# WD-Leong/CV-Lite-Object-Detection

Measured on AMD Instinct MI355X. Metric: training images/sec (whole node), FCOS-VOC 512x512 bs=16/GPU, higher is better.
Workload: dtype bf16; 1 GPU; FCOS ResNet-50-FPN train step (targets + fwd + loss + bwd + clip/SGD), 512x512, bs=16 per GPU; model=FCOS-ResNet50-FPN, global_batch=16, image_size=512, parallelism=dp1

## Files before the change

### cv-lite-object-detection_amd/csrc/conv_common.h

```cpp
#pragma once
#include "cvl_common.h"
#include "bn_acc.h"
#include <type_traits>

typedef short s16x8 __attribute__((ext_vector_type(8)));
typedef short s16x4 __attribute__((ext_vector_type(4)));
typedef __bf16 bf16x8 __attribute__((ext_vector_type(8)));
typedef float f32x4 __attribute__((ext_vector_type(4)));

constexpr int kMaxSeg = CVL_CONV_MAX_SEG;

extern thread_local int g_cvl_conv_last_kernel;
extern thread_local int g_cvl_conv_last_ktile;

__device__ __forceinline__ int xcd_remap(int b, int nwg) {
  const int q = nwg / 8, r = nwg % 8, x = b % 8;
  return (x < r ? x * (q + 1) : r * (q + 1) + (x - r) * q) + b / 8;
}

template <int N>
__device__ __forceinline__ void wait_vm() {
  __builtin_amdgcn_s_waitcnt((N & 15) | ((N >> 4) << 14) | (7 << 4) | (15 << 8));
}

__device__ __forceinline__ s16x4 ds_tr16(unsigned addr) {
  s16x4 v;
  asm volatile("ds_read_b64_tr_b16 %0, %1" : "=v"(v) : "v"(addr));
  return v;
}
__device__ __forceinline__ void lgkm_wait() { asm volatile("s_waitcnt lgkmcnt(0)" ::: "memory"); }
__device__ __forceinline__ void tr_pin(s16x4& v) { asm volatile("" : "+v"(v)); }
__device__ __forceinline__ s16x8 tr_join(s16x4 l, s16x4 h) {
  return s16x8{l[0], l[1], l[2], l[3], h[0], h[1], h[2], h[3]};
}

__device__ __forceinline__ unsigned lds_addr(const void* p) {
  return (unsigned)(size_t)(const __attribute__((address_space(3))) void*)p;
}

struct ConvSeg {
  int Hr, Wr, Hs, Ws;
  long src_base, src_img, dst_base, dst_img;
  int m_start;
  int rows;
  const cvl_bf16* w;
  const float* bias;
};

struct ConvArgs {
  const cvl_bf16* src;
  void* dst;
  acc_u64* stats;
  int acc_slots;
  int nseg, B;
  ConvSeg seg[kMaxSeg];
  int Cin, KH, KW, stride, pad_t, pad_l;
  int K, Npad, n_store, ld_dst, dst_coff, dst_f32, relu_out, relu_in;
  float beta;
  int m_tiles, m_total;
  float* slab;
  int splits, ksteps_per_split;
  int dbg;
  int dst_up, dst_w;
  const cvl_bf16* bz;
  const float* bmr;
  const float* bga;
  const float* bbe;
  acc_u64* bsum;
  float bhi;
  const cvl_bf16* by;
  unsigned long long* probe;
  const cvl_bf16* ymask;
};

uint64_t* cvl_probe_current(bool take);
void cvl_probe_enter_call();
void cvl_probe_leave_call();

__device__ __forceinline__ void probe_enter(unsigned long long* p) {
  if (blockIdx.x == 0 && threadIdx.x == 0) __hip_atomic_store(p, wall_clock64(), __ATOMIC_RELAXED, __HIP_MEMORY_SCOPE_AGENT);
}
__device__ __forceinline__ void probe_leave(unsigned long long* p) {
  __syncthreads();
  if (threadIdx.x == 0) {
    if (atomicAdd(p + 3, 1ull) == (unsigned long long)gridDim.x - 1) {
      const unsigned long long t = wall_clock64();
      const unsigned long long t0 = __hip_atomic_load(p, __ATOMIC_RELAXED, __HIP_MEMORY_SCOPE_AGENT);
      atomicAdd(p + 1, t - t0);
      atomicAdd(p + 2, 1ull);
      __hip_atomic_store(p + 3, 0ull, __ATOMIC_RELAXED, __HIP_MEMORY_SCOPE_AGENT);
    }
  }
}

int cvl_bn_acc_prepare(uint64_t* acc, long nstat, hipStream_t s);

int cvl_wgrad_reduce(const float* slab, float* dst0, float* dst1, long n4, int splits, int groups, float beta,
                     hipStream_t s);
int cvl_wgrad_defer_guard(const float* dst, hipStream_t s);
int cvl_wgrad_reduce_lanes(long elems4, int splits);

struct BnSumArgs {
  const cvl_bf16* z;
  const float* mr;
  const float* gamma;
  const float* beta;
  acc_u64* sums;
  float hi;
  const cvl_bf16* y;
};

enum { CVL_BSUM_NONE = 0, CVL_BSUM_Z = 1, CVL_BSUM_Y = 2 };
struct ConvCallOpts {
  bool bn_stats;
  int bsum;
  bool ymask;
  size_t workspace_bytes;
};

enum { CVL_PRE_NONE = 0, CVL_PRE_ZERO_GAPS = 1, CVL_PRE_S2DG3_PACK = 2 };

struct ConvPlan {
  int kernel;
  int bn, bk;
  bool dgrad;
  bool sw;
  bool wres;
  bool prio, acc, stamps;
  int stages;
  int bsum;
  bool ymask;
  int splits, ksteps_per_split;
  int grid;
  size_t workspace_bytes;
  int pre;
  size_t pack_bytes;
  int dbg;
  cvl_conv_desc desc;
  ConvArgs geo;
};

int conv_plan(const cvl_conv_desc* d, const ConvCallOpts& o, ConvPlan* p);
size_t conv_plan_workspace_bound(const cvl_conv_desc* d);
static inline void conv_plan_set_splits(ConvPlan* p, int nk, int want) {
  p->ksteps_per_split = (nk + want - 1) / want;
  p->splits = (nk + p->ksteps_per_split - 1) / p->ksteps_per_split;
}
static inline int conv_plan_ktile(const ConvPlan& p) { return p.kernel == CVL_CK_X32 || p.kernel == CVL_CK_P ? p.bk : 0; }

int launch_base(const ConvPlan& p, const ConvArgs& a, hipStream_t s);
int launch_l(const ConvPlan& p, const ConvArgs& a, hipStream_t s);
int launch_x(const ConvPlan& p, const ConvArgs& a, hipStream_t s);
int launch_h(const ConvPlan& p, const ConvArgs& a, hipStream_t s);
int launch_p(const ConvPlan& p, const ConvArgs& a, hipStream_t s);

bool cvl_conv_h_fits(const cvl_conv_desc* d, const ConvArgs& a, int* halo_px);
constexpr int kConvHWresCb = 2;
constexpr int kConvHStampWgs = 4096;
constexpr unsigned kConvBufRecords = 0x7fffffffu;

template <class F>
static inline void with_bool(bool b, F&& f) {
  if (b) f(std::true_type{});
  else f(std::false_type{});
}

__device__ __forceinline__ long conv_dst_row(const ConvArgs& a, const ConvSeg& S, int img, int q) {
  long r = q;
  if (a.dst_up != 1) {
    const int y = q / S.Wr, x = q - (q / S.Wr) * S.Wr;
    r = (long)y * a.dst_up * a.dst_w + (long)x * a.dst_up;
  }
  return S.dst_base + (long)img * S.dst_img + r;
}

static inline int cvl_conv_prepare(const cvl_conv_desc* d, int bm, ConvArgs* a) {
  CVL_CHECK_ARG(d);
  CVL_CHECK_ARG(d->nseg >= 1 && d->nseg <= kMaxSeg && d->B >= 1);
  CVL_CHECK_ARG(d->Cin > 0 && d->KH > 0 && d->KW > 0 && d->stride > 0);
  CVL_CHECK_ARG(d->mode == CVL_CONV_FWD || d->mode == CVL_CONV_DGRAD);
  CVL_CHECK_ARG(d->Npad > 0 && d->n_store > 0 && d->n_store <= d->Npad);
  CVL_CHECK_ARG(d->ld_dst >= d->dst_coff + d->n_store);
  a->slab = nullptr;
  a->splits = 1;
  a->ksteps_per_split = 0;
  a->dst_up = 1;
  a->dst_w = 0;
  a->dbg = 0;
  a->bz = nullptr; a->bmr = nullptr; a->bga = nullptr; a->bbe = nullptr; a->bsum = nullptr; a->bhi = 0.f;
  a->by = nullptr;
  a->probe = nullptr;
  a->ymask = nullptr;
  a->acc_slots = cvl_bn_acc_slots();
  a->nseg = d->nseg;
  a->B = d->B;
  a->Cin = d->Cin; a->KH = d->KH; a->KW = d->KW; a->stride = d->stride;
  a->pad_t = d->pad_t; a->pad_l = d->pad_l;
  a->K = d->KH * d->KW * d->Cin;
  a->Npad = d->Npad; a->n_store = d->n_store; a->ld_dst = d->ld_dst; a->dst_coff = d->dst_coff;
  a->dst_f32 = d->dst_f32; a->relu_out = d->relu_out; a->relu_in = d->relu_in; a->beta = d->beta;
  int m = 0;
  for (int i = 0; i < kMaxSeg; ++i) {
    ConvSeg& s = a->seg[i];
    if (i >= d->nseg) {
      s = a->seg[0];
      s.m_start = 0x7fffffff;
      continue;
    }
    const cvl_conv_seg& q = d->seg[i];
    CVL_CHECK_ARG(q.Hr > 0 && q.Wr > 0 && q.Hs > 0 && q.Ws > 0 && q.w);
    s.Hr = q.Hr; s.Wr = q.Wr; s.Hs = q.Hs; s.Ws = q.Ws;
    s.src_base = q.src_base; s.src_img = q.src_img; s.dst_base = q.dst_base; s.dst_img = q.dst_img;
    s.w = reinterpret_cast<const cvl_bf16*>(q.w);
    s.bias = q.bias;
    s.m_start = m;
    s.rows = d->B * q.Hr * q.Wr;
    m += ((s.rows + bm - 1) / bm) * bm;
  }
  a->m_total = m;
  a->m_tiles = m / bm;
  return CVL_OK;
}
```

### cv-lite-object-detection_amd/csrc/conv_dispatch.hip

```cpp
#include "conv_common.h"

namespace {

constexpr int BM_BASE = 128, NT_BASE = 256;
constexpr int BM = 256;
constexpr int H_BN = 64, H_BK = 32;

int device_cus() {
  static const int n = cvl_device_cus();
  return n;
}

int pick_bn(int npad) { return npad % 128 == 0 ? 128 : (npad % 64 == 0 ? 64 : 32); }

int base_split_want(const ConvArgs& a) {
  if (a.nseg != 1) return 1;
  const int BN_ = pick_bn(a.Npad), BK_ = a.Cin % 64 == 0 ? 64 : 32;
  const int tiles = a.m_tiles * (a.Npad / BN_);
  const int nk = a.K / BK_;
  const int max_tiles = cvl_tune_int("CVL_KSPLIT_MAX_TILES", 192);
  const int target = cvl_tune_int("CVL_KSPLIT_TARGET", 384);
  const int min_nk = cvl_dispatch_int("ksplit_min_nk", 4);
  if (tiles >= max_tiles || nk < min_nk) return 1;
  int s = (target + tiles - 1) / tiles;
// ... 55 lines not shown
    cvl_conv_seg& g = dd.seg[cls];
    g = q;
    g.Hr = q.Hs;
    g.Wr = q.Ws;
    g.w = sub + (size_t)cls * d->Npad * 4 * d->Cin;
    g.bias = nullptr;
    g.dst_base = q.dst_base + (long)(cls >> 1) * q.Wr + (cls & 1);
  }
  return dd;
}
const cvl_bf16* const kPackPlaceholder = reinterpret_cast<const cvl_bf16*>(16);

bool dst_chunks8(const cvl_conv_desc* d) { return d->n_store % 8 == 0 && d->ld_dst % 8 == 0 && d->dst_coff % 8 == 0; }

bool tiles_in_images(const ConvArgs& a, bool dense) {
  for (int i = 0; i < a.nseg; ++i) {
    const long hw = (long)a.seg[i].Hr * a.seg[i].Wr;
    if (hw % BM || (dense && a.seg[i].dst_img != hw)) return false;
  }
  return true;
}

bool buffer_bounds_ok(const ConvArgs& a) {
  for (int i = 0; i < a.nseg; ++i) {
    const ConvSeg& q = a.seg[i];
    const long src_bytes = (q.src_base + (long)a.B * q.src_img) * a.Cin * 2;
    if (src_bytes >= (long)kConvBufRecords - 65536) return false;
  }
  return (long)a.Npad * a.K * 2 < (long)kConvBufRecords;
}

bool x32_fits(const cvl_conv_desc* d, const ConvArgs& a) {
  const bool dg = d->mode == CVL_CONV_DGRAD;
  if (a.Npad % 256 || a.Cin % 32 || a.K / 32 < 1 || d->KH * d->KW > 32 || a.relu_in || (dg && d->stride != 1) ||
      a.dst_up != 1)
    return false;
  return buffer_bounds_ok(a);
}

bool plan_x(const cvl_conv_desc* d, const ConvArgs& a, const ConvCallOpts& o, ConvPlan* p) {
  if (cvl_dispatch_flag("no_x") || !x32_fits(d, a)) return false;
  p->kernel = CVL_CK_X32;
  p->bn = 256;
  p->bk = 32;
  p->grid = a.m_tiles * (a.Npad / 256);
  p->dbg = cvl_tune_int("CVL_X_ABLATE", 0);
  p->sw = !a.dst_f32 && !o.bn_stats && a.beta == 0.f && dst_chunks8(d) && !cvl_dispatch_flag("x_no_sw");
  p->ymask = p->sw && o.ymask && !a.relu_out && !cvl_dispatch_flag("no_relu_mask_fuse");
  return true;
}

bool p_fits(const cvl_conv_desc* d, const ConvArgs& a, const ConvCallOpts& o) {
  if (d->KH != 1 || d->KW != 1 || d->pad_t || d->pad_l || a.relu_in || a.nseg != 1 || a.K % 32) return false;
  const bool by = o.bsum == CVL_BSUM_Y;
  if (o.bsum && ((d->mode != CVL_CONV_DGRAD && a.dst_up == 1) || a.dst_f32 || (a.beta != 0.f) != by ||
                 (a.dst_up != 1 && !by) || o.bn_stats || (a.seg[0].Hr * a.seg[0].Wr) % BM ||
                 (a.dst_up == 1 && a.seg[0].dst_img != (long)a.seg[0].Hr * a.seg[0].Wr) || a.Npad % 64))
    return false;
  if (d->mode == CVL_CONV_DGRAD && d->stride != 1) return false;
  const ConvSeg& q = a.seg[0];
  if (d->stride == 1 && (q.Hs != q.Hr || q.Ws != q.Wr)) return false;
  if (a.dst_f32 ? (a.n_store % 4 || a.ld_dst % 4 || a.dst_coff % 4) : !dst_chunks8(d)) return false;
  if (o.bn_stats && (a.dst_f32 || (q.Hr * q.Wr) % BM)) return false;
  return buffer_bounds_ok(a);
}

bool plan_p(const cvl_conv_desc* d, const ConvArgs& a, const ConvCallOpts& o, ConvPlan* p) {
  if (cvl_dispatch_flag("no_p") || !p_fits(d, a, o)) return false;
  if (o.bsum && cvl_tune_flag("CVL_CONV_P_NO_BSUM")) return false;
  const bool wide = a.K <= 256 || (a.Npad >= 2 * a.K && cvl_dispatch_int("p_wide128", 1));
  const int bn = wide && a.Npad % 128 == 0 ? 128 : (a.Npad % 64 == 0 ? 64 : 0);
  const int fbn = cvl_dispatch_int("p_bn", 0);
  const int use = o.bsum ? 64 : (fbn && a.Npad % fbn == 0 ? fbn : bn);
  if (!use) return false;
  const int ntiles = a.m_tiles * (a.Npad / use);
  const int ntn = a.Npad / use;
  int grid = cvl_tune_int("CVL_CONV_P_WGS", 256);
  if (grid >= ntiles) grid = ntiles;
  else grid -= grid % ntn;
  if (grid < 1) return false;
  p->kernel = CVL_CK_P;
  p->bn = use;
  p->bk = a.K % 64 == 0 && use != 256 && cvl_dispatch_int("p_k64", 1) ? 64 : 32;
  p->grid = grid;
  p->dbg = cvl_tune_int("CVL_P_ABLATE", 0);
  p->bsum = o.bsum;
  p->acc = a.beta != 0.f && !cvl_tune_flag("CVL_P_NO_ACC");
  return true;
}

bool plan_h(const cvl_conv_desc* d, const ConvArgs& a, const ConvCallOpts& o, size_t ws_bytes, ConvPlan* p) {
  int halo_px = 0;
  if (cvl_dispatch_flag("no_h") || !cvl_conv_h_fits(d, a, &halo_px)) return false;
  const bool stg3 = !cvl_dispatch_flag("h_no_3stage") && halo_px <= 512;
  const bool bs = o.bsum != CVL_BSUM_NONE;
  p->kernel = CVL_CK_H64;
  p->bk = H_BK;
  p->bsum = o.bsum;
  if (a.Npad == 32) {
    if (o.bn_stats || bs) return false;
    p->bn = 32;
    p->stages = stg3 ? 3 : 2;
    p->grid = a.m_tiles < device_cus() ? a.m_tiles : device_cus();
    return true;
  }
  const int tiles = a.m_tiles * (a.Npad / H_BN);
  const bool sw_ok = !d->dst_f32 && d->beta == 0.f && dst_chunks8(d) && !(o.bn_stats && bs) && tiles_in_images(a, bs);
  if (!cvl_dispatch_flag("h_no_n32") && a.Npad % H_BN == 0 && 2 * tiles <= device_cus() && sw_ok) {
    p->bn = 32;
    p->sw = true;
    p->stages = stg3 ? 3 : 2;
    p->grid = 2 * tiles;
    return true;
  }
  const int ncb = a.Cin / H_BK;
  int splits = 1;
  if (a.nseg == 1 && !bs && ws_bytes && d->n_store % 8 == 0 && d->dst_coff % 8 == 0 &&
      (d->dst_f32 || d->ld_dst % 8 == 0) && d->n_store / 8 <= 256) {
    splits = h_split_want(a);
    if (slab_bytes(a, splits) > ws_bytes) splits = 1;
  }
  if (splits > 1) conv_plan_set_splits(p, ncb, splits);
  const int per_cu = cvl_tune_int("CVL_CONV_H_WG_PER_CU", 1);
  p->grid = p->splits > 1 ? tiles : (tiles < device_cus() * per_cu ? tiles : device_cus() * per_cu);
  p->bn = H_BN;
  p->stages = 2;
  p->wres = p->splits <= 1 && a.Npad == H_BN && ncb <= kConvHWresCb && a.nseg == 1 && !cvl_dispatch_flag("h_no_wres");
  p->sw = p->splits <= 1 && sw_ok && !cvl_dispatch_flag("h_no_sw");
  p->stamps = cvl_tune_flag("CVL_H_STAMPS") && p->splits <= 1 && p->grid <= kConvHStampWgs;
  return true;
}

bool large_fits(const cvl_conv_desc* d, const ConvCallOpts& o) {
  if (d->Cin % 32 != 0 || d->relu_in) return false;
  return d->dst_f32 ? (d->n_store % 4 == 0 && !o.bn_stats) : dst_chunks8(d);
}

bool plan_large(const cvl_conv_desc* d, const ConvArgs& a, const ConvCallOpts& o, ConvPlan* p) {
  if (cvl_dispatch_flag("no_l")) return false;
  const bool bs = o.bsum != CVL_BSUM_NONE, by = o.bsum == CVL_BSUM_Y;
  if (bs && (d->mode != CVL_CONV_DGRAD || d->dst_f32 || (d->beta != 0.f && !by) || a.dst_up != 1 || o.bn_stats))
    return false;
  if (by && (d->KH != 1 || d->KW != 1)) return false;
  if (d->Npad == 32 && d->KH == 3 && d->KW == 3 && d->mode == CVL_CONV_FWD && d->dst_f32 && !o.bn_stats &&
      !bs && a.dst_up == 1 && d->Cin % 32 == 0 && !d->relu_in && !cvl_dispatch_flag("no_h32"))
    return plan_h(d, a, o, 0, p);
  if (!large_fits(d, o)) return false;
  if (d->dst_f32 && (cvl_tune_flag("CVL_CONV_L_F32_N8") || cvl_tune_flag("CVL_CONV_L_NO_F32"))) return false;
  const bool l_cin = d->Cin % 64 == 0;
  const bool w256 = d->Npad % 256 == 0 && !cvl_dispatch_flag("no_256") &&
                    (d->mode == CVL_CONV_FWD || !cvl_tune_flag("CVL_CONV_NO_DGRAD_256"));
  const int bn = w256 ? 256 : (d->Npad % 128 == 0 ? 128 : (d->Npad % 64 == 0 ? 64 : 0));
  if (!bn) return false;
  if (l_cin && d->KH * d->KW * d->Cin < cvl_tune_int("CVL_CONV_L_MIN_K", 0) && !bs) return false;
  if (d->KH == 1 && d->KW == 1) {
    if (plan_p(d, a, o, p)) return true;
    if (by) return false;
  }
  const long min_tiles = cvl_dispatch_int("l_min_tiles", 128);
  int use_bn = bn;
  if (use_bn == 256 && (long)a.m_tiles * (a.Npad / 256) < cvl_dispatch_int("l256_min_tiles", 256)) use_bn = 128;
  const int w256_min_k = cvl_dispatch_int("w256_min_k", 512);
  if (use_bn == 256 && a.K < w256_min_k) use_bn = 128;
  const int fill = cvl_tune_int("CVL_CONV_L64_FILL", 256);
  const bool fill_pre = !cvl_tune_flag("CVL_CONV_L64_NO_FILL_PRE");
  const bool to64 = fill && use_bn == 128 && (long)a.m_tiles * (a.Npad / 128) < fill && a.Npad % 64 == 0 &&
                    !(bs && cvl_tune_flag("CVL_BSUM_NO_FILL"));
  if (!l_cin && d->Cin == 32 && bn == 256 && !bs && !o.bn_stats && cvl_dispatch_int("x_cin32", 1) &&
      plan_x(d, a, o, p))
    return true;
  const bool h_width = use_bn == 64 || to64 || !l_cin || cvl_tune_flag("CVL_CONV_H_ANY_N");
  if (h_width && use_bn != 256 && (!bs || ((a.seg[0].Hr * a.seg[0].Wr) % BM == 0 && !o.bn_stats)) &&
      (!bs || tiles_in_images(a, true)) && plan_h(d, a, o, o.workspace_bytes, p))
    return true;
  if (!l_cin) return false;
  if (fill_pre && to64) use_bn = 64;
  if ((long)a.m_tiles * (a.Npad / use_bn) < min_tiles) return false;
  if (to64) use_bn = 64;
  if (o.bn_stats)
    for (int i = 0; i < a.nseg; ++i)
      if ((a.seg[i].Hr * a.seg[i].Wr) % 4) return false;
  if (bs && (use_bn == 256 || !tiles_in_images(a, true))) return false;
  if (use_bn == 256 && plan_x(d, a, o, p)) return true;
  p->kernel = use_bn == 256 ? CVL_CK_L256 : (use_bn == 128 ? CVL_CK_L128 : CVL_CK_L64);
  p->bn = use_bn;
  p->bk = 64;
  p->grid = a.m_tiles * (a.Npad / use_bn);
  p->bsum = o.bsum;
  p->prio = !cvl_tune_flag("CVL_CONV_NO_PRIO");
  p->sw = !a.dst_f32 && a.beta == 0.f && !bs && a.dst_up == 1 && dst_chunks8(d) && !cvl_dispatch_flag("l_no_sw") &&
          (!o.bn_stats || tiles_in_images(a, false));
  return true;
}

void plan_base(const cvl_conv_desc* d, const ConvArgs& a, const ConvCallOpts& o, ConvPlan* p) {
// ... 127 lines not shown
```

### cv-lite-object-detection_amd/csrc/conv_igemm.hip

```cpp
#include "conv_common.h"

namespace {

constexpr int BM = 128;
constexpr int NT = 256;

template <int BK>
__device__ __forceinline__ int swz(int r) {
  return BK == 128 ? (r & 15) : (BK == 64 ? ((r >> 1) & 7) : ((r >> 2) & 3));
}

__device__ __forceinline__ s16x8 relu_bf16x8(s16x8 v) {
#pragma unroll
  for (int i = 0; i < 8; ++i) v[i] = v[i] < 0 ? (short)0 : v[i];
  return v;
}



template <int BN, int BK, bool DGRAD>
__global__ void __launch_bounds__(NT) conv_igemm_kernel(ConvArgs a) {
  constexpr int WM = BM / 2, WN = BN / 2;
  constexpr int TM = WM / 16, TN = WN / 16;
  constexpr int CPR = BK / 8;
// ... 398 lines not shown
  for (int line = blockIdx.y; line < B * H; line += gridDim.y) {
    const int img = line / H, y = line - img * H;
    const bool full = y % s != 0;
    const long base = dst_base + (long)img * dst_img + (long)y * W;
    for (int i = blockIdx.x * blockDim.x + threadIdx.x; i < W * n8; i += gridDim.x * blockDim.x) {
      const int x = i / n8, c = i - x * n8;
      if (!full && x % s == 0) continue;
      const long row = base + x;
      if (is_f32) reinterpret_cast<float*>(dst)[row * ld + coff + c] = 0.f;
      else *reinterpret_cast<s16x8*>(reinterpret_cast<cvl_bf16*>(dst) + row * ld + coff + c * 8) = s16x8{0, 0, 0, 0, 0, 0, 0, 0};
    }
  }
}

namespace {

int pre_pass(const ConvPlan& p, const cvl_conv_desc* d, void* dst, void* workspace, hipStream_t s) {
  if (p.pre == CVL_PRE_S2DG3_PACK) {
    const long b = (16L * d->Npad * (d->Cin / 8) + NT - 1) / NT;
    hipLaunchKernelGGL(s2dgrad3_pack_kernel, dim3((int)(b > 4096 ? 4096 : (b < 1 ? 1 : b))), dim3(NT), 0, s,
                       reinterpret_cast<const cvl_bf16*>(d->seg[0].w), reinterpret_cast<cvl_bf16*>(workspace), d->Npad,
                       d->Cin);
  } else if (p.pre == CVL_PRE_ZERO_GAPS) {
    const cvl_conv_seg& q = d->seg[0];
    const long line = (long)q.Wr * (d->dst_f32 ? d->n_store : d->n_store / 8);
    const int bx = (int)((line + NT - 1) / NT);
    const int by = d->B * q.Hr < 65535 ? d->B * q.Hr : 65535;
    hipLaunchKernelGGL(zero_gaps_kernel, dim3(bx < 1 ? 1 : bx, by), dim3(NT), 0, s, dst, d->dst_f32, q.dst_base,
                       q.dst_img, d->ld_dst, d->dst_coff, d->n_store, d->B, q.Hr, q.Wr, d->stride);
  } else {
    return CVL_OK;
  }
  return cvl_launch_status();
}

struct ConvIo {
  const void* src;
  void* dst;
  acc_u64* stats;
  const BnSumArgs* bsum;
  const void* ymask;
  void* workspace;
};

void fill_args(const ConvPlan& p, const ConvIo& io, ConvArgs* a) {
  *a = p.geo;
  a->src = reinterpret_cast<const cvl_bf16*>(io.src);
  a->dst = io.dst;
  a->stats = io.stats;
  if (p.bsum) {
    const BnSumArgs& b = *io.bsum;
    a->bz = b.z; a->bmr = b.mr; a->bga = b.gamma; a->bbe = b.beta; a->bsum = b.sums; a->bhi = b.hi;
    a->by = b.y;
  }
  if (p.ymask) a->ymask = reinterpret_cast<const cvl_bf16*>(io.ymask);
  if (p.kernel == CVL_CK_X32) a->probe = reinterpret_cast<unsigned long long*>(cvl_probe_current(true));
  a->dbg = p.dbg;
  a->splits = p.splits;
  a->ksteps_per_split = p.ksteps_per_split;
  char* ws = reinterpret_cast<char*>(io.workspace);
  if (p.splits > 1) a->slab = reinterpret_cast<float*>(ws + p.pack_bytes);
  if (p.pre == CVL_PRE_S2DG3_PACK)
    for (int i = 0; i < kMaxSeg; ++i)
      a->seg[i].w = reinterpret_cast<const cvl_bf16*>(ws) + (size_t)(i < a->nseg ? i : 0) * a->Npad * a->K;
}

}

thread_local int g_cvl_conv_last_kernel = CVL_CK_NONE;
thread_local int g_cvl_conv_last_ktile = 0;

extern "C" int cvl_conv_igemm_last_kernel(void) { return g_cvl_conv_last_kernel; }
extern "C" int cvl_conv_igemm_last_ktile(void) { return g_cvl_conv_last_ktile; }

int launch_base(const ConvPlan& p, const ConvArgs& a, hipStream_t s) {
  if (p.bn == 128) launch_bn<128>(p, a, s);
  else if (p.bn == 64) launch_bn<64>(p, a, s);
  else launch_bn<32>(p, a, s);
  return cvl_launch_status();
}

namespace {
int conv_run(const ConvPlan& p, const cvl_conv_desc* d, const ConvIo& io, hipStream_t s) {
  int st = pre_pass(p, d, io.dst, io.workspace, s);
  if (st) return st;
  ConvArgs a;
  fill_args(p, io, &a);
  switch (p.kernel) {
    case CVL_CK_P: st = launch_p(p, a, s); break;
    case CVL_CK_X32: st = launch_x(p, a, s); break;
    case CVL_CK_H64: st = launch_h(p, a, s); break;
    case CVL_CK_L64: case CVL_CK_L128: case CVL_CK_L256: st = launch_l(p, a, s); break;
    default: st = launch_base(p, a, s); break;
  }
  g_cvl_conv_last_kernel = p.kernel;
  g_cvl_conv_last_ktile = conv_plan_ktile(p);
  if (st || p.splits <= 1) return st;
  return splitk_finish_launch(a, s);
}
}

extern "C" const char* cvl_conv_kernel_name(int code) {
  switch (code) {
    case CVL_CK_BASE: return "conv_igemm_kernel (128-row)";
    case CVL_CK_BASE_SPLITK: return "conv_igemm_kernel (128-row, split-K)";
    case CVL_CK_L64: return "conv_igemm_l_kernel<64> (256x64)";
// ... 9 lines not shown
    case CVL_CK_WG_X: return "conv_wgrad_x_kernel (256x256, 5-slot ring of 32-row steps, grouped)";
    case CVL_CK_WG_H: return "conv_wgrad_h_kernel (64 ci x 64 co x 9 taps, 128-row halo steps)";
    case CVL_CK_H64: return "conv_igemm_h_kernel (256x64, 3x3 halo + 9-tap weight stage per channel block)";
    case CVL_CK_P: return "conv_igemm_p_kernel (persistent 1x1, K-tile stream across tiles)";
    default: return "none";
  }
}

int cvl_conv_f32(const cvl_conv_desc* d, const void* src, void* dst, acc_u64* bn_stats, hipStream_t s);
int cvl_relu_backward(const void* dy, const void* y, void* dx, long n, float beta, cvl_stream_t stream);

extern "C" size_t cvl_conv_igemm_workspace_size(const cvl_conv_desc* d) {
  if (!d) return 0;
  if (d->prec == CVL_PREC_F32) return 16;
  return conv_plan_workspace_bound(d);
}

extern "C" int cvl_conv_igemm(const cvl_conv_desc* d, const void* src, void* dst, uint64_t* bn_stats_acc,
                              void* workspace, size_t workspace_bytes, cvl_stream_t stream) {
  CVL_CHECK_ARG(d);
  acc_u64* bn_stats = reinterpret_cast<acc_u64*>(bn_stats_acc);
  if (d->prec == CVL_PREC_F32) return cvl_conv_f32(d, src, dst, bn_stats, (hipStream_t)stream);
  ConvPlan p;
  const int st = conv_plan(d, ConvCallOpts{bn_stats != nullptr, CVL_BSUM_NONE, false, workspace ? workspace_bytes : 0}, &p);
  if (st) return st;
  CVL_CHECK_ARG(src && dst);
  cvl_probe_enter_call();
  const int rst = conv_run(p, d, ConvIo{src, dst, bn_stats, nullptr, nullptr, workspace}, (hipStream_t)stream);
  cvl_probe_leave_call();
  return rst;
}

extern "C" int cvl_conv_igemm_relu_mask(const cvl_conv_desc* d, const void* src, void* dst, const void* y,
                                        void* workspace, size_t workspace_bytes, cvl_stream_t stream) {
  CVL_CHECK_ARG(d && src && dst && y && d->mode == CVL_CONV_DGRAD && d->prec == CVL_PREC_BF16 && !d->dst_f32 &&
                d->beta == 0.f && !d->relu_out);
  ConvPlan p;
  int st = conv_plan(d, ConvCallOpts{false, CVL_BSUM_NONE, true, workspace ? workspace_bytes : 0}, &p);
  if (st) return st;
  if (!p.ymask) CVL_CHECK_ARG(d->ld_dst == d->n_store && d->dst_coff == 0);
  cvl_probe_enter_call();
  st = conv_run(p, d, ConvIo{src, dst, nullptr, nullptr, y, workspace}, (hipStream_t)stream);
  cvl_probe_leave_call();
  if (st || p.ymask) return st;
  long rows = 0;
  for (int i = 0; i < d->nseg; ++i) {
    const long e = d->seg[i].dst_base + (long)d->B * (d->seg[i].dst_img ? d->seg[i].dst_img : (long)d->seg[i].Hr * d->seg[i].Wr);
    rows = e > rows ? e : rows;
  }
  return cvl_relu_backward(dst, y, dst, rows * d->n_store, 0.f, stream);
}

namespace {
int dgrad_bnsum_call(const cvl_conv_desc* d, const void* src, void* dst, int form, const BnSumArgs& b, int32_t* fused,
                     void* workspace, size_t workspace_bytes, cvl_stream_t stream) {
  *fused = 0;
  if (d->prec == CVL_PREC_F32) return cvl_conv_f32(d, src, dst, nullptr, (hipStream_t)stream);
  const size_t ws = workspace ? workspace_bytes : 0;
  ConvPlan p;
  int st = conv_plan(d, ConvCallOpts{false, form, false, ws}, &p);
  if (st) return st;
  const bool fuse = p.kernel != CVL_CK_NONE && src && dst;
  if (!fuse && (st = conv_plan(d, ConvCallOpts{false, CVL_BSUM_NONE, false, ws}, &p))) return st;
  CVL_CHECK_ARG(src && dst);
  if (!fuse) cvl_probe_enter_call();
  st = conv_run(p, d, ConvIo{src, dst, nullptr, &b, nullptr, workspace}, (hipStream_t)stream);
  if (!fuse) cvl_probe_leave_call();
  *fused = fuse && st == CVL_OK ? 1 : 0;
  return st;
}
}

extern "C" int cvl_conv_igemm_dgrad_bnsum(const cvl_conv_desc* d, const void* src, void* dst, const void* z,
                                          const float* mean_rstd, const float* gamma, const float* beta, float act_hi,
                                          uint64_t* sums, int32_t* fused, void* workspace, size_t workspace_bytes,
                                          cvl_stream_t stream) {
  CVL_CHECK_ARG(d && fused && z && mean_rstd && gamma && beta && sums);
  const BnSumArgs b{reinterpret_cast<const cvl_bf16*>(z), mean_rstd, gamma, beta, reinterpret_cast<acc_u64*>(sums),
                    act_hi, nullptr};
  return dgrad_bnsum_call(d, src, dst, CVL_BSUM_Z, b, fused, workspace, workspace_bytes, stream);
}

extern "C" int cvl_conv_igemm_dgrad_bnsum_res(const cvl_conv_desc* d, const void* src, void* dst, const void* y,
                                              const void* z, const float* mean_rstd, const float* gamma,
                                              const float* beta, uint64_t* sums, int32_t* fused, void* workspace,
                                              size_t workspace_bytes, cvl_stream_t stream) {
  CVL_CHECK_ARG(d && fused && y && z && mean_rstd && gamma && beta && sums);
  const BnSumArgs b{reinterpret_cast<const cvl_bf16*>(z), mean_rstd, gamma, beta, reinterpret_cast<acc_u64*>(sums),
                    INFINITY, reinterpret_cast<const cvl_bf16*>(y)};
  return dgrad_bnsum_call(d, src, dst, CVL_BSUM_Y, b, fused, workspace, workspace_bytes, stream);
}
```

### cv-lite-object-detection_amd/csrc/conv_igemm_p.hip

```cpp
#include "conv_common.h"

namespace {

constexpr int NT = 512, BM = 256;
constexpr unsigned kRecords = 0x7fffffffu;
constexpr unsigned kOOB = 0x80000000u;
constexpr int LDS_BYTES = 163840;

template <int BK>
__device__ __forceinline__ int swz(int r) { return (r >> 1) & (BK / 8 - 1); }

__device__ __forceinline__ void dma16(__amdgpu_buffer_rsrc_t r, const void* lds_dst, unsigned voff) {
  __builtin_amdgcn_raw_ptr_buffer_load_lds(r, (__attribute__((address_space(3))) void*)lds_dst, 16, (int)voff, 0,
                                           0, 0);
}

template <int BN, int BK>
struct PCfg {
  static constexpr int WGM = BN == 256 ? 2 : 4, WGN = 8 / WGM;
  static constexpr int WM = BM / WGM, WN = BN / WGN, TM = WM / 16, TN = WN / 16;
  static constexpr int SLOT_B = (BM + BN) * BK * 2;
  static constexpr int PR = 8 * 64 * 16 / (BK * 2);
  static constexpr int APW = BM / PR;
  static constexpr int BPW = BN >= PR ? BN / PR : 1;
  static constexpr int PW = APW + BPW;
  static constexpr int RED_B = WGM * BN * 2 * 4;
  static constexpr int DUMMY_B = BN < PR ? 4 * 1024 : 0;
  static constexpr int NS = (LDS_BYTES - RED_B - DUMMY_B) / SLOT_B;
  static constexpr int D = NS - 1;
  static_assert(D >= 2, "ring too short");
};

typedef __bf16 bf16x2 __attribute__((ext_vector_type(2)));
typedef float f32x2 __attribute__((ext_vector_type(2)));
typedef unsigned u32x4 __attribute__((ext_vector_type(4)));

__device__ __forceinline__ void wait_vm_atleast(int n) {
  if (n >= 63) wait_vm<63>();
  else if (n >= 48) wait_vm<48>();
  else if (n >= 36) wait_vm<36>();
  else if (n >= 30) wait_vm<30>();
  else if (n >= 24) wait_vm<24>();
  else if (n >= 21) wait_vm<21>();
  else if (n >= 18) wait_vm<18>();
  else if (n >= 15) wait_vm<15>();
  else if (n >= 12) wait_vm<12>();
  else if (n >= 9) wait_vm<9>();
  else if (n >= 6) wait_vm<6>();
  else if (n >= 3) wait_vm<3>();
  else wait_vm<0>();
}

__device__ __forceinline__ s16x8 gload16_untracked(const void* p) {
  s16x8 v;
  asm volatile("global_load_dwordx4 %0, %1, off" : "=v"(v) : "v"(p) : "memory");
  return v;
}
__device__ __forceinline__ void pin16(s16x8& v) { asm volatile("" : "+v"(v)); }

template <int BN, int BK, bool RELU, bool F32, int BS = 0, bool ACC = false>
__global__ void __launch_bounds__(NT) conv_igemm_p_kernel(ConvArgs a, int ntiles) {
  using C = PCfg<BN, BK>;
  constexpr int TM = C::TM, TN = C::TN, NS = C::NS, D = C::D;
  __shared__ __attribute__((aligned(16))) char lds[C::NS * C::SLOT_B + C::RED_B + C::DUMMY_B];
  float* red = reinterpret_cast<float*>(lds + NS * C::SLOT_B);
  char* dummy = lds + NS * C::SLOT_B + C::RED_B;

  const int tid = threadIdx.x;
  const int wave = __builtin_amdgcn_readfirstlane(tid >> 6), lane = tid & 63;
  const ConvSeg& S = a.seg[0];
  const int HWr = S.Hr * S.Wr;
  const int ntn = a.Npad / BN;
  const int nk = a.K / BK;
  const int G = gridDim.x;
  const int L = xcd_remap(blockIdx.x, G);
  const int nmc = G / ntn;
  const int mchunk = (a.m_tiles + nmc - 1) / nmc;
  const int mt0 = (L / ntn) * mchunk;
  const int my_tiles = max(0, min(mchunk, a.m_tiles - mt0));
  const int total = my_tiles * nk;
  const bool dense_src = a.stride == 1 && S.Hs == S.Hr && S.Ws == S.Wr && S.src_img == (long)HWr;
  const int Cin2 = a.Cin * 2;
  const int K2 = a.K * 2;

  constexpr int LPR = BK / 8, PR = C::PR, WR = PR / 8;
  const int prow = wave * WR + lane / LPR, ch = lane % LPR;
  const unsigned chs = (unsigned)((ch ^ swz<BK>(prow)) * 16);
  const __amdgpu_buffer_rsrc_t rsA = __builtin_amdgcn_make_buffer_rsrc((void*)a.src, (short)0, (int)kRecords, 0x00020000);
  const __amdgpu_buffer_rsrc_t rsB = __builtin_amdgcn_make_buffer_rsrc((void*)S.w, (short)0, (int)kRecords, 0x00020000);

  int ik = 0, it = 0, islot = 0;
  unsigned ia[C::APW], ib[C::BPW];
  const int n0 = (L % ntn) * BN;
  auto set_issue_tile = [&](int k) {
    const int m0 = (mt0 + k) * BM;
#pragma unroll
    for (int p = 0; p < C::APW; ++p) {
      const int ml = ((a.dbg & 16) ? 0 : m0) + p * PR + prow;
      long pix;
      if (dense_src) {
        pix = S.src_base + ml;
      } else {
        const int img = ml / HWr, q = ml - img * HWr;
        const int oy = q / S.Wr, ox = q - oy * S.Wr;
        pix = S.src_base + (long)img * S.src_img + (long)(oy * a.stride) * S.Ws + ox * a.stride;
      }
      ia[p] = ml < S.rows ? (unsigned)(pix * Cin2) + chs : kOOB;
    }
#pragma unroll
    for (int j = 0; j < C::BPW; ++j) {
      const int nr = n0 + j * PR + prow;
// ... 20 lines not shown
    if (live && ++ik == nk) {
      ik = 0;
      ++it;
      if (it < my_tiles) set_issue_tile(it);
    }
  };

  const int wm = wave / C::WGN, wn = wave % C::WGN;
  const int lr = lane & 15, lg = lane >> 4;
  unsigned fao[TM], fbo[TN];
#pragma unroll
  for (int i = 0; i < TM; ++i) {
    const int r = wm * C::WM + i * 16 + lr;
    fao[i] = (unsigned)(r * BK * 2 + ((lg ^ swz<BK>(r)) * 16));
  }
#pragma unroll
  for (int j = 0; j < TN; ++j) {
    const int r = wn * C::WN + j * 16 + lr;
    fbo[j] = (unsigned)(BM * BK * 2 + r * BK * 2 + ((lg ^ swz<BK>(r)) * 16));
  }
  f32x4 acc[TM][TN];
#pragma unroll
  for (int i = 0; i < TM; ++i)
#pragma unroll
    for (int j = 0; j < TN; ++j) acc[i][j] = f32x4{0.f, 0.f, 0.f, 0.f};

  float bcol[TN][4];
#pragma unroll
  for (int j = 0; j < TN; ++j)
#pragma unroll
    for (int e = 0; e < 4; ++e) {
      const int n = n0 + wn * C::WN + j * 16 + 4 * lg + e;
      bcol[j][e] = (S.bias && n < a.n_store) ? S.bias[n] : 0.f;
    }
  constexpr int NJP = BS ? TN / 2 : 1;
  const int lgo = ((lg & 1) ? 16 : 0) + ((lg & 2) ? 8 : 0);
  float bga[NJP][8], bbe[NJP][8], bm[NJP][8], brs[NJP][8], bs1[NJP][8], bs2[NJP][8];
  int bimg = -1;
  if (BS) {
#pragma unroll
    for (int jp = 0; jp < NJP; ++jp)
#pragma unroll
      for (int u = 0; u < 8; ++u) {
        const int c = n0 + wn * C::WN + jp * 32 + lgo + u;
        bga[jp][u] = a.bga[c];
        bbe[jp][u] = a.bbe[c];
        bs1[jp][u] = 0.f;
        bs2[jp][u] = 0.f;
      }
  }
  wait_vm<0>();
  s16x8 zv[BS ? TM : 1][NJP];
  s16x8 yv[BS == 2 ? TM : 1][BS == 2 ? NJP : 1];
  s16x8 ov[ACC ? TM : 1][ACC ? TN / 2 : 1];

  float ss1[TN][4], ss2[TN][4];
#pragma unroll
  for (int j = 0; j < TN; ++j)
#pragma unroll
    for (int e = 0; e < 4; ++e) { ss1[j][e] = 0.f; ss2[j][e] = 0.f; }
  auto row16_sum = [](float v) {
    v += __int_as_float(__builtin_amdgcn_mov_dpp(__float_as_int(v), 0xB1, 0xF, 0xF, false));
    v += __int_as_float(__builtin_amdgcn_mov_dpp(__float_as_int(v), 0x4E, 0xF, 0xF, false));
    v += __int_as_float(__builtin_amdgcn_mov_dpp(__float_as_int(v), 0x141, 0xF, 0xF, false));
    v += __int_as_float(__builtin_amdgcn_mov_dpp(__float_as_int(v), 0x140, 0xF, 0xF, false));
    return v;
  };
  auto flush_stats = [&](int img) {
#pragma unroll
    for (int j = 0; j < TN; ++j)
#pragma unroll
      for (int e = 0; e < 4; ++e) {
        const float s1 = row16_sum(ss1[j][e]), s2 = row16_sum(ss2[j][e]);
        ss1[j][e] = 0.f;
        ss2[j][e] = 0.f;
        if (lr == 0) {
          const int c = wn * C::WN + j * 16 + 4 * lg + e;
          red[(wm * BN + c) * 2] = s1;
          red[(wm * BN + c) * 2 + 1] = s2;
        }
      }
    __syncthreads();
    if (tid < BN && n0 + tid < a.n_store) {
      float t1 = 0.f, t2 = 0.f;
#pragma unroll
      for (int w = 0; w < C::WGM; ++w) { t1 += red[(w * BN + tid) * 2]; t2 += red[(w * BN + tid) * 2 + 1]; }
      acc_u64* st = a.stats + acc_idx((long)img * a.n_store + n0 + tid, 0, a.acc_slots);
      acc_add(st, t1, a.acc_slots);
      acc_add(st + a.acc_slots, t2, a.acc_slots);
    }
  };

  auto flush_bsum = [&](int img) {
#pragma unroll
    for (int jp = 0; jp < NJP; ++jp)
#pragma unroll
      for (int u = 0; u < 8; ++u) {
        const float t1 = row16_sum(bs1[jp][u]), t2 = row16_sum(bs2[jp][u]);
        bs1[jp][u] = 0.f;
        bs2[jp][u] = 0.f;
        if (lr == 0) {
          const int c = wn * C::WN + jp * 32 + lgo + u;
          red[(wm * BN + c) * 2] = t1;
          red[(wm * BN + c) * 2 + 1] = t2;
        }
      }
    __syncthreads();
    if (tid < BN && n0 + tid < a.n_store) {
      float t1 = 0.f, t2 = 0.f;
#pragma unroll
      for (int w = 0; w < C::WGM; ++w) { t1 += red[(w * BN + tid) * 2]; t2 += red[(w * BN + tid) * 2 + 1]; }
      acc_u64* st = a.bsum + acc_idx((long)img * a.n_store + n0 + tid, 0, a.acc_slots);
      acc_add(st, t1, a.acc_slots);
      acc_add(st + a.acc_slots, t2, a.acc_slots);
    }
  };

  auto epilogue = [&](int k) {
    const int m0 = (mt0 + k) * BM;
    const bool dense_dst = a.dst_up == 1 && S.dst_img == (long)HWr;
    const bool do_stats = a.stats && !(a.dbg & 1);
    if (ACC) {
      wait_vm_atleast(C::PW * (nk - 1));
#pragma unroll
      for (int i = 0; i < TM; ++i)
#pragma unroll
        for (int jp = 0; jp < TN / 2; ++jp) pin16(ov[i][jp]);
    }
    if (BS) {
      wait_vm_atleast(C::PW * (nk - 1));
#pragma unroll
      for (int i = 0; i < TM; ++i)
#pragma unroll
        for (int jp = 0; jp < NJP; ++jp) {
          pin16(zv[i][jp]);
          if (BS == 2) pin16(yv[i][jp]);
        }
      const int img = m0 / HWr;
      if (img != bimg) {
        bimg = img;
#pragma unroll
        for (int jp = 0; jp < NJP; ++jp)
#pragma unroll
          for (int u = 0; u < 8; ++u) {
            const long bc = (long)img * a.n_store + n0 + wn * C::WN + jp * 32 + lgo + u;
            bm[jp][u] = a.bmr[bc * 2];
            brs[jp][u] = a.bmr[bc * 2 + 1];
          }
      }
    }
#pragma unroll
    for (int i = 0; i < TM; ++i) {
      const int ml = m0 + wm * C::WM + i * 16 + lr;
      const bool row_ok = ml < S.rows && !(a.dbg & 2);
      long drow;
      if (dense_dst || !row_ok) {
        drow = S.dst_base + ml;
      } else {
        const int img = ml / HWr, q = ml - img * HWr;
        drow = conv_dst_row(a, S, img, q);
      }
      if (F32) {
#pragma unroll
        for (int j = 0; j < TN; ++j) {
          f32x4 v;
#pragma unroll
          for (int e = 0; e < 4; ++e) {
            v[e] = acc[i][j][e] + bcol[j][e];
            if (RELU) v[e] = fmaxf(v[e], 0.f);
          }
          const int n = n0 + wn * C::WN + j * 16 + 4 * lg;
          if (!row_ok || n >= a.n_store) continue;
          f32x4* pd = reinterpret_cast<f32x4*>(reinterpret_cast<float*>(a.dst) + drow * a.ld_dst + a.dst_coff + n);
          if (a.beta != 0.f) v += a.beta * *pd;
          *pd = v;
        }
        continue;
      }
#pragma unroll
      for (int j = 0; j < TN; j += 2) {
        unsigned pk[2][2];
#pragma unroll
        for (int jj = 0; jj < 2; ++jj)
#pragma unroll
          for (int h = 0; h < 2; ++h) {
            float v0 = acc[i][j + jj][2 * h] + bcol[j + jj][2 * h];
            float v1 = acc[i][j + jj][2 * h + 1] + bcol[j + jj][2 * h + 1];
            if (RELU) { v0 = fmaxf(v0, 0.f); v1 = fmaxf(v1, 0.f); }
            const unsigned u = __builtin_bit_cast(unsigned, __builtin_convertvector((f32x2){v0, v1}, bf16x2));
            pk[jj][h] = u;
            if (do_stats) {
              const float r0 = __uint_as_float(u << 16), r1 = __uint_as_float(u & 0xffff0000u);
              ss1[j + jj][2 * h] += r0;
              ss2[j + jj][2 * h] = __builtin_fmaf(r0, r0, ss2[j + jj][2 * h]);
              ss1[j + jj][2 * h + 1] += r1;
              ss2[j + jj][2 * h + 1] = __builtin_fmaf(r1, r1, ss2[j + jj][2 * h + 1]);
            }
          }
#pragma unroll
        for (int h = 0; h < 2; ++h) {
          const auto sw = __builtin_amdgcn_permlane16_swap(pk[0][h], pk[1][h], false, false);
          pk[0][h] = sw[0];
          pk[1][h] = sw[1];
        }
        const int n = n0 + wn * C::WN + j * 16 + ((lg & 1) ? 16 : 0) + ((lg & 2) ? 8 : 0);
        if (!row_ok || n >= a.n_store) continue;
        s16x8* pd = reinterpret_cast<s16x8*>(reinterpret_cast<cvl_bf16*>(a.dst) + drow * a.ld_dst + a.dst_coff + n);
        s16x8 o = __builtin_bit_cast(s16x8, (u32x4){pk[0][0], pk[0][1], pk[1][0], pk[1][1]});
        if (ACC) {
          const s16x8 old = ov[i][j / 2];
#pragma unroll
          for (int u = 0; u < 8; ++u)
            o[u] = (short)f32_to_bf16(bf16_to_f32((cvl_bf16)o[u]) + a.beta * bf16_to_f32((cvl_bf16)old[u]));
        } else if (a.beta != 0.f) {
          const s16x8 old = *pd;
#pragma unroll
          for (int u = 0; u < 8; ++u)
            o[u] = (short)f32_to_bf16(bf16_to_f32((cvl_bf16)o[u]) + a.beta * bf16_to_f32((cvl_bf16)old[u]));
        }
        if (BS) {
          const s16x8 zz = zv[i][j / 2];
#pragma unroll
          for (int u = 0; u < 8; ++u) {
            const float zf = bf16_to_f32((cvl_bf16)zz[u]);
            const float xh = (zf - bm[j / 2][u]) * brs[j / 2][u];
            bool on;
            if (BS == 2) {
              on = bf16_to_f32((cvl_bf16)yv[i][j / 2][u]) > 0.f;
            } else {
              const float af = __builtin_fmaf(bga[j / 2][u], xh, bbe[j / 2][u]);
              on = af > 0.f && af < a.bhi;
            }
            const float gv = on ? bf16_to_f32((cvl_bf16)o[u]) : 0.f;
            bs1[j / 2][u] += gv;
            bs2[j / 2][u] = __builtin_fmaf(gv, xh, bs2[j / 2][u]);
          }
        }
        *pd = o;
      }
    }
    if (do_stats) {
      const int img = m0 / HWr;
      if (k == my_tiles - 1 || (m0 + BM) / HWr != img) flush_stats(img);
    }
    if (BS) {
      const int img = m0 / HWr;
      if (k == my_tiles - 1 || (m0 + BM) / HWr != img) flush_bsum(img);
    }
#pragma unroll
    for (int i = 0; i < TM; ++i)
#pragma unroll
      for (int j = 0; j < TN; ++j) acc[i][j] = f32x4{0.f, 0.f, 0.f, 0.f};
  };

  unsigned long long* stamp = ((a.dbg & 8) && tid == 0) ? reinterpret_cast<unsigned long long*>(a.dst) + blockIdx.x * 4 : nullptr;
  if (stamp) stamp[0] = wall_clock64();
#pragma unroll
  for (int d = 0; d < D; ++d) issue();
  int rslot = 0, ck = 0, ct = 0;
  for (int g = 0; g < total; ++g) {
    wait_vm<(D - 1) * C::PW>();
    __builtin_amdgcn_s_barrier();
    asm volatile("" ::: "memory");
    issue();
    if (ACC && ck == 0) {
      const int m0 = (mt0 + ct) * BM;
      const bool dense_dst = a.dst_up == 1 && S.dst_img == (long)HWr;
#pragma unroll
      for (int i = 0; i < TM; ++i) {
        const int ml = m0 + wm * C::WM + i * 16 + lr;
        long drow = S.dst_base;
        if (ml < S.rows) {
          if (dense_dst) {
            drow = S.dst_base + ml;
          } else {
            const int img = ml / HWr, q = ml - img * HWr;
            drow = conv_dst_row(a, S, img, q);
          }
        }
#pragma unroll
        for (int jp = 0; jp < TN / 2; ++jp) {
          int n = n0 + wn * C::WN + jp * 32 + lgo;
          if (n >= a.n_store) n = 0;
          ov[i][jp] = gload16_untracked(reinterpret_cast<const cvl_bf16*>(a.dst) + drow * a.ld_dst + a.dst_coff + n);
        }
      }
    }
    if (BS && ck == 0) {
      const int m0 = (mt0 + ct) * BM;
      const bool dense_dst = a.dst_up == 1 && S.dst_img == (long)HWr;
#pragma unroll
      for (int i = 0; i < TM; ++i)
#pragma unroll
        for (int jp = 0; jp < NJP; ++jp) {
          const int ml = m0 + wm * C::WM + i * 16 + lr;
          long row = S.dst_base + ml;
          if (!dense_dst && ml < S.rows) {
            const int img = ml / HWr, q = ml - img * HWr;
            row = conv_dst_row(a, S, img, q);
          }
          zv[i][jp] = gload16_untracked(a.bz + row * a.ld_dst + a.dst_coff + n0 + wn * C::WN + jp * 32 + lgo);
          if (BS == 2)
            yv[i][jp] = gload16_untracked(a.by + row * a.ld_dst + a.dst_coff + n0 + wn * C::WN + jp * 32 + lgo);
        }
    }
    const char* sl = lds + rslot * C::SLOT_B;
#pragma unroll
    for (int kh = 0; kh < BK / 32; ++kh) {
      s16x8 fa[TM], fb[TN];
#pragma unroll
      for (int i = 0; i < TM; ++i) fa[i] = *reinterpret_cast<const s16x8*>(sl + (fao[i] ^ (unsigned)(kh * 64)));
#pragma unroll
      for (int j = 0; j < TN; ++j) fb[j] = *reinterpret_cast<const s16x8*>(sl + (fbo[j] ^ (unsigned)(kh * 64)));
#pragma unroll
      for (int i = 0; i < TM; ++i)
#pragma unroll
        for (int j = 0; j < TN; ++j)
          acc[i][j] = __builtin_amdgcn_mfma_f32_16x16x32_bf16(__builtin_bit_cast(bf16x8, fb[j]),
                                                               __builtin_bit_cast(bf16x8, fa[i]), acc[i][j], 0, 0, 0);
    }
    rslot = rslot == NS - 1 ? 0 : rslot + 1;
    if (++ck == nk) {
      ck = 0;
      epilogue(ct);
      ++ct;
    }
  }
  wait_vm<0>();
  if (stamp) { stamp[1] = wall_clock64(); stamp[2] = total; }
}

template <int BN_, int BK_, bool ACC_>
void p_launch(const ConvPlan& p, const ConvArgs& a, hipStream_t s) {
  const dim3 grid(p.grid);
  const int ntiles = a.m_tiles * (a.Npad / p.bn);
  if (p.bsum == CVL_BSUM_Y) {
    hipLaunchKernelGGL((conv_igemm_p_kernel<64, BK_, false, false, 2, true>), grid, dim3(NT), 0, s, a, ntiles);
  } else if (p.bsum) {
    hipLaunchKernelGGL((conv_igemm_p_kernel<64, BK_, false, false, 1>), grid, dim3(NT), 0, s, a, ntiles);
  } else if (a.dst_f32) {
    with_bool(a.relu_out != 0, [&](auto RELU) {
      hipLaunchKernelGGL((conv_igemm_p_kernel<BN_, BK_, decltype(RELU)::value, true>), grid, dim3(NT), 0, s, a, ntiles);
    });
  } else if (a.relu_out) {
    hipLaunchKernelGGL((conv_igemm_p_kernel<BN_, BK_, true, false>), grid, dim3(NT), 0, s, a, ntiles);
  } else if (p.acc) {
    hipLaunchKernelGGL((conv_igemm_p_kernel<BN_, BK_, false, false, false, ACC_>), grid, dim3(NT), 0, s, a, ntiles);
  } else {
    hipLaunchKernelGGL((conv_igemm_p_kernel<BN_, BK_, false, false>), grid, dim3(NT), 0, s, a, ntiles);
  }
}

}

int launch_p(const ConvPlan& p, const ConvArgs& a, hipStream_t s) {
  if (p.bn == 256) p_launch<256, 32, false>(p, a, s);
  else if (p.bn == 128 && p.bk == 64) p_launch<128, 64, true>(p, a, s);
  else if (p.bn == 128) p_launch<128, 32, true>(p, a, s);
  else if (p.bk == 64) p_launch<64, 64, true>(p, a, s);
  else p_launch<64, 32, true>(p, a, s);
  return cvl_launch_status();
}
```

### cv-lite-object-detection_amd/csrc/nn_ops.hip

```cpp
#include "conv_common.h"

namespace {

constexpr int NT = 256;

__device__ __forceinline__ void unpack8(s16x8 v, float* f) {
#pragma unroll
  for (int i = 0; i < 8; ++i) f[i] = bf16_to_f32((cvl_bf16)v[i]);
}
__device__ __forceinline__ s16x8 pack8(const float* f) {
  s16x8 v;
#pragma unroll
  for (int i = 0; i < 8; ++i) v[i] = (short)f32_to_bf16(f[i]);
  return v;
}

#ifndef BN_NT
#define BN_NT 1
#endif
__device__ __forceinline__ s16x8 ld_rows(const cvl_bf16* p) {
  if (BN_NT) return __builtin_nontemporal_load(reinterpret_cast<const s16x8*>(p));
  return *reinterpret_cast<const s16x8*>(p);
}

// ... 204 lines not shown
  const int c = blockIdx.x * NT + threadIdx.x;
  if (c >= C) return;
  for (int b = 0; b < B; ++b) {
    float mean, rstd;
    double var;
    const long bc = (long)b * C + c;
    bn_moments(acc_dec(stats, bc, 0, slots), acc_dec(stats, bc, 1, slots), HW, eps, &mean, &rstd, &var);
    mr[((long)b * C + c) * 2] = mean;
    mr[((long)b * C + c) * 2 + 1] = rstd;
  }
  if (run_mean) bn_running(stats, slots, B, C, c, HW, eps, momentum, run_mean, run_var);
}

struct BnFin {
  const acc_u64* stats;
  float* mr_out;
  float* run_mean;
  float* run_var;
  float eps, momentum;
  int slots;
};

#ifndef BNA_UNR_V
#define BNA_UNR_V 4
#endif
constexpr int BNA_UNR = BNA_UNR_V;

constexpr int BN_FIN_MAXC = 2048;

struct BnRes {
  const cvl_bf16* z;
  const float* gamma;
  const float* beta;
  BnFin fin;
};

__device__ __forceinline__ void bn_fin_prologue(const BnFin& fin, float2* smr, int b, int C, int HW) {
  for (int c = threadIdx.x; c < C; c += NT) {
    const long bc = (long)b * C + c;
    float mm, rr;
    double var;
    bn_moments(acc_dec(fin.stats, bc, 0, fin.slots), acc_dec(fin.stats, bc, 1, fin.slots), HW, fin.eps, &mm, &rr, &var);
    smr[c] = float2{mm, rr};
    if (blockIdx.x == 0) { fin.mr_out[bc * 2] = mm; fin.mr_out[bc * 2 + 1] = rr; }
  }
}

__device__ __forceinline__ void bn_fin_running(const BnFin& fin, int nimg, int C, int HW) {
  if (fin.run_mean)
    for (int c = blockIdx.x * NT + threadIdx.x; c < C; c += gridDim.x * NT)
      bn_running(fin.stats, fin.slots, nimg, C, c, HW, fin.eps, fin.momentum, fin.run_mean, fin.run_var);
}

template <bool FIN, bool RBN = false>
__global__ void __launch_bounds__(NT) bn_apply_kernel(const cvl_bf16* __restrict__ z, const float* __restrict__ mr,
                                                      const float* __restrict__ gamma, const float* __restrict__ beta,
                                                      const cvl_bf16* __restrict__ res, cvl_bf16* __restrict__ y,
                                                      int C, int HW, int relu, int rows_per_blk, BnFin fin,
                                                      BnRes rb) {
  static_assert(FIN || !RBN, "the BN residual form fuses both finalizes");
  const int b = FIN ? (int)blockIdx.y - 1 : (int)blockIdx.y;
  const int C8 = C / 8;
  const int tpr = C8 < NT ? C8 : NT;
  const int rpp = NT / tpr;
  const int cg = threadIdx.x % tpr, rsub = threadIdx.x / tpr;
  __shared__ float2 smr[FIN ? BN_FIN_MAXC : 1];
  __shared__ float2 smr2[RBN ? BN_FIN_MAXC : 1];
  if (FIN && b < 0) {
    bn_fin_running(fin, (int)gridDim.y - 1, C, HW);
    if (RBN) bn_fin_running(rb.fin, (int)gridDim.y - 1, C, HW);
    return;
  }
  if (FIN) {
    bn_fin_prologue(fin, smr, b, C, HW);
    if (RBN) bn_fin_prologue(rb.fin, smr2, b, C, HW);
    __syncthreads();
  }
  if (rsub >= rpp) return;
  const int r0 = blockIdx.x * rows_per_blk;
  const int r1 = min(r0 + rows_per_blk, HW);
  for (int cgb = cg; cgb < C8; cgb += tpr) {
    const int c0 = cgb * 8;
    float m[8], rs[8], ga[8], be[8];
    float m2[8], rs2[8], ga2[8], be2[8];
#pragma unroll
    for (int u = 0; u < 8; ++u) {
      const long bc = (long)b * C + c0 + u;
      if (FIN) {
        m[u] = smr[c0 + u].x;
        rs[u] = smr[c0 + u].y;
      } else {
        m[u] = mr[bc * 2];
        rs[u] = mr[bc * 2 + 1];
      }
      ga[u] = gamma[c0 + u];
      be[u] = beta[c0 + u];
      if (RBN) {
        m2[u] = smr2[c0 + u].x;
        rs2[u] = smr2[c0 + u].y;
        ga2[u] = rb.gamma[c0 + u];
        be2[u] = rb.beta[c0 + u];
      }
    }
    const cvl_bf16* rsrc = RBN ? rb.z : res;
    for (int r = r0 + rsub; r < r1; r += rpp * BNA_UNR) {
      s16x8 vz[BNA_UNR], vr[BNA_UNR];
      long off[BNA_UNR];
#pragma unroll
      for (int q = 0; q < BNA_UNR; ++q) {
        const int rq = min(r + q * rpp, r1 - 1);
        off[q] = ((long)b * HW + rq) * C + c0;
        vz[q] = ld_rows(z + off[q]);
        if (rsrc) vr[q] = ld_rows(rsrc + off[q]);
      }
#pragma unroll
      for (int q = 0; q < BNA_UNR; ++q) {
        if (r + q * rpp >= r1) break;
        float v[8], rr[8];
        unpack8(vz[q], v);
        if (RBN) {
          unpack8(vr[q], rr);
#pragma unroll
          for (int u = 0; u < 8; ++u) rr[u] = bn_affine(rr[u], m2[u], rs2[u], ga2[u], be2[u]);
          unpack8(pack8(rr), rr);
        } else if (res) {
          unpack8(vr[q], rr);
        }
#pragma unroll
        for (int u = 0; u < 8; ++u) {
          float o = bn_affine(v[u], m[u], rs[u], ga[u], be[u]);
          if (RBN || res) o += rr[u];
          if (relu) o = o > 0.f ? o : 0.f;
          if (relu == 2) o = fminf(o, 6.0f);
          v[u] = o;
        }
        *reinterpret_cast<s16x8*>(y + off[q]) = pack8(v);
      }
    }
  }
}

inline int bn_rows_per_blk(int B, int HW, int C) {
  const int C8 = C / 8, tpr = C8 < NT ? C8 : NT, rpp = NT / tpr;
  static const int target = cvl_tune_int("CVL_BNA_BLOCKS", 1024);
  const int chunks = (target + B - 1) / B;
  int rpb = (HW + chunks - 1) / chunks;
  const int lo = rpp * 4 * (C8 > NT ? 1 : 1);
  rpb = rpb < lo ? lo : rpb;
  return (rpb + rpp - 1) / rpp * rpp;
}

inline int bn1_rows_per_blk(int B, int HW, int C) {
  const int C8 = C / 8, tpr = C8 < NT ? C8 : NT, rpp = NT / tpr;
  static const int target = cvl_tune_int("CVL_BNB1_BLOCKS", 512);
  const int chunks = (target + B - 1) / B;
  int rpb = (HW + chunks - 1) / chunks;
  const int lo = rpp * 4;
  rpb = rpb < lo ? lo : rpb;
  return (rpb + rpp - 1) / rpp * rpp;
}

#ifndef BN_UNR_V
#define BN_UNR_V 4
#endif
constexpr int BN_UNR = BN_UNR_V;

struct BnPG {
  float* dgamma;
  float* dbeta;
  float* conv_dbias;
  float beta_acc;
  const acc_u64* psums;
  int slots;
  const cvl_bf16* sc_z = nullptr;
  const float* sc_mr = nullptr;
};

template <int PASS, int MASK = 0, bool SC = false>
__global__ void __launch_bounds__(NT) bn_bwd_kernel(const cvl_bf16* __restrict__ dy, const cvl_bf16* __restrict__ y,
                                                    const cvl_bf16* __restrict__ z, const float* __restrict__ mr,
                                                    const float* __restrict__ gamma, const acc_u64* __restrict__ sums,
                                                    cvl_bf16* __restrict__ dz, cvl_bf16* __restrict__ g_out,
                                                    float* __restrict__ part, int C, int HW, int rows_per_blk,
                                                    int group, float dz_beta, BnPG pg,
                                                    const float* __restrict__ bnb, float act_hi) {
  const int nimg = PASS == 1 ? (int)gridDim.y - 1 : (int)gridDim.y;
  const int b = PASS == 1 ? (int)blockIdx.y - 1 : (int)blockIdx.y;
  const int C8 = C / 8;
  const int tpr = C8 < NT ? C8 : NT;
  const int rpp = NT / tpr;
  const int cg = threadIdx.x % tpr, rsub = threadIdx.x / tpr;
  const int r0 = blockIdx.x * rows_per_blk;
  const int r1 = min(r0 + rows_per_blk, HW);
  const int g0 = (b / group) * group;
  const int gsz = min(g0 + group, nimg) - g0;
  const float inv = 1.0f / ((float)HW * (float)gsz);
  __shared__ float red[NT][17];
  if (PASS == 1 && b < 0) {
    if (!pg.dgamma) return;
    const acc_u64* ps = pg.psums ? pg.psums : sums;
    for (int c = blockIdx.x * NT + threadIdx.x; c < C; c += gridDim.x * NT) {
      if (pg.conv_dbias) pg.conv_dbias[c] = 0.f;
      double a1 = 0.0, a2 = 0.0;
#pragma unroll 8
      for (int bb = 0; bb < nimg; ++bb) {
        a1 += acc_dec(ps, (long)bb * C + c, 0, pg.slots);
        a2 += acc_dec(ps, (long)bb * C + c, 1, pg.slots);
      }
      pg.dbeta[c] = (float)a1 + (pg.beta_acc != 0.f ? pg.beta_acc * pg.dbeta[c] : 0.f);
      pg.dgamma[c] = (float)a2 + (pg.beta_acc != 0.f ? pg.beta_acc * pg.dgamma[c] : 0.f);
    }
    return;
  }
  const int n_iter = (C8 + tpr - 1) / tpr;
  for (int itr = 0; itr < n_iter; ++itr) {
    const int cgb = itr * tpr + cg;
    const bool act = cgb < C8;
    const int c0 = (act ? cgb : C8 - 1) * 8;
    float m[8], rs[8], s1[8], s2[8], k1[8], k2[8], gm[8], ga[8], be[8];
    float msc[8], rssc[8];
    const bool use_y = PASS != 2 && (MASK == 0 ? y != nullptr : MASK == 1);
    const bool zmask = PASS != 2 && (MASK == 0 ? (!y && bnb) : MASK == 2);
#pragma unroll
    for (int u = 0; u < 8; ++u) {
      const long bc = (long)b * C + c0 + u;
      m[u] = PASS == 2 ? 0.f : mr[bc * 2];
      rs[u] = PASS == 2 ? 1.f : mr[bc * 2 + 1];
      ga[u] = zmask ? gamma[c0 + u] : 0.f;
      be[u] = zmask ? bnb[c0 + u] : 0.f;
      s1[u] = 0.f; s2[u] = 0.f;
      if (PASS == 1) {
        k1[u] = (float)acc_dec(sums, bc, 0, pg.slots) * inv;
        k2[u] = (float)acc_dec(sums, bc, 1, pg.slots) * inv;
        gm[u] = gamma[c0 + u] * rs[u];
      }
      if (SC) {
        msc[u] = pg.sc_mr[bc * 2];
        rssc[u] = pg.sc_mr[bc * 2 + 1];
      }
    }

    if (rsub < rpp && act) {
      for (int r = r0 + rsub; r < r1; r += rpp * BN_UNR) {
        s16x8 vg[BN_UNR], vz[BN_UNR], vy[BN_UNR], vs[SC ? BN_UNR : 1];
        long off[BN_UNR];
#pragma unroll
        for (int q = 0; q < BN_UNR; ++q) {
          const int rq = min(r + q * rpp, r1 - 1);
          off[q] = ((long)b * HW + rq) * C + c0;
          vg[q] = ld_rows(dy + off[q]);
          if (PASS != 2) vz[q] = ld_rows(z + off[q]);
          if (use_y) vy[q] = ld_rows(y + off[q]);
          if (SC) vs[q] = ld_rows(pg.sc_z + off[q]);
        }
#pragma unroll
        for (int q = 0; q < BN_UNR; ++q) {
          const bool ok = r + q * rpp < r1;
          float g[8], zz[8];
          unpack8(vg[q], g);
          if (PASS == 2) {
            if (ok) {
#pragma unroll
              for (int u = 0; u < 8; ++u) { s1[u] += g[u]; s2[u] += g[u] * g[u]; }
            }
            continue;
          }
          unpack8(vz[q], zz);
          if (use_y) {
            float yy[8];
            unpack8(vy[q], yy);
#pragma unroll
            for (int u = 0; u < 8; ++u) g[u] = (yy[u] > 0.f && yy[u] < act_hi) ? g[u] : 0.f;
          } else if (zmask) {
#pragma unroll
            for (int u = 0; u < 8; ++u) {
              const float a = bn_affine(zz[u], m[u], rs[u], ga[u], be[u]);
              g[u] = (a > 0.f && a < act_hi) ? g[u] : 0.f;
            }
          }
          if (PASS == 0) {
            if (ok) {
#pragma unroll
              for (int u = 0; u < 8; ++u) {
                s1[u] += g[u];
                s2[u] += g[u] * ((zz[u] - m[u]) * rs[u]);
              }
            }
          } else if (ok) {
            if (g_out) *reinterpret_cast<s16x8*>(g_out + off[q]) = pack8(g);
            if (SC) {
              float zs[8];
              unpack8(vs[q], zs);
#pragma unroll
              for (int u = 0; u < 8; ++u) {
                s1[u] += g[u];
                s2[u] += g[u] * ((zs[u] - msc[u]) * rssc[u]);
              }
            }
            float o[8];
#pragma unroll
            for (int u = 0; u < 8; ++u) {
              const float xh = (zz[u] - m[u]) * rs[u];
              o[u] = gm[u] * (g[u] - k1[u] - xh * k2[u]);
            }
            if (dz_beta != 0.f) {
              float old[8];
              unpack8(*reinterpret_cast<const s16x8*>(dz + off[q]), old);
#pragma unroll
              for (int u = 0; u < 8; ++u) o[u] += dz_beta * old[u];
            }
            *reinterpret_cast<s16x8*>(dz + off[q]) = pack8(o);
          }
        }
      }
    }
    if (PASS == 1 && !SC) continue;
    __syncthreads();
#pragma unroll
    for (int u = 0; u < 8; ++u) { red[threadIdx.x][u] = s1[u]; red[threadIdx.x][8 + u] = s2[u]; }
    __syncthreads();
    if (rsub == 0 && act) {
      float* pp = part + (((long)b * gridDim.x + blockIdx.x) * C + c0) * 2;
      for (int u = 0; u < 8; ++u) {
        float a1 = 0.f, a2 = 0.f;
        for (int k = 0; k < rpp; ++k) { a1 += red[k * tpr + cg][u]; a2 += red[k * tpr + cg][8 + u]; }
// ... 834 lines not shown
  if (Kp % 8 == 0 && Kp <= I2C_MAXK && KH <= 7 && KW <= 7 && stride >= 1 && stride <= 2 && C <= 4 &&
      (long)B * Ho < (1L << 24)) {
    const int nseg = (Wo + I2C_PX - 1) / I2C_PX;
    const int nrb = (Ho + I2C_OY - 1) / I2C_OY;
    hipLaunchKernelGGL(im2col_tile_kernel, dim3(B * nrb * nseg), dim3(NT), 0, S_, x, (cvl_bf16*)out, H, W, C, KH, KW,
                       stride, pad_t, pad_l, Ho, Wo, Kp / 8);
    return cvl_launch_status();
  }
  if (Kp % 8 == 0 && total / 8 < (1L << 31) - NT && (long)H * W * C < (1L << 31)) {
    const int n8 = (int)(total / 8);
    hipLaunchKernelGGL(im2col8_kernel, dim3((n8 + NT - 1) / NT), dim3(NT), 0, S_, x, (cvl_bf16*)out, n8, H, W, C,
                       KW, KH * KW * C, stride, pad_t, pad_l, Ho, Wo, Kp / 8);
    return cvl_launch_status();
  }
  hipLaunchKernelGGL(im2col_kernel, dim3(grid_for(total)), dim3(NT), 0, S_, x, (cvl_bf16*)out, B, H, W,
                     C, KH, KW, stride, pad_t, pad_l, Ho, Wo, Kp);
  return cvl_launch_status();
}

extern "C" int cvl_bn_acc_slots(void) { return g_acc_slots; }

int cvl_bn_acc_prepare(uint64_t* acc, long nstat, hipStream_t s) { return acc_decode_launch((acc_u64*)acc, nstat, s); }

extern "C" int cvl_bn_set_exact(int on) {
  g_acc_slots = on ? kAccSlots : 1;
  return CVL_OK;
}

extern "C" int cvl_bn_acc_decode(const uint64_t* acc, double* out, int64_t n, cvl_stream_t stream) {
  CVL_CHECK_ARG(acc && out && n >= 0);
  if (n == 0) return CVL_OK;
  hipLaunchKernelGGL(bn_acc_decode_kernel, dim3(grid_for(n)), dim3(NT), 0, S_, (const acc_u64*)acc, out, (long)n,
                     g_acc_slots);
  return cvl_launch_status();
}

extern "C" int cvl_bn_finalize(uint64_t* stats, float* mean_rstd, float* run_mean, float* run_var,
                               int B, int C, int HW, float eps, float momentum, cvl_stream_t stream) {
  CVL_CHECK_ARG(stats && mean_rstd && B > 0 && C > 0 && HW > 0);
  const int dst = acc_decode_launch((acc_u64*)stats, 2L * B * C, S_);
  if (dst) return dst;
  hipLaunchKernelGGL(bn_finalize_kernel, dim3((C + NT - 1) / NT), dim3(NT), 0, S_, (const acc_u64*)stats, mean_rstd,
                     run_mean, run_var, B, C, HW, eps, momentum, g_acc_slots);
  return cvl_launch_status();
}

extern "C" int cvl_bn_apply(const void* z, const float* mean_rstd, const float* gamma, const float* beta,
                            const void* residual, void* y, int B, int HW, int C, int relu,
                            cvl_stream_t stream) {
  CVL_CHECK_ARG(z && mean_rstd && gamma && beta && y && C % 8 == 0 && B > 0 && HW > 0);
  const int rpb = bn_rows_per_blk(B, HW, C);
  hipLaunchKernelGGL(bn_apply_kernel<false>, dim3((HW + rpb - 1) / rpb, B), dim3(NT), 0, S_, (const cvl_bf16*)z,
                     mean_rstd, gamma, beta, (const cvl_bf16*)residual, (cvl_bf16*)y, C, HW, relu, rpb,
                     BnFin{nullptr, nullptr, nullptr, nullptr, 0.f, 0.f, 1}, BnRes{});
  return cvl_launch_status();
}

extern "C" int cvl_bn_finalize_apply(uint64_t* stats, float* mean_rstd, float* run_mean, float* run_var,
                                     const void* z, const float* gamma, const float* beta, const void* residual,
                                     void* y, int B, int HW, int C, int relu, float eps, float momentum,
                                     cvl_stream_t stream) {
  CVL_CHECK_ARG(stats && mean_rstd && z && gamma && beta && y && C % 8 == 0 && B > 0 && HW > 0);
  CVL_CHECK_ARG(C <= BN_FIN_MAXC);
  CVL_CHECK_ARG((run_mean == nullptr) == (run_var == nullptr));
  const int dst = acc_decode_launch((acc_u64*)stats, 2L * B * C, S_);
  if (dst) return dst;
  const int rpb = bn_rows_per_blk(B, HW, C);
  hipLaunchKernelGGL(bn_apply_kernel<true>, dim3((HW + rpb - 1) / rpb, B + 1), dim3(NT), 0, S_, (const cvl_bf16*)z,
                     (const float*)nullptr, gamma, beta, (const cvl_bf16*)residual, (cvl_bf16*)y, C, HW, relu, rpb,
                     BnFin{(const acc_u64*)stats, mean_rstd, run_mean, run_var, eps, momentum, g_acc_slots}, BnRes{});
  return cvl_launch_status();
}

extern "C" int cvl_bn_finalize_apply_bnres(uint64_t* stats, float* mean_rstd, float* run_mean, float* run_var,
                                           const void* z, const float* gamma, const float* beta, uint64_t* res_stats,
                                           float* res_mean_rstd, float* res_run_mean, float* res_run_var,
                                           const void* res_z, const float* res_gamma, const float* res_beta,
                                           float res_eps, float res_momentum, void* y, int B, int HW, int C, int relu,
                                           float eps, float momentum, cvl_stream_t stream) {
  CVL_CHECK_ARG(stats && mean_rstd && z && gamma && beta && y && C % 8 == 0 && B > 0 && HW > 0);
  CVL_CHECK_ARG(res_stats && res_mean_rstd && res_z && res_gamma && res_beta);
  CVL_CHECK_ARG(C <= BN_FIN_MAXC);
  CVL_CHECK_ARG((run_mean == nullptr) == (run_var == nullptr));
  CVL_CHECK_ARG((res_run_mean == nullptr) == (res_run_var == nullptr));
  int dst = acc_decode_launch((acc_u64*)stats, 2L * B * C, S_);
  if (!dst) dst = acc_decode_launch((acc_u64*)res_stats, 2L * B * C, S_);
  if (dst) return dst;
  const int rpb = bn_rows_per_blk(B, HW, C);
  hipLaunchKernelGGL((bn_apply_kernel<true, true>), dim3((HW + rpb - 1) / rpb, B + 1), dim3(NT), 0, S_, (const cvl_bf16*)z,
                     (const float*)nullptr, gamma, beta, (const cvl_bf16*)nullptr, (cvl_bf16*)y, C, HW, relu, rpb,
                     BnFin{(const acc_u64*)stats, mean_rstd, run_mean, run_var, eps, momentum, g_acc_slots},
                     BnRes{(const cvl_bf16*)res_z, res_gamma, res_beta,
                           BnFin{(const acc_u64*)res_stats, res_mean_rstd, res_run_mean, res_run_var, res_eps,
                                 res_momentum, g_acc_slots}});
  return cvl_launch_status();
}

extern "C" size_t cvl_bn_backward_workspace_size(int B, int HW, int C) {
  if (B <= 0 || HW <= 0 || C <= 0) return 0;
  const int rpb = bn_bwd_rows_per_blk(B, HW, C);
  const int nchunk = (HW + rpb - 1) / rpb;
  return sizeof(acc_u64) * 2 * (size_t)B * C + sizeof(double) * 2 * (size_t)C +
         sizeof(float) * 2 * 2 * (size_t)B * nchunk * C;
}

static int bn_backward_impl(const void* dy, const void* y_relu, const float* bn_beta, const void* z,
                            const float* mean_rstd, const float* gamma, void* workspace, size_t workspace_bytes,
                            void* dz, void* g_out, float* dgamma, float* dbeta, float beta_acc, float* conv_dbias,
                            int B, int HW, int C, cvl_stream_t stream, float act_hi = INFINITY) {
  CVL_CHECK_ARG(dy && z && mean_rstd && gamma && workspace && dz && dgamma && dbeta && C % 8 == 0);
  CVL_CHECK_ARG(B > 0 && HW > 0);
  CVL_CHECK_ARG(workspace_bytes >= cvl_bn_backward_workspace_size(B, HW, C));
  const int rpb = bn_bwd_rows_per_blk(B, HW, C);
  const int nchunk = (HW + rpb - 1) / rpb;
  acc_u64* sums = reinterpret_cast<acc_u64*>(workspace);
  double* dbsum = reinterpret_cast<double*>(sums + 2 * (size_t)B * C);
  float* part0 = reinterpret_cast<float*>(dbsum + 2 * (size_t)C);
  dim3 g1(nchunk, B);
  const bool ym = y_relu != nullptr, zm = !ym && bn_beta != nullptr;
  auto k0 = ym ? bn_bwd_kernel<0, 1> : zm ? bn_bwd_kernel<0, 2> : bn_bwd_kernel<0, 3>;
  auto k1 = ym ? bn_bwd_kernel<1, 1> : zm ? bn_bwd_kernel<1, 2> : bn_bwd_kernel<1, 3>;
  hipLaunchKernelGGL(k0, g1, dim3(NT), 0, S_, (const cvl_bf16*)dy, (const cvl_bf16*)y_relu,
                     (const cvl_bf16*)z, mean_rstd, gamma, (const acc_u64*)nullptr, (cvl_bf16*)nullptr,
                     (cvl_bf16*)nullptr, part0, C, HW, rpb, 1, 0.f, BnPG{}, bn_beta, act_hi);
  hipLaunchKernelGGL(bn_colsum_kernel, dim3((C + 31) / 32, B), dim3(NT), 0, S_, (const float*)part0, nchunk, C,
                     sums, 1);
  const int rpb1 = bn1_rows_per_blk(B, HW, C);
  hipLaunchKernelGGL(k1, dim3((HW + rpb1 - 1) / rpb1, B + 1), dim3(NT), 0, S_, (const cvl_bf16*)dy, (const cvl_bf16*)y_relu,
                     (const cvl_bf16*)z, mean_rstd, gamma, (const acc_u64*)sums, (cvl_bf16*)dz, (cvl_bf16*)g_out,
                     (float*)nullptr, C, HW, rpb1, 1, 0.f, BnPG{dgamma, dbeta, conv_dbias, beta_acc, nullptr, 1}, bn_beta,
                     act_hi);
  return cvl_launch_status();
}

extern "C" int cvl_bn_backward(const void* dy, const void* y_relu, const void* z, const float* mean_rstd,
                               const float* gamma, void* workspace, size_t workspace_bytes, void* dz, void* g_out,
                               float* dgamma, float* dbeta, float beta_acc, float* conv_dbias, int B, int HW,
                               int C, cvl_stream_t stream) {
  return bn_backward_impl(dy, y_relu, nullptr, z, mean_rstd, gamma, workspace, workspace_bytes, dz, g_out, dgamma,
                          dbeta, beta_acc, conv_dbias, B, HW, C, stream);
}

extern "C" int cvl_bn_backward_relu(const void* dy, const void* z, const float* mean_rstd, const float* gamma,
                                    const float* beta, void* workspace, size_t workspace_bytes, void* dz,
                                    float* dgamma, float* dbeta, float beta_acc, float* conv_dbias, int B, int HW,
                                    int C, cvl_stream_t stream) {
  CVL_CHECK_ARG(beta);
  return bn_backward_impl(dy, nullptr, beta, z, mean_rstd, gamma, workspace, workspace_bytes, dz, nullptr, dgamma,
                          dbeta, beta_acc, conv_dbias, B, HW, C, stream);
}

extern "C" int cvl_bn_backward_relu6(const void* dy, const void* z, const float* mean_rstd, const float* gamma,
                                     const float* beta, void* workspace, size_t workspace_bytes, void* dz,
                                     float* dgamma, float* dbeta, float beta_acc, float* conv_dbias, int B, int HW,
                                     int C, cvl_stream_t stream) {
  CVL_CHECK_ARG(beta);
  return bn_backward_impl(dy, nullptr, beta, z, mean_rstd, gamma, workspace, workspace_bytes, dz, nullptr, dgamma,
                          dbeta, beta_acc, conv_dbias, B, HW, C, stream, 6.0f);
}

extern "C" int cvl_bn_backward_relu_sums(const void* dy, const void* z, const float* mean_rstd, const float* gamma,
                                         const float* beta, uint64_t* sums, void* dz, float* dgamma,
                                         float* dbeta, float beta_acc, float* conv_dbias, float act_hi, int B,
                                         int HW, int C, cvl_stream_t stream) {
  CVL_CHECK_ARG(dy && z && mean_rstd && gamma && beta && sums && dz && dgamma && dbeta && C % 8 == 0);
  CVL_CHECK_ARG(B > 0 && HW > 0);
  const int dst = acc_decode_launch((acc_u64*)sums, 2L * B * C, S_);
  if (dst) return dst;
  const int rpb = bn1_rows_per_blk(B, HW, C);
  const int nchunk = (HW + rpb - 1) / rpb;
  hipLaunchKernelGGL((bn_bwd_kernel<1, 2>), dim3(nchunk, B + 1), dim3(NT), 0, S_, (const cvl_bf16*)dy, (const cvl_bf16*)nullptr,
                     (const cvl_bf16*)z, mean_rstd, gamma, (const acc_u64*)sums, (cvl_bf16*)dz, (cvl_bf16*)nullptr, (float*)nullptr,
                     C, HW, rpb, 1, 0.f, BnPG{dgamma, dbeta, conv_dbias, beta_acc, nullptr, g_acc_slots}, beta, act_hi);
  return cvl_launch_status();
}

extern "C" int cvl_bn_backward_res_sums(const void* dy, const void* y, const void* z, const float* mean_rstd,
                                        const float* gamma, uint64_t* sums, void* dz, void* g_out,
                                        float* dgamma, float* dbeta, float beta_acc, float* conv_dbias, int B,
                                        int HW, int C, cvl_stream_t stream) {
  CVL_CHECK_ARG(dy && y && z && mean_rstd && gamma && sums && dz && dgamma && dbeta && C % 8 == 0);
  CVL_CHECK_ARG(B > 0 && HW > 0);
  const int dst = acc_decode_launch((acc_u64*)sums, 2L * B * C, S_);
  if (dst) return dst;
  const int rpb = bn1_rows_per_blk(B, HW, C);
  const int nchunk = (HW + rpb - 1) / rpb;
  hipLaunchKernelGGL((bn_bwd_kernel<1, 1>), dim3(nchunk, B + 1), dim3(NT), 0, S_, (const cvl_bf16*)dy, (const cvl_bf16*)y,
                     (const cvl_bf16*)z, mean_rstd, gamma, (const acc_u64*)sums, (cvl_bf16*)dz, (cvl_bf16*)g_out, (float*)nullptr,
                     C, HW, rpb, 1, 0.f, BnPG{dgamma, dbeta, conv_dbias, beta_acc, nullptr, g_acc_slots}, (const float*)nullptr, INFINITY);
  return cvl_launch_status();
}

extern "C" size_t cvl_bn_backward_res_sums_sc_workspace_size(int B, int HW, int C) {
  if (B <= 0 || HW <= 0 || C <= 0) return 0;
  const int rpb = bn1_rows_per_blk(B, HW, C);
  return sizeof(float) * 2 * (size_t)B * ((HW + rpb - 1) / rpb) * C;
}

extern "C" int cvl_bn_backward_res_sums_sc(const void* dy, const void* y, const void* z, const float* mean_rstd,
                                           const float* gamma, uint64_t* sums, void* dz, void* g_out,
                                           float* dgamma, float* dbeta, float beta_acc, float* conv_dbias,
                                           const void* z_sc, const float* mean_rstd_sc, void* workspace,
                                           size_t workspace_bytes, uint64_t* sc_sums, int B, int HW, int C,
                                           cvl_stream_t stream) {
  CVL_CHECK_ARG(dy && y && z && mean_rstd && gamma && sums && dz && g_out && dgamma && dbeta && C % 8 == 0);
  CVL_CHECK_ARG(z_sc && mean_rstd_sc && workspace && sc_sums && B > 0 && HW > 0);
  CVL_CHECK_ARG(workspace_bytes >= cvl_bn_backward_res_sums_sc_workspace_size(B, HW, C));
  const int dst = acc_decode_launch((acc_u64*)sums, 2L * B * C, S_);
  if (dst) return dst;
  const int rpb = bn1_rows_per_blk(B, HW, C);
  const int nchunk = (HW + rpb - 1) / rpb;
  float* part = reinterpret_cast<float*>(workspace);
  BnPG pg{dgamma, dbeta, conv_dbias, beta_acc, nullptr, g_acc_slots};
  pg.sc_z = (const cvl_bf16*)z_sc;
  pg.sc_mr = mean_rstd_sc;
  hipLaunchKernelGGL((bn_bwd_kernel<1, 1, true>), dim3(nchunk, B + 1), dim3(NT), 0, S_, (const cvl_bf16*)dy,
                     (const cvl_bf16*)y, (const cvl_bf16*)z, mean_rstd, gamma, (const acc_u64*)sums, (cvl_bf16*)dz,
                     (cvl_bf16*)g_out, part, C, HW, rpb, 1, 0.f, pg, (const float*)nullptr, INFINITY);
  hipLaunchKernelGGL(bn_colsum_kernel, dim3((C + 31) / 32, B), dim3(NT), 0, S_, (const float*)part, nchunk, C,
                     (acc_u64*)sc_sums, 1);
  return cvl_launch_status();
}

extern "C" size_t cvl_bn_backward_sc_workspace_size(int B, int HW, int C) {
  if (B <= 0 || HW <= 0 || C <= 0) return 0;
  return cvl_bn_backward_workspace_size(B, HW, C) + cvl_bn_backward_res_sums_sc_workspace_size(B, HW, C);
}

extern "C" int cvl_bn_backward_sc(const void* dy, const void* y, const void* z, const float* mean_rstd,
                                  const float* gamma, void* workspace, size_t workspace_bytes, void* dz, void* g_out,
                                  float* dgamma, float* dbeta, float beta_acc, float* conv_dbias, const void* z_sc,
                                  const float* mean_rstd_sc, uint64_t* sc_sums, int B, int HW, int C,
                                  cvl_stream_t stream) {
  CVL_CHECK_ARG(dy && y && z && mean_rstd && gamma && workspace && dz && g_out && dgamma && dbeta && C % 8 == 0);
  CVL_CHECK_ARG(z_sc && mean_rstd_sc && sc_sums && B > 0 && HW > 0);
  CVL_CHECK_ARG(workspace_bytes >= cvl_bn_backward_sc_workspace_size(B, HW, C));
  const int rpb = bn_bwd_rows_per_blk(B, HW, C);
  const int nchunk = (HW + rpb - 1) / rpb;
  acc_u64* sums = reinterpret_cast<acc_u64*>(workspace);
  double* dbsum = reinterpret_cast<double*>(sums + 2 * (size_t)B * C);
  float* part0 = reinterpret_cast<float*>(dbsum + 2 * (size_t)C);
  float* part_sc = reinterpret_cast<float*>(reinterpret_cast<char*>(workspace) + cvl_bn_backward_workspace_size(B, HW, C));
  hipLaunchKernelGGL((bn_bwd_kernel<0, 1>), dim3(nchunk, B), dim3(NT), 0, S_, (const cvl_bf16*)dy, (const cvl_bf16*)y,
                     (const cvl_bf16*)z, mean_rstd, gamma, (const acc_u64*)nullptr, (cvl_bf16*)nullptr,
                     (cvl_bf16*)nullptr, part0, C, HW, rpb, 1, 0.f, BnPG{}, (const float*)nullptr, INFINITY);
  hipLaunchKernelGGL(bn_colsum_kernel, dim3((C + 31) / 32, B), dim3(NT), 0, S_, (const float*)part0, nchunk, C,
                     sums, 1);
  const int rpb1 = bn1_rows_per_blk(B, HW, C);
  const int nchunk1 = (HW + rpb1 - 1) / rpb1;
  BnPG pg{dgamma, dbeta, conv_dbias, beta_acc, nullptr, 1};
  pg.sc_z = (const cvl_bf16*)z_sc;
  pg.sc_mr = mean_rstd_sc;
  hipLaunchKernelGGL((bn_bwd_kernel<1, 1, true>), dim3(nchunk1, B + 1), dim3(NT), 0, S_, (const cvl_bf16*)dy,
                     (const cvl_bf16*)y, (const cvl_bf16*)z, mean_rstd, gamma, (const acc_u64*)sums, (cvl_bf16*)dz,
                     (cvl_bf16*)g_out, part_sc, C, HW, rpb1, 1, 0.f, pg, (const float*)nullptr, INFINITY);
  hipLaunchKernelGGL(bn_colsum_kernel, dim3((C + 31) / 32, B), dim3(NT), 0, S_, (const float*)part_sc, nchunk1, C,
                     (acc_u64*)sc_sums, 1);
  return cvl_launch_status();
}

extern "C" int cvl_bn_backward_sums(const void* dy, const void* z, const float* mean_rstd, const float* gamma,
                                    const uint64_t* sums, void* dz, float* dgamma, float* dbeta, float beta_acc,
                                    float* conv_dbias, int B, int HW, int C, cvl_stream_t stream) {
  CVL_CHECK_ARG(dy && z && mean_rstd && gamma && sums && dz && dgamma && dbeta && C % 8 == 0 && B > 0 && HW > 0);
  const int rpb = bn1_rows_per_blk(B, HW, C);
  const int nchunk = (HW + rpb - 1) / rpb;
  hipLaunchKernelGGL((bn_bwd_kernel<1, 3>), dim3(nchunk, B + 1), dim3(NT), 0, S_, (const cvl_bf16*)dy,
                     (const cvl_bf16*)nullptr, (const cvl_bf16*)z, mean_rstd, gamma, (const acc_u64*)sums, (cvl_bf16*)dz,
                     (cvl_bf16*)nullptr, (float*)nullptr, C, HW, rpb, 1, 0.f,
                     BnPG{dgamma, dbeta, conv_dbias, beta_acc, nullptr, 1}, (const float*)nullptr, INFINITY);
  return cvl_launch_status();
}

extern "C" int cvl_bn_relu_maxpool3x3s2(const void* z, const float* mean_rstd, const float* gamma, const float* beta,
                                        void* y, uint8_t* argmax, int B, int H, int W, int C, cvl_stream_t stream) {
  CVL_CHECK_ARG(z && mean_rstd && gamma && beta && y && argmax && C % 8 == 0 && B > 0);
  const int Ho = (H + 2 - 3) / 2 + 1, Wo = (W + 2 - 3) / 2 + 1;
  if (C == 64) {
    const long blocks = (long)B * ((Ho + PTY - 1) / PTY) * ((Wo + PTX - 1) / PTX);
    CVL_CHECK_ARG(blocks < (1l << 31));
    hipLaunchKernelGGL(bn_relu_maxpool64_kernel, dim3((unsigned)blocks), dim3(NT), 0, S_, (const cvl_bf16*)z,
                       mean_rstd, gamma, beta, (cvl_bf16*)y, argmax, H, W, Ho, Wo);
    return cvl_launch_status();
  }
  const long total = (long)B * Ho * Wo * (C / 8);
  hipLaunchKernelGGL(bn_relu_maxpool_kernel, dim3(grid_for(total)), dim3(NT), 0, S_, (const cvl_bf16*)z, mean_rstd,
                     gamma, beta, (cvl_bf16*)y, argmax, B, H, W, C, Ho, Wo);
  return cvl_launch_status();
}

extern "C" int cvl_maxpool3x3s2(const void* x, void* y, uint8_t* argmax, int B, int H, int W, int C,
                                cvl_stream_t stream) {
  CVL_CHECK_ARG(x && y && argmax && C % 8 == 0);
  const int Ho = (H + 2 - 3) / 2 + 1, Wo = (W + 2 - 3) / 2 + 1;
  const long total = (long)B * Ho * Wo * (C / 8);
  hipLaunchKernelGGL(maxpool_fwd_kernel, dim3(grid_for(total)), dim3(NT), 0, S_, (const cvl_bf16*)x,
                     (cvl_bf16*)y, argmax, B, H, W, C, Ho, Wo);
  return cvl_launch_status();
}

extern "C" int cvl_maxpool3x3s2_backward(const void* dy, const uint8_t* argmax, void* dx, int B, int H,
                                         int W, int C, cvl_stream_t stream) {
  CVL_CHECK_ARG(dy && dx && argmax && C % 8 == 0);
  const int Ho = (H + 2 - 3) / 2 + 1, Wo = (W + 2 - 3) / 2 + 1;
  if (C == 64) {
    const long blocks = (long)B * ((H + BTY - 1) / BTY) * ((W + BTX - 1) / BTX);
    CVL_CHECK_ARG(blocks < (1l << 31));
    hipLaunchKernelGGL(maxpool_bwd64_kernel<false>, dim3((unsigned)blocks), dim3(NT), 0, S_, (const cvl_bf16*)dy, argmax,
                       (cvl_bf16*)dx, H, W, Ho, Wo, PoolBn{});
    return cvl_launch_status();
  }
// ... 253 lines not shown
```

### cv-lite-object-detection_amd/cvlite/_lib.py

```python
import ctypes
import os

import torch

_HERE = os.path.dirname(os.path.abspath(__file__))
LIB_PATH = os.environ.get("CVL_LIB") or os.path.join(_HERE, "libcvlite_hip.so")


def dispatch(key, default=0):
    for tok in os.environ.get("CVL_DISPATCH", "").split(","):
        k, _, v = tok.strip().partition("=")
        if k == key:
            return int(v) if v else 1
    return default

c_int, c_float, c_size_t, c_void_p = ctypes.c_int, ctypes.c_float, ctypes.c_size_t, ctypes.c_void_p
P = c_void_p

SIGNATURES = {
    "cvl_version": (c_int, []),
    "cvl_fcos_assign": (c_int, [P, P, P, c_int, c_int, c_int, c_int, c_int, P, P, P, P, P]),
    "cvl_fcos_loss_workspace_size": (c_size_t, [c_int, c_int]),
    "cvl_fcos_loss": (c_int, [P, c_int, P, c_int, P, c_int, c_int, c_int, c_int, c_float, P,
                              P, c_int, c_int, P, c_int, c_int, P, c_size_t, P]),
    "cvl_fcos_loss_ex": (c_int, [P, c_int, P, c_int, P, c_int, c_int, c_int, c_int, c_float, c_float, c_float,
                                 c_float, P, P, c_int, c_int, P, c_int, c_int, P, c_size_t, P]),
    "cvl_fcos_decode": (c_int, [P, c_int, c_int, c_int, ctypes.c_double, P, P]),
    "cvl_fcos_v1_decode": (c_int, [P, c_int, c_int, c_int, c_float, c_float, P, P]),
    "cvl_conv_igemm_workspace_size": (c_size_t, [P]),
    "cvl_conv_igemm": (c_int, [P, P, P, P, P, c_size_t, P]),
    "cvl_conv_igemm_relu_mask": (c_int, [P, P, P, P, P, c_size_t, P]),
    "cvl_conv_igemm_last_kernel": (c_int, []),
    "cvl_conv_igemm_last_ktile": (c_int, []),
    "cvl_conv_igemm_plan": (c_int, [P, c_int, c_size_t, P, P]),
    "cvl_conv_kernel_name": (ctypes.c_char_p, [c_int]),
    "cvl_centernet_peak_decode_workspace_size": (ctypes.c_size_t, [c_int, c_int, c_int, c_int]),
    "cvl_centernet_peak_decode": (c_int, [P, c_int, c_int, c_int, c_int, c_int, c_float, c_float, c_int, P, P, P,
                                          ctypes.c_size_t, P]),
    "cvl_conv_igemm_dgrad_bnsum": (c_int, [P, P, P, P, P, P, P, c_float, P, P, P, ctypes.c_size_t, P]),
    "cvl_bn_backward_relu_sums": (c_int, [P, P, P, P, P, P, P, P, P, c_float, P, c_float, c_int, c_int, c_int, P]),
    "cvl_conv_igemm_dgrad_bnsum_res": (c_int, [P, P, P, P, P, P, P, P, P, P, P, ctypes.c_size_t, P]),
    "cvl_bn_backward_res_sums": (c_int, [P, P, P, P, P, P, P, P, P, P, c_float, P, c_int, c_int, c_int, P]),
    "cvl_bn_backward_res_sums_sc_workspace_size": (c_size_t, [c_int, c_int, c_int]),
    "cvl_bn_backward_res_sums_sc": (c_int, [P, P, P, P, P, P, P, P, P, P, c_float, P, P, P, P, c_size_t, P, c_int,
                                            c_int, c_int, P]),
    "cvl_bn_backward_sums": (c_int, [P, P, P, P, P, P, P, P, c_float, P, c_int, c_int, c_int, P]),
    "cvl_bn_backward_sc_workspace_size": (c_size_t, [c_int, c_int, c_int]),
    "cvl_bn_backward_sc": (c_int, [P, P, P, P, P, P, c_size_t, P, P, P, P, c_float, P, P, P, P, c_int, c_int, c_int, P]),
    "cvl_probe_arm": (c_int, [P]),
    "cvl_probe_clock_hz": (ctypes.c_double, []),
    "cvl_conv_wgrad_workspace_size": (c_size_t, [P]),
    "cvl_conv_wgrad": (c_int, [P, P, P, P, c_float, P, c_size_t, P]),
    "cvl_conv_wgrad_grouped_workspace_size": (c_size_t, [P, c_int]),
    "cvl_conv_wgrad_grouped": (c_int, [P, c_int, P, P, P, c_float, P, c_size_t, P]),
    "cvl_conv_wgrad_batch_workspace_size": (c_size_t, [P, c_int]),
    "cvl_conv_wgrad_batch": (c_int, [P, c_int, P, P, P, c_float, P, c_size_t, P]),
    "cvl_pack_conv_weights": (c_int, [P, c_int, c_int, c_int, c_int, c_int, c_int, P, c_int, c_int, P, P]),
    "cvl_pack_conv_weights_multi": (c_int, [P, P, c_int, P]),
    "cvl_im2col": (c_int, [P, c_int, c_int, c_int, c_int, c_int, c_int, c_int, c_int, c_int, c_int,
                           c_int, c_int, P, P]),
    "cvl_bn_finalize": (c_int, [P, P, P, P, c_int, c_int, c_int, c_float, c_float, P]),
    "cvl_bn_acc_decode": (c_int, [P, P, ctypes.c_int64, P]),
    "cvl_bn_set_exact": (c_int, [c_int]),
    "cvl_bn_acc_slots": (c_int, []),
    "cvl_stem_conv7x7s2": (c_int, [P, c_int, c_int, c_int, P, P, P, P, P]),
    "cvl_stem_wgrad_workspace_size": (c_size_t, [c_int, c_int, c_int]),
    "cvl_stem_wgrad": (c_int, [P, c_int, c_int, c_int, P, P, c_float, P, c_size_t, P]),
    "cvl_bn_apply": (c_int, [P, P, P, P, P, P, c_int, c_int, c_int, c_int, P]),
    "cvl_bn_finalize_apply": (c_int, [P, P, P, P, P, P, P, P, P, c_int, c_int, c_int, c_int, c_float, c_float, P]),
    "cvl_bn_finalize_apply_bnres": (c_int, [P, P, P, P, P, P, P, P, P, P, P, P, P, P, c_float, c_float, P, c_int,
                                            c_int, c_int, c_int, c_float, c_float, P]),
    "cvl_bn_backward_workspace_size": (c_size_t, [c_int, c_int, c_int]),
    "cvl_bn_backward": (c_int, [P, P, P, P, P, P, c_size_t, P, P, P, P, c_float, P, c_int, c_int, c_int, P]),
    "cvl_bn_backward_relu": (c_int, [P, P, P, P, P, P, c_size_t, P, P, P, c_float, P, c_int, c_int, c_int, P]),
    "cvl_maxpool3x3s2": (c_int, [P, P, P, c_int, c_int, c_int, c_int, P]),
    "cvl_bn_relu_maxpool3x3s2": (c_int, [P, P, P, P, P, P, c_int, c_int, c_int, c_int, P]),
    "cvl_maxpool3x3s2_backward": (c_int, [P, P, P, c_int, c_int, c_int, c_int, P]),
    "cvl_maxpool3x3s2_backward_bn_relu_workspace_size": (c_size_t, [c_int, c_int, c_int, c_int]),
    "cvl_maxpool3x3s2_backward_bn_relu": (c_int, [P, P, P, P, P, P, P, c_size_t, P, P, P, P, c_float, P, c_int, c_int,
                                                  c_int, c_int, P]),
    "cvl_upsample2x_add": (c_int, [P, P, P, c_int, c_int, c_int, c_int, P]),
    "cvl_upsample2x_backward": (c_int, [P, P, c_int, c_int, c_int, c_int, c_float, P]),
    "cvl_relu_backward": (c_int, [P, P, P, ctypes.c_long, c_float, P]),
    "cvl_add": (c_int, [P, P, P, ctypes.c_long, P]),
    "cvl_bias_grad_workspace_size": (c_size_t, [c_int, c_int, c_int]),
    "cvl_bias_grad_multi_workspace_size": (c_size_t, [P, c_int]),
    "cvl_bias_grad_multi": (c_int, [P, c_int, P, c_size_t, P]),
    "cvl_bias_grad": (c_int, [P, c_int, c_int, c_int, ctypes.c_int64, ctypes.c_int64, c_int, c_int, P, c_size_t,
# ... 52 lines not shown
                                     P, P]),
    "cvl_centernet_decode": (c_int, [P, c_int, c_int, c_int, c_int, ctypes.c_double, c_float, ctypes.c_double,
                                     ctypes.c_double, ctypes.c_double, ctypes.c_double, P, P, P]),
    "cvl_centernet_scale_decode": (c_int, [P, c_int, c_int, c_int, c_int, c_int, c_int, c_int, c_int, P, c_float,
                                           c_float, ctypes.c_double, ctypes.c_double, ctypes.c_double,
                                           ctypes.c_double, P, P, P]),
    "cvl_nms_workspace_size": (c_size_t, [c_int, c_int]),
    "cvl_nms": (c_int, [P, c_int, P, c_int, ctypes.c_double, P, P, P, P]),
    "cvl_soft_nms_workspace_size": (c_size_t, [c_int, c_int]),
    "cvl_soft_nms": (c_int, [P, c_int, P, c_int, ctypes.c_double, P, P, P, P, P]),
    "cvl_retina_corners": (c_int, [P, c_int, c_int, c_int, c_float, c_float, c_int, P, P]),
    "cvl_retina_decode_workspace_size": (c_size_t, [c_int, P, c_int]),
    "cvl_retina_decode": (c_int, [P, c_int, P, c_int, c_int, P, P, P, c_int, c_int, c_float, P, P, P, c_size_t,
                                  P]),
    "cvl_retina_nms_workspace_size": (c_size_t, [c_int, c_int]),
    "cvl_retina_nms": (c_int, [P, c_int, P, c_int, c_int, c_float, P, P, P, P]),
    "cvl_fcos_center_assign": (c_int, [P, P, P, c_int, c_int, c_int, c_int, c_int, P, P, c_int, P, P, P]),
    "cvl_fcos_center_v1_assign": (c_int, [P, P, P, c_int, c_int, c_int, c_int, c_int, P, P, P, P, P]),
    "cvl_resize_pad_normalize": (c_int, [P, c_int, c_int, c_int, c_int, c_int, c_int, c_int, c_int, c_int, P, P]),
    "cvl_image_augment_workspace_size": (c_size_t, [c_int, c_int]),
    "cvl_image_augment": (c_int, [P, P, P, P, P, P, c_int, c_int, c_int, c_int, P, c_size_t, P]),
    "cvl_fcos_detect_workspace_size": (c_size_t, [c_int, c_int, c_int, c_int]),
    "cvl_fcos_detect": (c_int, [P, c_int, P, c_int, c_int, P, P, c_int, c_int, c_float, c_float, c_int, c_int, P, P,
                                P, P, P, c_size_t, P]),
    "cvl_jpeg_info": (c_int, [P, c_size_t, P]),
    "cvl_jpeg_entropy_decode": (c_int, [P, c_size_t, P, c_size_t, P]),
    "cvl_jpeg_batch_sizes": (c_int, [P, c_int, P, P]),
    "cvl_jpeg_decode_batch": (c_int, [P, P, c_int, P, P, c_size_t, P, c_size_t, P, P]),
    "cvl_bn_apply_f32": (c_int, [P, P, P, P, P, P, c_int, c_int, c_int, c_int, P]),
    "cvl_bn_finalize_apply_f32": (c_int, [P, P, P, P, P, P, P, P, P, c_int, c_int, c_int, c_int, c_float, c_float,
                                          P]),
    "cvl_bn_backward_f32_workspace_size": (c_size_t, [c_int, c_int]),
    "cvl_bn_backward_f32": (c_int, [P, P, P, P, P, P, P, c_size_t, P, P, P, P, c_float, P, c_float, c_int, c_int,
                                    c_int, P]),
    "cvl_maxpool3x3s2_f32": (c_int, [P, P, P, c_int, c_int, c_int, c_int, P]),
    "cvl_maxpool3x3s2_backward_f32": (c_int, [P, P, P, c_int, c_int, c_int, c_int, P]),
    "cvl_upsample2x_add_f32": (c_int, [P, P, P, c_int, c_int, c_int, c_int, P]),
    "cvl_upsample2x_backward_f32": (c_int, [P, P, c_int, c_int, c_int, c_int, c_float, P]),
    "cvl_relu_backward_f32": (c_int, [P, P, P, ctypes.c_long, c_float, P]),
    "cvl_add_f32": (c_int, [P, P, P, ctypes.c_long, P]),
    "cvl_bias_grad_multi_f32": (c_int, [P, c_int, P]),
    "cvl_retina_loss_f32": (c_int, [P, c_int, P, c_int, P, c_int, P, c_int, c_int, P, c_float, P, P, c_int, P, c_int,
                                    P, P]),
}


class CvlError(RuntimeError):
    pass


_lib = None


NEWER = {"cvl_conv_igemm_last_ktile", "cvl_conv_igemm_plan"}


def load():
    global _lib
    if _lib is None:
        if not os.path.exists(LIB_PATH):
            raise CvlError("cvlite native library not built (%s): run __graft_entry__.build() or "
                           "make -C cv-lite-object-detection_amd/csrc" % LIB_PATH)
        lib = ctypes.CDLL(LIB_PATH)
        for name, (res, args) in SIGNATURES.items():
            if name in NEWER and os.environ.get("CVL_LIB") and not hasattr(lib, name):
                continue
            fn = getattr(lib, name)
            fn.restype = res
            fn.argtypes = args
        _lib = lib
        if os.environ.get("CVL_BN_EXACT", "0") == "1":
            lib.cvl_bn_set_exact(1)
    return _lib


def call(name, *args):
    st = getattr(load(), name)(*args)
    if st != 0:
        if st >= 1000:
            raise CvlError("%s failed: hipError %d" % (name, st - 1000))
        raise CvlError("%s: invalid argument (status %d)" % (name, st))
    return True


def ptr(t):
    return None if t is None else c_void_p(t.data_ptr())


def stream():
    return c_void_p(torch.cuda.current_stream().cuda_stream)


def require_cuda(*tensors):
    if not torch.cuda.is_available():
        raise CvlError("cvlite ops need an MI355X GPU (no CPU fallback)")
    for t in tensors:
        if t is not None and not t.is_cuda:
            raise CvlError("cvlite ops take device tensors")
        if t is not None and not t.is_contiguous():
            raise CvlError("cvlite ops take contiguous tensors")
```

### cv-lite-object-detection_amd/cvlite/layers.py

```python
import math

import os

import torch

from . import ops_nn as nn
from . import _lib

BF16 = torch.bfloat16
F32 = torch.float32


def act_dtype(precision=None):
    p = (precision or os.environ.get("CVL_PRECISION", "bf16")).lower()
    if p not in ("bf16", "fp32"):
        raise ValueError("precision must be 'bf16' or 'fp32'")
    return F32 if p == "fp32" else BF16


def glorot_uniform(fan_in, fan_out):
    lim = math.sqrt(6.0 / (fan_in + fan_out))

    def init(gen, shape):
        return (torch.rand(shape, generator=gen, dtype=torch.float64) * 2 - 1).mul_(lim).float()
# ... 145 lines not shown

    def dgrad_desc(self, B, segs, ld_dst=None, beta=0.0):
        Ho, Wo = segs[0]["Hs"], segs[0]["Ws"]
        _, _, pt, pl = self.out_hw(segs[0]["Hr"], segs[0]["Wr"])
        return nn.make_desc(nn.DGRAD, B, self.cout_pad, self.k, self.k, self.stride, pt, pl, self.cin_pad,
                            self.cin, self.cin if ld_dst is None else ld_dst, segs, beta=beta)

    def fwd(self, x, B, H, W, out=None, stats=None, relu_out=False, relu_in=False):
        Ho, Wo, _, _ = self.out_hw(H, W)
        if out is None:
            out = torch.empty((B, Ho, Wo, self.cout), dtype=x.dtype, device=x.device)
        d = self.fwd_desc(B, [nn.seg(Ho, Wo, H, W, self.wf, self.bias_arg())], ld_dst=self.cout,
                          relu_out=relu_out, relu_in=relu_in)
        nn.conv_igemm(d, x, out, stats)
        return out, Ho, Wo

    def wgrad(self, x, dy, B, H, W, relu_in=False, dw=None, beta=0.0, bias=True):
        Ho, Wo, _, _ = self.out_hw(H, W)
        d = self.fwd_desc(B, [nn.seg(Ho, Wo, H, W, self.wf, None)], ld_dst=self.cout_pad_ld(dy),
                          relu_in=relu_in)
        if _wgb is not None and self.k in (1, 3) and beta == 0.0 and not relu_in and x.dtype == BF16:
            _wgb.append((d, x, dy, self.dw if dw is None else dw))
        else:
            nn.conv_wgrad(d, x, dy, self.dw if dw is None else dw, beta)
        if self.has_bias and bias:
            nn.bias_grad(dy, self.cout_pad_ld(dy), 0, self.cout, 0, Ho * Wo, Ho * Wo, B, self.db)

    def cout_pad_ld(self, dy):
        return int(dy.shape[-1])

    def dgrad(self, dy, B, H, W, out=None, beta=0.0, bn_next=None):
        Ho, Wo, _, _ = self.out_hw(H, W)
        if out is None:
            out = torch.empty((B, H, W, self.cin), dtype=dy.dtype, device=dy.device)
        d = self.dgrad_desc(B, [nn.seg(H, W, Ho, Wo, self.wd)], ld_dst=self.cin, beta=beta)
        if bn_next is None:
            nn.conv_igemm(d, dy, out)
            return out
        z, mr, ga, be, sums = bn_next[:5]
        y = bn_next[5] if len(bn_next) > 5 else None
        zero = sums is None
        if zero:
            sums = nn.bn_acc(B, self.cin, dy.device, zero=False)
        if y is not None:
            fused = nn.conv_igemm_dgrad_bnsum_res(d, dy, out, y, z, mr, ga, be, sums, zero=zero)
        else:
            fused = nn.conv_igemm_dgrad_bnsum(d, dy, out, z, mr, ga, be, sums, zero=zero)
        return out, (sums if fused else None)


FUSE_BNSUM = not _lib.dispatch("no_bnsum_fuse")
FUSE_BNSUM_RES = FUSE_BNSUM and not _lib.dispatch("no_bnsum_res")
FUSE_SC_BNSUM = FUSE_BNSUM_RES and not _lib.dispatch("no_sc_bnsum")

WGRAD_BATCH = not _lib.dispatch("no_wgrad_batch")
_wgb = None


class wgrad_batch(object):
    def __enter__(self):
        global _wgb
        self.own = _wgb is None and WGRAD_BATCH
        if self.own:
            _wgb = []
        return self

    def __exit__(self, exc_type, *exc):
        global _wgb
        if self.own:
            try:
                if exc_type is None:
                    flush_wgrad_batch()
            finally:
                _wgb = None
        return False


def conv_wgrad(d, x, dy, dw):
    if _wgb is not None and x.dtype == BF16:
        _wgb.append((d, x, dy, dw))
    else:
        nn.conv_wgrad(d, x, dy, dw)


def flush_wgrad_batch():
    if _wgb:
        items = list(_wgb)
        del _wgb[:]
        nn.conv_wgrad_batch([i[0] for i in items], [i[1] for i in items], [i[2] for i in items],
                            [i[3] for i in items])


class StatsArena(object):

    def __init__(self, n_stats, device):
        self.slots = nn.acc_slots()
        self.buf = torch.zeros(n_stats * self.slots, dtype=torch.int64, device=device)
        self.off = 0

    def take(self, B, c):
        n = B * c * 2 * self.slots
        assert self.off + n <= self.buf.numel(), "stats arena too small"
        v = self.buf[self.off:self.off + n].view(B, c, 2, self.slots)
        self.off += n
        return v


class BatchNorm(object):

    def __init__(self, store, name, c, eps=1.001e-5, momentum=0.99):
        self.name, self.c, self.eps, self.momentum = name, c, eps, momentum
        self.gname = store.add(name + "/gamma", (c,), constant(1.0))
        self.bname = store.add(name + "/beta", (c,), constant(0.0))
        self.store = store
        self.run_mean = self.run_var = None

    def init_buffers(self, device):
        self.run_mean = torch.zeros(self.c, dtype=torch.float32, device=device)
        self.run_var = torch.ones(self.c, dtype=torch.float32, device=device)

    def moving_mean_rstd(self, B):
        mr = torch.empty((B, self.c, 2), dtype=torch.float32, device=self.run_mean.device)
        mr[:, :, 0] = self.run_mean
        mr[:, :, 1] = torch.rsqrt(self.run_var + self.eps)
        return mr

    def normalize(self, z, stats, B, HW, relu, residual=None, train=True, residual_bn=None):
        y = torch.empty_like(z)
        if train and residual_bn is not None:
            rz, rstats, rmr, rbn = residual_bn
            mr = torch.empty((B, self.c, 2), dtype=torch.float32, device=z.device)
            nn.bn_finalize_apply_bnres(stats, mr, self.run_mean, self.run_var, z, self.gamma, self.beta, rstats, rmr,
                                       rbn.run_mean, rbn.run_var, rz, rbn.gamma, rbn.beta, rbn.eps, rbn.momentum, y,
                                       B, HW, self.c, relu, self.eps, self.momentum)
        elif train:
            mr = torch.empty((B, self.c, 2), dtype=torch.float32, device=z.device)
            nn.bn_finalize_apply(stats, mr, self.run_mean, self.run_var, z, self.gamma, self.beta, residual, y, B,
                                 HW, self.c, relu, self.eps, self.momentum)
        else:
            mr = self.moving_mean_rstd(B)
            nn.bn_apply(z, mr, self.gamma, self.beta, residual, y, B, HW, self.c, relu)
        return y, mr

    @property
    def gamma(self):
        return self.store.p(self.gname)

    @property
    def beta(self):
        return self.store.p(self.bname)


class ConvBN(object):

    def __init__(self, store, name, k, cin, cout, stride=1, pad="same", dgrad=True, cin_k=None,
                 bn_name=None):
        self.conv = Conv(store, name + "_conv" if bn_name is None else name, k, cin, cout, stride, pad,
                         bias=True, dgrad=dgrad, cin_k=cin_k)
        self.bn = BatchNorm(store, (name + "_bn") if bn_name is None else bn_name, cout)

    def forward(self, x, B, H, W, relu=True, residual=None, train=True, arena=None, defer=False,
                residual_bn=None):
        c = self.conv.cout
        Ho, Wo, _, _ = self.conv.out_hw(H, W)
        stats = None
        if train:
            stats = arena.take(B, c) if arena is not None else nn.bn_acc(B, c, x.device)
        z, _, _ = self.conv.fwd(x, B, H, W, stats=stats)
        if defer:
            assert train and residual is None and not relu, "defer: the projection shortcut's BN only"
            mr = torch.empty((B, c, 2), dtype=torch.float32, device=z.device)
            return (z, stats, mr, self.bn), (x, z, None, mr, B, H, W, Ho, Wo, relu, False)
        y, mr = self.bn.normalize(z, stats, B, Ho * Wo, relu, residual=residual, train=train,
                                  residual_bn=residual_bn)
        return y, (x, z, y, mr, B, H, W, Ho, Wo, relu, residual is not None or residual_bn is not None)

    def bn_next_ctx(self, saved, arena=None):
        x, z, y, mr, B, H, W, Ho, Wo, relu, has_res = saved
        if not relu or has_res or not FUSE_BNSUM or z.dtype != BF16:
            return None
        return (z, mr, self.bn.gamma, self.bn.beta, arena.take(B, self.bn.c) if arena is not None else None)
# ... 51 lines not shown
```

### cv-lite-object-detection_amd/cvlite/ops_nn.py

```python
import ctypes

import torch

from . import _lib
from ._lib import ptr, stream

c_int, c_int64, c_float, c_void_p = ctypes.c_int, ctypes.c_int64, ctypes.c_float, ctypes.c_void_p
BF16 = torch.bfloat16
FWD, DGRAD = 0, 1
MAX_SEG = 10


class ConvSeg(ctypes.Structure):
    _fields_ = [("Hr", c_int), ("Wr", c_int), ("Hs", c_int), ("Ws", c_int),
                ("src_base", c_int64), ("src_img", c_int64), ("dst_base", c_int64), ("dst_img", c_int64),
                ("w", c_void_p), ("bias", c_void_p)]


class ConvDesc(ctypes.Structure):
    _fields_ = [("mode", c_int), ("B", c_int), ("Cin", c_int), ("KH", c_int), ("KW", c_int),
                ("stride", c_int), ("pad_t", c_int), ("pad_l", c_int), ("Npad", c_int),
                ("n_store", c_int), ("ld_dst", c_int), ("dst_coff", c_int), ("dst_f32", c_int),
                ("relu_out", c_int), ("relu_in", c_int), ("beta", c_float), ("nseg", c_int),
                ("seg", ConvSeg * MAX_SEG), ("prec", c_int)]
# ... 221 lines not shown


def bn_acc(B, C, device, zero=True):
    f = torch.zeros if zero else torch.empty
    return f((B, C, 2, acc_slots()), dtype=torch.int64, device=device)


def bn_acc_value(acc):
    acc = acc.contiguous()
    out = torch.empty(acc.shape[:-1], dtype=torch.float64, device=acc.device)
    _lib.call("cvl_bn_acc_decode", acc_ptr(acc), ptr(out), out.numel(), stream())
    return out


def _acc_add_f32(bins, f):
    u = f.contiguous().view(torch.int32).to(torch.int64) & 0xffffffff
    e = (u >> 23) & 0xff
    r = e - ACC_E0
    k = torch.div(r.clamp(min=0), ACC_W, rounding_mode="floor")
    bad = (e == 255) | ((e != 0) & (r >= 0) & (k >= ACC_BINS))
    ok = (e != 0) & (r >= 0) & (k < ACC_BINS)
    m = ((u & 0x7fffff) | 0x800000) << (r - k * ACC_W).clamp(min=0)
    v = torch.where((u >> 31) == 1, -m, m)
    bins.scatter_add_(-1, torch.where(ok, k, 0).unsqueeze(-1), torch.where(ok, v, 0).unsqueeze(-1))
    bins[..., ACC_BINS] += bad.to(torch.int64)


def bn_acc_encode(values, exact=None):
    v = values.to(torch.float64)
    if exact is None:
        exact = acc_slots() == ACC_SLOTS
    if not exact:
        return v.contiguous().view(torch.int64).unsqueeze(-1).clone()
    out = torch.zeros(v.shape + (ACC_SLOTS,), dtype=torch.int64, device=v.device)
    hi = v.to(torch.float32)
    r = v - hi.double()
    mid = r.to(torch.float32)
    lo = (r - mid.double()).to(torch.float32)
    for piece in (hi, mid, lo):
        _acc_add_f32(out, piece)
    return out


def bn_finalize(stats, mean_rstd, run_mean, run_var, B, C, HW, eps, momentum):
    _lib.call("cvl_bn_finalize", acc_ptr(stats), ptr(mean_rstd), ptr(run_mean), ptr(run_var), B, C, HW,
              float(eps), float(momentum), stream())


def bn_apply(z, mean_rstd, gamma, beta, residual, y, B, HW, C, relu):
    _lib.call("cvl_bn_apply_f32" if _is_f32(z) else "cvl_bn_apply", ptr(z), ptr(mean_rstd), ptr(gamma), ptr(beta), ptr(residual), ptr(y),
              B, HW, C, int(relu), stream())


def bn_finalize_apply(stats, mean_rstd, run_mean, run_var, z, gamma, beta, residual, y, B, HW, C, relu, eps,
                      momentum):
    _lib.call("cvl_bn_finalize_apply_f32" if _is_f32(z) else "cvl_bn_finalize_apply", acc_ptr(stats), ptr(mean_rstd), ptr(run_mean), ptr(run_var), ptr(z), ptr(gamma),
              ptr(beta), ptr(residual), ptr(y), B, HW, C, int(relu), float(eps), float(momentum), stream())


def bn_finalize_apply_bnres(stats, mean_rstd, run_mean, run_var, z, gamma, beta, res_stats, res_mean_rstd,
                            res_run_mean, res_run_var, res_z, res_gamma, res_beta, res_eps, res_momentum, y, B,
                            HW, C, relu, eps, momentum):
    _lib.call("cvl_bn_finalize_apply_bnres", acc_ptr(stats), ptr(mean_rstd), ptr(run_mean), ptr(run_var), ptr(z),
              ptr(gamma), ptr(beta), acc_ptr(res_stats), ptr(res_mean_rstd), ptr(res_run_mean), ptr(res_run_var),
              ptr(res_z), ptr(res_gamma), ptr(res_beta), float(res_eps), float(res_momentum), ptr(y), B, HW, C,
              int(relu), float(eps), float(momentum), stream())


def bn_backward(dy, y_relu, z, mean_rstd, gamma, dz, g_out, dgamma, dbeta, B, HW, C, beta_acc=0.0,
                conv_dbias=None):
    if _is_f32(dy):
        return bn_backward_f32(dy, y_relu, z, mean_rstd, gamma, None, dz, g_out, dgamma, dbeta, B, HW, C, beta_acc,
                               conv_dbias)
    n = int(_lib.load().cvl_bn_backward_workspace_size(B, HW, C))
    ws = torch.empty(n, dtype=torch.uint8, device=dy.device)
    _lib.call("cvl_bn_backward", ptr(dy), ptr(y_relu), ptr(z), ptr(mean_rstd), ptr(gamma), ptr(ws), n,
              ptr(dz), ptr(g_out), ptr(dgamma), ptr(dbeta), float(beta_acc), ptr(conv_dbias), B, HW, C,
              stream())


def bn_backward_f32(dy, y_relu, z, mean_rstd, gamma, bn_beta, dz, g_out, dgamma, dbeta, B, HW, C, beta_acc=0.0,
                    conv_dbias=None, act_hi=float("inf")):
    n = int(_lib.load().cvl_bn_backward_f32_workspace_size(B, C))
    ws = torch.empty(n, dtype=torch.uint8, device=dy.device)
    _lib.call("cvl_bn_backward_f32", ptr(dy), ptr(y_relu), ptr(z), ptr(mean_rstd), ptr(gamma), ptr(bn_beta), ptr(ws), n,
              ptr(dz), ptr(g_out), ptr(dgamma), ptr(dbeta), float(beta_acc), ptr(conv_dbias), float(act_hi), B, HW, C,
              stream())


def bn_backward_relu6(dy, z, mean_rstd, gamma, beta, dz, dgamma, dbeta, B, HW, C, beta_acc=0.0, conv_dbias=None):
    n = int(_lib.load().cvl_bn_backward_workspace_size(B, HW, C))
    ws = torch.empty(n, dtype=torch.uint8, device=dy.device)
    _lib.call("cvl_bn_backward_relu6", ptr(dy), ptr(z), ptr(mean_rstd), ptr(gamma), ptr(beta), ptr(ws), n, ptr(dz),
              ptr(dgamma), ptr(dbeta), float(beta_acc), ptr(conv_dbias), B, HW, C, stream())


def _dw_shapes(x, Ho, Wo):
    B, H, W, C = x.shape
    return B, H, W, C, Ho, Wo


def depthwise_fwd(x, w, y, k, stride, pad_t, pad_l):
    B, H, W, C = x.shape
    Ho, Wo = y.shape[1], y.shape[2]
    _lib.call("cvl_depthwise_fwd", ptr(x), ptr(w), ptr(y), B, H, W, C, int(k), int(stride), int(pad_t), int(pad_l),
              Ho, Wo, stream())


def depthwise_dgrad(dy, w, dx, k, stride, pad_t, pad_l, beta=0.0):
    B, H, W, C = dx.shape
    Ho, Wo = dy.shape[1], dy.shape[2]
    _lib.call("cvl_depthwise_dgrad", ptr(dy), ptr(w), ptr(dx), B, H, W, C, int(k), int(stride), int(pad_t),
              int(pad_l), Ho, Wo, float(beta), stream())


def depthwise_wgrad(x, dy, dw, k, stride, pad_t, pad_l, beta=0.0):
    B, H, W, C = x.shape
    Ho, Wo = dy.shape[1], dy.shape[2]
    n = int(_lib.load().cvl_depthwise_wgrad_workspace_size(B, Ho, Wo, C, int(k)))
    ws = torch.empty(max(n, 16), dtype=torch.uint8, device=x.device)
    _lib.call("cvl_depthwise_wgrad", ptr(x), ptr(dy), ptr(dw), float(beta), B, H, W, C, int(k), int(stride),
              int(pad_t), int(pad_l), Ho, Wo, ptr(ws), ws.numel(), stream())


def conv_igemm_dgrad_bnsum(desc, src, dst, z, mean_rstd, gamma, beta, sums, act_hi=float("inf"), zero=True):
    _prec(desc, src)
    n = int(_lib.load().cvl_conv_igemm_workspace_size(ctypes.byref(desc)))
    ws = torch.empty(n, dtype=torch.uint8, device=src.device) if n > 16 else None
    if zero:
        sums.zero_()
    flag = ctypes.c_int32(0)
    _lib.call("cvl_conv_igemm_dgrad_bnsum", ctypes.byref(desc), ptr(src), ptr(dst), ptr(z), ptr(mean_rstd), ptr(gamma),
              ptr(beta), float(act_hi), acc_ptr(sums), ctypes.addressof(flag), ptr(ws), n if ws is not None else 0,
              stream())
    return bool(flag.value)


def conv_igemm_dgrad_bnsum_res(desc, src, dst, y, z, mean_rstd, gamma, beta, sums, zero=True):
    _prec(desc, src)
    n = int(_lib.load().cvl_conv_igemm_workspace_size(ctypes.byref(desc)))
    ws = torch.empty(n, dtype=torch.uint8, device=src.device) if n > 16 else None
    if zero:
        sums.zero_()
    flag = ctypes.c_int32(0)
    _lib.call("cvl_conv_igemm_dgrad_bnsum_res", ctypes.byref(desc), ptr(src), ptr(dst), ptr(y), ptr(z),
              ptr(mean_rstd), ptr(gamma), ptr(beta), acc_ptr(sums), ctypes.addressof(flag), ptr(ws),
              n if ws is not None else 0, stream())
    return bool(flag.value)


def bn_backward_res_sums(dy, y, z, mean_rstd, gamma, sums, dz, g_out, dgamma, dbeta, B, HW, C, beta_acc=0.0,
                         conv_dbias=None):
    _lib.call("cvl_bn_backward_res_sums", ptr(dy), ptr(y), ptr(z), ptr(mean_rstd), ptr(gamma), acc_ptr(sums), ptr(dz),
              ptr(g_out), ptr(dgamma), ptr(dbeta), float(beta_acc), ptr(conv_dbias), B, HW, C, stream())


def bn_backward_res_sums_sc(dy, y, z, mean_rstd, gamma, sums, dz, g_out, dgamma, dbeta, z_sc, mean_rstd_sc, sc_sums,
                            B, HW, C, beta_acc=0.0, conv_dbias=None):
    n = int(_lib.load().cvl_bn_backward_res_sums_sc_workspace_size(B, HW, C))
    ws = torch.empty(n, dtype=torch.uint8, device=dy.device)
    _lib.call("cvl_bn_backward_res_sums_sc", ptr(dy), ptr(y), ptr(z), ptr(mean_rstd), ptr(gamma), acc_ptr(sums),
              ptr(dz), ptr(g_out), ptr(dgamma), ptr(dbeta), float(beta_acc), ptr(conv_dbias), ptr(z_sc),
              ptr(mean_rstd_sc), ptr(ws), n, ptr(sc_sums), B, HW, C, stream())


def bn_backward_sc(dy, y, z, mean_rstd, gamma, dz, g_out, dgamma, dbeta, z_sc, mean_rstd_sc, sc_sums, B, HW, C,
                   beta_acc=0.0, conv_dbias=None):
    n = int(_lib.load().cvl_bn_backward_sc_workspace_size(B, HW, C))
    ws = torch.empty(n, dtype=torch.uint8, device=dy.device)
    _lib.call("cvl_bn_backward_sc", ptr(dy), ptr(y), ptr(z), ptr(mean_rstd), ptr(gamma), ptr(ws), n, ptr(dz),
              ptr(g_out), ptr(dgamma), ptr(dbeta), float(beta_acc), ptr(conv_dbias), ptr(z_sc), ptr(mean_rstd_sc),
              ptr(sc_sums), B, HW, C, stream())


def bn_backward_sums(dy, z, mean_rstd, gamma, sums, dz, dgamma, dbeta, B, HW, C, beta_acc=0.0, conv_dbias=None):
    _lib.call("cvl_bn_backward_sums", ptr(dy), ptr(z), ptr(mean_rstd), ptr(gamma), ptr(sums), ptr(dz), ptr(dgamma),
              ptr(dbeta), float(beta_acc), ptr(conv_dbias), B, HW, C, stream())


def bn_backward_relu_sums(dy, z, mean_rstd, gamma, beta, sums, dz, dgamma, dbeta, B, HW, C, beta_acc=0.0,
                          conv_dbias=None, act_hi=float("inf")):
    _lib.call("cvl_bn_backward_relu_sums", ptr(dy), ptr(z), ptr(mean_rstd), ptr(gamma), ptr(beta), acc_ptr(sums), ptr(dz),
              ptr(dgamma), ptr(dbeta), float(beta_acc), ptr(conv_dbias), float(act_hi), B, HW, C, stream())


def bn_backward_relu(dy, z, mean_rstd, gamma, beta, dz, dgamma, dbeta, B, HW, C, beta_acc=0.0, conv_dbias=None):
    if _is_f32(dy):
        return bn_backward_f32(dy, None, z, mean_rstd, gamma, beta, dz, None, dgamma, dbeta, B, HW, C, beta_acc,
                               conv_dbias)
    n = int(_lib.load().cvl_bn_backward_workspace_size(B, HW, C))
    ws = torch.empty(n, dtype=torch.uint8, device=dy.device)
    _lib.call("cvl_bn_backward_relu", ptr(dy), ptr(z), ptr(mean_rstd), ptr(gamma), ptr(beta), ptr(ws), n, ptr(dz),
              ptr(dgamma), ptr(dbeta), float(beta_acc), ptr(conv_dbias), B, HW, C, stream())


def bn_relu_maxpool3x3s2(z, mean_rstd, gamma, beta, y, argmax):
    B, H, W, C = z.shape
    _lib.call("cvl_bn_relu_maxpool3x3s2", ptr(z), ptr(mean_rstd), ptr(gamma), ptr(beta), ptr(y), ptr(argmax), B, H,
              W, C, stream())


def maxpool3x3s2(x, y, argmax):
    B, H, W, C = x.shape
    _lib.call("cvl_maxpool3x3s2_f32" if _is_f32(x) else "cvl_maxpool3x3s2", ptr(x), ptr(y), ptr(argmax), B, H, W, C, stream())


def maxpool3x3s2_backward(dy, argmax, dx):
    B, H, W, C = dx.shape
    _lib.call("cvl_maxpool3x3s2_backward_f32" if _is_f32(dy) else "cvl_maxpool3x3s2_backward", ptr(dy), ptr(argmax), ptr(dx), B, H, W, C, stream())


def maxpool3x3s2_backward_bn_relu(dp, argmax, z, mean_rstd, gamma, beta, dy, dz, dgamma, dbeta, beta_acc=0.0,
                                  conv_dbias=None):
    B, H, W, C = z.shape
    n = int(_lib.load().cvl_maxpool3x3s2_backward_bn_relu_workspace_size(B, H, W, C))
    ws = torch.empty(n, dtype=torch.uint8, device=z.device)
    _lib.call("cvl_maxpool3x3s2_backward_bn_relu", ptr(dp), ptr(argmax), ptr(z), ptr(mean_rstd), ptr(gamma),
              ptr(beta), ptr(ws), n, ptr(dy), ptr(dz), ptr(dgamma), ptr(dbeta), float(beta_acc), ptr(conv_dbias),
              B, H, W, C, stream())


def upsample2x_add(a, b, out, B, H, W, C):
    _lib.call("cvl_upsample2x_add_f32" if _is_f32(a) else "cvl_upsample2x_add", ptr(a), ptr(b), ptr(out), B, H, W, C, stream())
# ... 232 lines not shown
```

### include/cvlite.h

```cpp
#ifndef CVLITE_H_
#define CVLITE_H_

#include <stddef.h>
#include <stdint.h>

#ifdef __cplusplus
extern "C" {
#endif

typedef void* cvl_stream_t;

enum { CVL_OK = 0, CVL_EINVAL = 1, CVL_EHIP = 1000 };

int cvl_version(void);

int cvl_fcos_assign(const float* boxes, const int32_t* nbox, const float* img_dim, int B, int n_max,
                    int pad_h, int pad_w, int num_classes, const int32_t* strides ,
                    const float* size_bounds , float* targets, int32_t* num_targets,
                    cvl_stream_t stream);

size_t cvl_fcos_loss_workspace_size(int B, int P);
int cvl_fcos_loss(const float* reg_pred, int ld_reg, const float* cls_pred, int ld_cls,
                  const float* targets, int B, int P, int num_classes, int reg_type,
                  float grad_scale, float* losses, void* d_reg, int ld_dreg, int dreg_dtype,
// ... 108 lines not shown
               int pad_l, int Ho, int Wo, int Kp, void* out, cvl_stream_t stream);

int cvl_bn_finalize(uint64_t* stats, float* mean_rstd, float* run_mean, float* run_var, int B,
                    int C, int HW, float eps, float momentum, cvl_stream_t stream);
int cvl_bn_apply(const void* z, const float* mean_rstd, const float* gamma, const float* beta,
                 const void* residual, void* y, int B, int HW, int C, int relu, cvl_stream_t stream);
int cvl_bn_finalize_apply(uint64_t* stats, float* mean_rstd, float* run_mean, float* run_var,
                          const void* z, const float* gamma, const float* beta, const void* residual, void* y,
                          int B, int HW, int C, int relu, float eps, float momentum, cvl_stream_t stream);
int cvl_bn_finalize_apply_bnres(uint64_t* stats, float* mean_rstd, float* run_mean, float* run_var,
                                const void* z, const float* gamma, const float* beta, uint64_t* res_stats,
                                float* res_mean_rstd, float* res_run_mean, float* res_run_var,
                                const void* res_z, const float* res_gamma, const float* res_beta,
                                float res_eps, float res_momentum, void* y, int B, int HW, int C, int relu,
                                float eps, float momentum, cvl_stream_t stream);
size_t cvl_bn_backward_workspace_size(int B, int HW, int C);
int cvl_bn_backward(const void* dy, const void* y_relu, const void* z, const float* mean_rstd,
                    const float* gamma, void* workspace, size_t workspace_bytes, void* dz, void* g_out,
                    float* dgamma, float* dbeta, float beta_acc, float* conv_dbias, int B, int HW, int C,
                    cvl_stream_t stream);
int cvl_bn_backward_relu(const void* dy, const void* z, const float* mean_rstd, const float* gamma,
                         const float* beta, void* workspace, size_t workspace_bytes, void* dz, float* dgamma,
                         float* dbeta, float beta_acc, float* conv_dbias, int B, int HW, int C,
                         cvl_stream_t stream);
int cvl_conv_igemm_dgrad_bnsum(const cvl_conv_desc* d, const void* src, void* dst, const void* z,
                               const float* mean_rstd, const float* gamma, const float* beta, float act_hi,
                               uint64_t* sums, int32_t* fused, void* workspace, size_t workspace_bytes,
                               cvl_stream_t stream);
int cvl_bn_backward_relu_sums(const void* dy, const void* z, const float* mean_rstd, const float* gamma,
                              const float* beta, uint64_t* sums, void* dz, float* dgamma, float* dbeta,
                              float beta_acc, float* conv_dbias, float act_hi, int B, int HW, int C,
                              cvl_stream_t stream);
int cvl_conv_igemm_dgrad_bnsum_res(const cvl_conv_desc* d, const void* src, void* dst, const void* y, const void* z,
                                   const float* mean_rstd, const float* gamma, const float* beta, uint64_t* sums,
                                   int32_t* fused, void* workspace, size_t workspace_bytes, cvl_stream_t stream);
int cvl_bn_backward_res_sums(const void* dy, const void* y, const void* z, const float* mean_rstd, const float* gamma,
                             uint64_t* sums, void* dz, void* g_out, float* dgamma, float* dbeta, float beta_acc,
                             float* conv_dbias, int B, int HW, int C, cvl_stream_t stream);
size_t cvl_bn_backward_res_sums_sc_workspace_size(int B, int HW, int C);
int cvl_bn_backward_res_sums_sc(const void* dy, const void* y, const void* z, const float* mean_rstd,
                                const float* gamma, uint64_t* sums, void* dz, void* g_out, float* dgamma,
                                float* dbeta, float beta_acc, float* conv_dbias, const void* z_sc,
                                const float* mean_rstd_sc, void* workspace, size_t workspace_bytes,
                                uint64_t* sc_sums, int B, int HW, int C, cvl_stream_t stream);
size_t cvl_bn_backward_sc_workspace_size(int B, int HW, int C);
int cvl_bn_backward_sc(const void* dy, const void* y, const void* z, const float* mean_rstd, const float* gamma,
                       void* workspace, size_t workspace_bytes, void* dz, void* g_out, float* dgamma, float* dbeta,
                       float beta_acc, float* conv_dbias, const void* z_sc, const float* mean_rstd_sc,
                       uint64_t* sc_sums, int B, int HW, int C, cvl_stream_t stream);
int cvl_bn_backward_sums(const void* dy, const void* z, const float* mean_rstd, const float* gamma,
                         const uint64_t* sums, void* dz, float* dgamma, float* dbeta, float beta_acc,
                         float* conv_dbias, int B, int HW, int C, cvl_stream_t stream);

int cvl_bn_backward_relu6(const void* dy, const void* z, const float* mean_rstd, const float* gamma,
                          const float* beta, void* workspace, size_t workspace_bytes, void* dz, float* dgamma,
                          float* dbeta, float beta_acc, float* conv_dbias, int B, int HW, int C, cvl_stream_t stream);

int cvl_bn_relu_maxpool3x3s2(const void* z, const float* mean_rstd, const float* gamma, const float* beta, void* y,
                             uint8_t* argmax, int B, int H, int W, int C, cvl_stream_t stream);
int cvl_maxpool3x3s2(const void* x, void* y, uint8_t* argmax, int B, int H, int W, int C,
                     cvl_stream_t stream);
int cvl_maxpool3x3s2_backward(const void* dy, const uint8_t* argmax, void* dx, int B, int H, int W,
                              int C, cvl_stream_t stream);
size_t cvl_maxpool3x3s2_backward_bn_relu_workspace_size(int B, int H, int W, int C);
int cvl_maxpool3x3s2_backward_bn_relu(const void* dp, const uint8_t* argmax, const void* z, const float* mean_rstd,
                                      const float* gamma, const float* beta, void* workspace,
                                      size_t workspace_bytes, void* dy, void* dz, float* dgamma, float* dbeta,
                                      float beta_acc, float* conv_dbias, int B, int H, int W, int C,
                                      cvl_stream_t stream);
int cvl_upsample2x_add(const void* a, const void* b, void* out, int B, int H, int W, int C,
                       cvl_stream_t stream);
int cvl_upsample2x_backward(const void* dout, void* db, int B, int H, int W, int C, float beta,
                            cvl_stream_t stream);
int cvl_relu_backward(const void* dy, const void* y, void* dx, long n, float beta, cvl_stream_t stream);
int cvl_add(const void* a, const void* b, void* out, long n, cvl_stream_t stream);
size_t cvl_bias_grad_workspace_size(int ncol, int HW, int B);
int cvl_bias_grad(const void* dy, int ld, int coff, int ncol, int64_t base, int64_t img_stride, int HW,
                  int B, void* workspace, size_t workspace_bytes, float* db, float beta, cvl_stream_t stream);
#define CVL_BIAS_MAX_ITEMS 16
typedef struct {
  const void* dy;
  float* db;
  int64_t base, img_stride;
  int ld, coff, ncol, HW, B;
  float beta;
} cvl_bias_item;
size_t cvl_bias_grad_multi_workspace_size(const cvl_bias_item* items, int n);
int cvl_bias_grad_multi(const cvl_bias_item* items, int n, void* workspace, size_t workspace_bytes,
                        cvl_stream_t stream);

int cvl_bn_apply_f32(const float* z, const float* mean_rstd, const float* gamma, const float* beta,
                     const float* residual, float* y, int B, int HW, int C, int relu, cvl_stream_t stream);
int cvl_bn_finalize_apply_f32(uint64_t* stats, float* mean_rstd, float* run_mean, float* run_var,
                              const float* z, const float* gamma, const float* beta, const float* residual,
                              float* y, int B, int HW, int C, int relu, float eps, float momentum,
                              cvl_stream_t stream);
size_t cvl_bn_backward_f32_workspace_size(int B, int C);
int cvl_bn_backward_f32(const float* dy, const float* y_relu, const float* z, const float* mean_rstd,
                        const float* gamma, const float* bn_beta, void* workspace, size_t workspace_bytes,
                        float* dz, float* g_out, float* dgamma, float* dbeta, float beta_acc,
                        float* conv_dbias, float act_hi, int B, int HW, int C, cvl_stream_t stream);
int cvl_maxpool3x3s2_f32(const float* x, float* y, uint8_t* argmax, int B, int H, int W, int C,
                         cvl_stream_t stream);
int cvl_maxpool3x3s2_backward_f32(const float* dy, const uint8_t* argmax, float* dx, int B, int H, int W,
                                  int C, cvl_stream_t stream);
int cvl_upsample2x_add_f32(const float* a, const float* b, float* out, int B, int H, int W, int C,
// ... 207 lines not shown
```

Before: 1427 images/s.

## Store ReLU masks as packed bits and use them in BN backward and dgrad

The BN-apply kernels in the forward pass now also write a 1-bit-per-element ReLU mask beside the bf16 output. The BN backward kernels and the fused dgrad+BN-sum conv kernel read these bits instead of reloading the full bf16 activation y to rebuild the ReLU gate. This cuts backward memory traffic per gated element from 2 bytes to 1 bit. In exchange the forward pass does an extra byte-store per 8 channels, and the new code adds more kernel variants and alignment constraints.

```diff
diff --git a/cv-lite-object-detection_amd/csrc/conv_common.h b/cv-lite-object-detection_amd/csrc/conv_common.h
--- a/cv-lite-object-detection_amd/csrc/conv_common.h
+++ b/cv-lite-object-detection_amd/csrc/conv_common.h
@@ -69,6 +69,7 @@
   acc_u64* bsum;
   float bhi;
   const cvl_bf16* by;
+  const uint8_t* bbits;
   unsigned long long* probe;
   const cvl_bf16* ymask;
 };
@@ -108,9 +109,10 @@
   acc_u64* sums;
   float hi;
   const cvl_bf16* y;
-};
-
-enum { CVL_BSUM_NONE = 0, CVL_BSUM_Z = 1, CVL_BSUM_Y = 2 };
+  const uint8_t* bits;
+};
+
+enum { CVL_BSUM_NONE = 0, CVL_BSUM_Z = 1, CVL_BSUM_Y = 2, CVL_BSUM_BITS = 3 };
 struct ConvCallOpts {
   bool bn_stats;
   int bsum;
@@ -189,6 +191,7 @@
   a->dbg = 0;
   a->bz = nullptr; a->bmr = nullptr; a->bga = nullptr; a->bbe = nullptr; a->bsum = nullptr; a->bhi = 0.f;
   a->by = nullptr;
+  a->bbits = nullptr;
   a->probe = nullptr;
   a->ymask = nullptr;
   a->acc_slots = cvl_bn_acc_slots();
diff --git a/cv-lite-object-detection_amd/csrc/conv_dispatch.hip b/cv-lite-object-detection_amd/csrc/conv_dispatch.hip
--- a/cv-lite-object-detection_amd/csrc/conv_dispatch.hip
+++ b/cv-lite-object-detection_amd/csrc/conv_dispatch.hip
@@ -131,7 +131,8 @@
 
 bool p_fits(const cvl_conv_desc* d, const ConvArgs& a, const ConvCallOpts& o) {
   if (d->KH != 1 || d->KW != 1 || d->pad_t || d->pad_l || a.relu_in || a.nseg != 1 || a.K % 32) return false;
-  const bool by = o.bsum == CVL_BSUM_Y;
+  const bool by = o.bsum == CVL_BSUM_Y || o.bsum == CVL_BSUM_BITS;
+  if (o.bsum == CVL_BSUM_BITS && (a.ld_dst % 8 || a.dst_coff % 8)) return false;
   if (o.bsum && ((d->mode != CVL_CONV_DGRAD && a.dst_up == 1) || a.dst_f32 || (a.beta != 0.f) != by ||
                  (a.dst_up != 1 && !by) || o.bn_stats || (a.seg[0].Hr * a.seg[0].Wr) % BM ||
                  (a.dst_up == 1 && a.seg[0].dst_img != (long)a.seg[0].Hr * a.seg[0].Wr) || a.Npad % 64))
@@ -217,9 +218,12 @@
 
 bool plan_large(const cvl_conv_desc* d, const ConvArgs& a, const ConvCallOpts& o, ConvPlan* p) {
   if (cvl_dispatch_flag("no_l")) return false;
-  const bool bs = o.bsum != CVL_BSUM_NONE, by = o.bsum == CVL_BSUM_Y;
-  if (bs && (d->mode != CVL_CONV_DGRAD || d->dst_f32 || (d->beta != 0.f && !by) || a.dst_up != 1 || o.bn_stats))
-    return false;
+  const bool bs = o.bsum != CVL_BSUM_NONE, by = o.bsum == CVL_BSUM_Y || o.bsum == CVL_BSUM_BITS;
+  const bool scat = by && a.dst_up != 1 && d->KH == 1 && d->KW == 1 && d->mode == CVL_CONV_FWD;
+  if (bs && !scat &&
+      (d->mode != CVL_CONV_DGRAD || d->dst_f32 || (d->beta != 0.f && !by) || a.dst_up != 1 || o.bn_stats))
+    return false;
+  if (scat && (d->dst_f32 || o.bn_stats)) return false;
   if (by && (d->KH != 1 || d->KW != 1)) return false;
   if (d->Npad == 32 && d->KH == 3 && d->KW == 3 && d->mode == CVL_CONV_FWD && d->dst_f32 && !o.bn_stats &&
       !bs && a.dst_up == 1 && d->Cin % 32 == 0 && !d->relu_in && !cvl_dispatch_flag("no_h32"))
diff --git a/cv-lite-object-detection_amd/csrc/conv_igemm.hip b/cv-lite-object-detection_amd/csrc/conv_igemm.hip
--- a/cv-lite-object-detection_amd/csrc/conv_igemm.hip
+++ b/cv-lite-object-detection_amd/csrc/conv_igemm.hip
@@ -474,6 +474,7 @@
     const BnSumArgs& b = *io.bsum;
     a->bz = b.z; a->bmr = b.mr; a->bga = b.gamma; a->bbe = b.beta; a->bsum = b.sums; a->bhi = b.hi;
     a->by = b.y;
+    a->bbits = b.bits;
   }
   if (p.ymask) a->ymask = reinterpret_cast<const cvl_bf16*>(io.ymask);
   if (p.kernel == CVL_CK_X32) a->probe = reinterpret_cast<unsigned long long*>(cvl_probe_current(true));
@@ -589,6 +590,18 @@
 }
 
 namespace {
+int dgrad_bnsum_plan_form(const cvl_conv_desc* d, int offer, size_t ws, int32_t* form) {
+  *form = CVL_BSUM_NONE;
+  if (d->prec == CVL_PREC_F32) return CVL_OK;
+  for (int f = offer; f != CVL_BSUM_NONE; f = f == CVL_BSUM_BITS ? CVL_BSUM_Y : CVL_BSUM_NONE) {
+    ConvPlan p;
+    const int st = conv_plan(d, ConvCallOpts{false, f, false, ws}, &p);
+    if (st) return st;
+    if (p.kernel != CVL_CK_NONE) { *form = f; break; }
+  }
+  return CVL_OK;
+}
+
 int dgrad_bnsum_call(const cvl_conv_desc* d, const void* src, void* dst, int form, const BnSumArgs& b, int32_t* fused,
                      void* workspace, size_t workspace_bytes, cvl_stream_t stream) {
   *fused = 0;
@@ -614,7 +627,7 @@
                                           cvl_stream_t stream) {
   CVL_CHECK_ARG(d && fused && z && mean_rstd && gamma && beta && sums);
   const BnSumArgs b{reinterpret_cast<const cvl_bf16*>(z), mean_rstd, gamma, beta, reinterpret_cast<acc_u64*>(sums),
-                    act_hi, nullptr};
+                    act_hi, nullptr, nullptr};
   return dgrad_bnsum_call(d, src, dst, CVL_BSUM_Z, b, fused, workspace, workspace_bytes, stream);
 }
 
@@ -624,6 +637,39 @@
                                               size_t workspace_bytes, cvl_stream_t stream) {
   CVL_CHECK_ARG(d && fused && y && z && mean_rstd && gamma && beta && sums);
   const BnSumArgs b{reinterpret_cast<const cvl_bf16*>(z), mean_rstd, gamma, beta, reinterpret_cast<acc_u64*>(sums),
-                    INFINITY, reinterpret_cast<const cvl_bf16*>(y)};
+                    INFINITY, reinterpret_cast<const cvl_bf16*>(y), nullptr};
   return dgrad_bnsum_call(d, src, dst, CVL_BSUM_Y, b, fused, workspace, workspace_bytes, stream);
 }
+
+extern "C" int cvl_conv_igemm_dgrad_bnsum_res_bits(const cvl_conv_desc* d, const void* src, void* dst, const void* y,
+                                                   const uint8_t* relu_bits, const void* z, const float* mean_rstd,
+                                                   const float* gamma, const float* beta, uint64_t* sums,
+                                                   int32_t* fused, int32_t* form, void* workspace,
+                                                   size_t workspace_bytes, cvl_stream_t stream) {
+  CVL_CHECK_ARG(d && fused && y && relu_bits && z && mean_rstd && gamma && beta && sums);
+  const BnSumArgs b{reinterpret_cast<const cvl_bf16*>(z), mean_rstd, gamma, beta, reinterpret_cast<acc_u64*>(sums),
+                    INFINITY, reinterpret_cast<const cvl_bf16*>(y), relu_bits};
+  int32_t tmp = 0, *pf = form ? form : &tmp;
+  *pf = 0;
+  int st = dgrad_bnsum_plan_form(d, CVL_BSUM_BITS, workspace ? workspace_bytes : 0, pf);
+  if (st) return st;
+  st = dgrad_bnsum_call(d, src, dst, *pf ? *pf : CVL_BSUM_Y, b, fused, workspace, workspace_bytes, stream);
+  if (st || !*fused) *pf = 0;
+  return st;
+}
+
+extern "C" int cvl_conv_igemm_plan_bnsum(const cvl_conv_desc* d, int offer, size_t workspace_bytes, int32_t* form,
+                                         int32_t* kernel, int32_t* ktile) {
+  CVL_CHECK_ARG(d && form && kernel && ktile && offer >= CVL_BSUM_Z && offer <= CVL_BSUM_BITS);
+  *form = 0;
+  *kernel = CVL_CK_NONE;
+  *ktile = 0;
+  if (d->prec == CVL_PREC_F32) return CVL_OK;
+  int st = dgrad_bnsum_plan_form(d, offer, workspace_bytes, form);
+  if (st) return st;
+  ConvPlan p;
+  if ((st = conv_plan(d, ConvCallOpts{false, *form, false, workspace_bytes}, &p))) return st;
+  *kernel = p.kernel;
+  *ktile = conv_plan_ktile(p);
+  return CVL_OK;
+}
diff --git a/cv-lite-object-detection_amd/csrc/conv_igemm_p.hip b/cv-lite-object-detection_amd/csrc/conv_igemm_p.hip
--- a/cv-lite-object-detection_amd/csrc/conv_igemm_p.hip
+++ b/cv-lite-object-detection_amd/csrc/conv_igemm_p.hip
@@ -57,6 +57,12 @@
   return v;
 }
 __device__ __forceinline__ void pin16(s16x8& v) { asm volatile("" : "+v"(v)); }
+__device__ __forceinline__ unsigned gload1_untracked(const void* p) {
+  unsigned v;
+  asm volatile("global_load_ubyte %0, %1, off" : "=v"(v) : "v"(p) : "memory");
+  return v;
+}
+__device__ __forceinline__ void pin1(unsigned& v) { asm volatile("" : "+v"(v)); }
 
 template <int BN, int BK, bool RELU, bool F32, int BS = 0, bool ACC = false>
 __global__ void __launch_bounds__(NT) conv_igemm_p_kernel(ConvArgs a, int ntiles) {
@@ -183,6 +189,7 @@
   wait_vm<0>();
   s16x8 zv[BS ? TM : 1][NJP];
   s16x8 yv[BS == 2 ? TM : 1][BS == 2 ? NJP : 1];
+  unsigned bv[BS == 3 ? TM : 1][BS == 3 ? NJP : 1];
   s16x8 ov[ACC ? TM : 1][ACC ? TN / 2 : 1];
 
   float ss1[TN][4], ss2[TN][4];
@@ -266,6 +273,7 @@
         for (int jp = 0; jp < NJP; ++jp) {
           pin16(zv[i][jp]);
           if (BS == 2) pin16(yv[i][jp]);
+          if (BS == 3) pin1(bv[i][jp]);
         }
       const int img = m0 / HWr;
       if (img != bimg) {
@@ -358,6 +366,8 @@
             bool on;
             if (BS == 2) {
               on = bf16_to_f32((cvl_bf16)yv[i][j / 2][u]) > 0.f;
+            } else if (BS == 3) {
+              on = (bv[i][j / 2] >> u) & 1u;
             } else {
               const float af = __builtin_fmaf(bga[j / 2][u], xh, bbe[j / 2][u]);
               on = af > 0.f && af < a.bhi;
@@ -433,6 +443,8 @@
           zv[i][jp] = gload16_untracked(a.bz + row * a.ld_dst + a.dst_coff + n0 + wn * C::WN + jp * 32 + lgo);
           if (BS == 2)
             yv[i][jp] = gload16_untracked(a.by + row * a.ld_dst + a.dst_coff + n0 + wn * C::WN + jp * 32 + lgo);
+          if (BS == 3)
+            bv[i][jp] = gload1_untracked(a.bbits + ((row * a.ld_dst + a.dst_coff + n0 + wn * C::WN + jp * 32 + lgo) >> 3));
         }
     }
     const char* sl = lds + rslot * C::SLOT_B;
@@ -465,7 +477,9 @@
 void p_launch(const ConvPlan& p, const ConvArgs& a, hipStream_t s) {
   const dim3 grid(p.grid);
   const int ntiles = a.m_tiles * (a.Npad / p.bn);
-  if (p.bsum == CVL_BSUM_Y) {
+  if (p.bsum == CVL_BSUM_BITS) {
+    hipLaunchKernelGGL((conv_igemm_p_kernel<64, BK_, false, false, 3, true>), grid, dim3(NT), 0, s, a, ntiles);
+  } else if (p.bsum == CVL_BSUM_Y) {
     hipLaunchKernelGGL((conv_igemm_p_kernel<64, BK_, false, false, 2, true>), grid, dim3(NT), 0, s, a, ntiles);
   } else if (p.bsum) {
     hipLaunchKernelGGL((conv_igemm_p_kernel<64, BK_, false, false, 1>), grid, dim3(NT), 0, s, a, ntiles);
diff --git a/cv-lite-object-detection_amd/csrc/nn_ops.hip b/cv-lite-object-detection_amd/csrc/nn_ops.hip
--- a/cv-lite-object-detection_amd/csrc/nn_ops.hip
+++ b/cv-lite-object-detection_amd/csrc/nn_ops.hip
@@ -280,12 +280,12 @@
       bn_running(fin.stats, fin.slots, nimg, C, c, HW, fin.eps, fin.momentum, fin.run_mean, fin.run_var);
 }
 
-template <bool FIN, bool RBN = false>
+template <bool FIN, bool RBN = false, bool BITS = false>
 __global__ void __launch_bounds__(NT) bn_apply_kernel(const cvl_bf16* __restrict__ z, const float* __restrict__ mr,
                                                       const float* __restrict__ gamma, const float* __restrict__ beta,
                                                       const cvl_bf16* __restrict__ res, cvl_bf16* __restrict__ y,
                                                       int C, int HW, int relu, int rows_per_blk, BnFin fin,
-                                                      BnRes rb) {
+                                                      BnRes rb, uint8_t* __restrict__ bits) {
   static_assert(FIN || !RBN, "the BN residual form fuses both finalizes");
   const int b = FIN ? (int)blockIdx.y - 1 : (int)blockIdx.y;
   const int C8 = C / 8;
@@ -362,7 +362,16 @@
           if (relu == 2) o = fminf(o, 6.0f);
           v[u] = o;
         }
-        *reinterpret_cast<s16x8*>(y + off[q]) = pack8(v);
+        const s16x8 pv = pack8(v);
+        *reinterpret_cast<s16x8*>(y + off[q]) = pv;
+        if (BITS) {
+          float rv[8];
+          unpack8(pv, rv);
+          unsigned mk = 0;
+#pragma unroll
+          for (int u = 0; u < 8; ++u) mk |= (rv[u] > 0.f ? 1u : 0u) << u;
+          bits[off[q] >> 3] = (uint8_t)mk;
+        }
       }
     }
   }
@@ -448,6 +457,7 @@
     float m[8], rs[8], s1[8], s2[8], k1[8], k2[8], gm[8], ga[8], be[8];
     float msc[8], rssc[8];
     const bool use_y = PASS != 2 && (MASK == 0 ? y != nullptr : MASK == 1);
+    constexpr bool use_b = PASS != 2 && MASK == 4;
     const bool zmask = PASS != 2 && (MASK == 0 ? (!y && bnb) : MASK == 2);
 #pragma unroll
     for (int u = 0; u < 8; ++u) {
@@ -471,6 +481,7 @@
     if (rsub < rpp && act) {
       for (int r = r0 + rsub; r < r1; r += rpp * BN_UNR) {
         s16x8 vg[BN_UNR], vz[BN_UNR], vy[BN_UNR], vs[SC ? BN_UNR : 1];
+        unsigned vb[BN_UNR];
         long off[BN_UNR];
 #pragma unroll
         for (int q = 0; q < BN_UNR; ++q) {
@@ -479,6 +490,7 @@
           vg[q] = ld_rows(dy + off[q]);
           if (PASS != 2) vz[q] = ld_rows(z + off[q]);
           if (use_y) vy[q] = ld_rows(y + off[q]);
+          if (use_b) vb[q] = reinterpret_cast<const uint8_t*>(y)[off[q] >> 3];
           if (SC) vs[q] = ld_rows(pg.sc_z + off[q]);
         }
 #pragma unroll
@@ -499,6 +511,9 @@
             unpack8(vy[q], yy);
 #pragma unroll
             for (int u = 0; u < 8; ++u) g[u] = (yy[u] > 0.f && yy[u] < act_hi) ? g[u] : 0.f;
+          } else if (use_b) {
+#pragma unroll
+            for (int u = 0; u < 8; ++u) g[u] = ((vb[q] >> u) & 1u) ? g[u] : 0.f;
           } else if (zmask) {
 #pragma unroll
             for (int u = 0; u < 8; ++u) {
@@ -1439,32 +1454,50 @@
   const int rpb = bn_rows_per_blk(B, HW, C);
   hipLaunchKernelGGL(bn_apply_kernel<false>, dim3((HW + rpb - 1) / rpb, B), dim3(NT), 0, S_, (const cvl_bf16*)z,
                      mean_rstd, gamma, beta, (const cvl_bf16*)residual, (cvl_bf16*)y, C, HW, relu, rpb,
-                     BnFin{nullptr, nullptr, nullptr, nullptr, 0.f, 0.f, 1}, BnRes{});
-  return cvl_launch_status();
-}
-
-extern "C" int cvl_bn_finalize_apply(uint64_t* stats, float* mean_rstd, float* run_mean, float* run_var,
-                                     const void* z, const float* gamma, const float* beta, const void* residual,
-                                     void* y, int B, int HW, int C, int relu, float eps, float momentum,
-                                     cvl_stream_t stream) {
+                     BnFin{nullptr, nullptr, nullptr, nullptr, 0.f, 0.f, 1}, BnRes{}, (uint8_t*)nullptr);
+  return cvl_launch_status();
+}
+
+static int bn_finalize_apply_impl(uint64_t* stats, float* mean_rstd, float* run_mean, float* run_var,
+                                  const void* z, const float* gamma, const float* beta, const void* residual,
+                                  void* y, uint8_t* bits, int B, int HW, int C, int relu, float eps, float momentum,
+                                  cvl_stream_t stream) {
   CVL_CHECK_ARG(stats && mean_rstd && z && gamma && beta && y && C % 8 == 0 && B > 0 && HW > 0);
   CVL_CHECK_ARG(C <= BN_FIN_MAXC);
   CVL_CHECK_ARG((run_mean == nullptr) == (run_var == nullptr));
   const int dst = acc_decode_launch((acc_u64*)stats, 2L * B * C, S_);
   if (dst) return dst;
   const int rpb = bn_rows_per_blk(B, HW, C);
-  hipLaunchKernelGGL(bn_apply_kernel<true>, dim3((HW + rpb - 1) / rpb, B + 1), dim3(NT), 0, S_, (const cvl_bf16*)z,
+  auto k = bits ? bn_apply_kernel<true, false, true> : bn_apply_kernel<true>;
+  hipLaunchKernelGGL(k, dim3((HW + rpb - 1) / rpb, B + 1), dim3(NT), 0, S_, (const cvl_bf16*)z,
                      (const float*)nullptr, gamma, beta, (const cvl_bf16*)residual, (cvl_bf16*)y, C, HW, relu, rpb,
-                     BnFin{(const acc_u64*)stats, mean_rstd, run_mean, run_var, eps, momentum, g_acc_slots}, BnRes{});
-  return cvl_launch_status();
-}
-
-extern "C" int cvl_bn_finalize_apply_bnres(uint64_t* stats, float* mean_rstd, float* run_mean, float* run_var,
-                                           const void* z, const float* gamma, const float* beta, uint64_t* res_stats,
-                                           float* res_mean_rstd, float* res_run_mean, float* res_run_var,
-                                           const void* res_z, const float* res_gamma, const float* res_beta,
-                                           float res_eps, float res_momentum, void* y, int B, int HW, int C, int relu,
-                                           float eps, float momentum, cvl_stream_t stream) {
+                     BnFin{(const acc_u64*)stats, mean_rstd, run_mean, run_var, eps, momentum, g_acc_slots}, BnRes{}, bits);
+  return cvl_launch_status();
+}
+
+extern "C" int cvl_bn_finalize_apply(uint64_t* stats, float* mean_rstd, float* run_mean, float* run_var,
+                                     const void* z, const float* gamma, const float* beta, const void* residual,
+                                     void* y, int B, int HW, int C, int relu, float eps, float momentum,
+                                     cvl_stream_t stream) {
+  return bn_finalize_apply_impl(stats, mean_rstd, run_mean, run_var, z, gamma, beta, residual, y, nullptr, B, HW, C,
+                                relu, eps, momentum, stream);
+}
+
+extern "C" int cvl_bn_finalize_apply_bits(uint64_t* stats, float* mean_rstd, float* run_mean, float* run_var,
+                                          const void* z, const float* gamma, const float* beta,
+                                          const void* residual, void* y, uint8_t* relu_bits, int B, int HW, int C,
+                                          int relu, float eps, float momentum, cvl_stream_t stream) {
+  CVL_CHECK_ARG(relu_bits && relu == 1);
+  return bn_finalize_apply_impl(stats, mean_rstd, run_mean, run_var, z, gamma, beta, residual, y, relu_bits, B, HW,
+                                C, relu, eps, momentum, stream);
+}
+
+static int bn_finalize_apply_bnres_impl(uint64_t* stats, float* mean_rstd, float* run_mean, float* run_var,
+                                        const void* z, const float* gamma, const float* beta, uint64_t* res_stats,
+                                        float* res_mean_rstd, float* res_run_mean, float* res_run_var,
+                                        const void* res_z, const float* res_gamma, const float* res_beta,
+                                        float res_eps, float res_momentum, void* y, uint8_t* bits, int B, int HW,
+                                        int C, int relu, float eps, float momentum, cvl_stream_t stream) {
   CVL_CHECK_ARG(stats && mean_rstd && z && gamma && beta && y && C % 8 == 0 && B > 0 && HW > 0);
   CVL_CHECK_ARG(res_stats && res_mean_rstd && res_z && res_gamma && res_beta);
   CVL_CHECK_ARG(C <= BN_FIN_MAXC);
@@ -1474,13 +1507,38 @@
   if (!dst) dst = acc_decode_launch((acc_u64*)res_stats, 2L * B * C, S_);
   if (dst) return dst;
   const int rpb = bn_rows_per_blk(B, HW, C);
-  hipLaunchKernelGGL((bn_apply_kernel<true, true>), dim3((HW + rpb - 1) / rpb, B + 1), dim3(NT), 0, S_, (const cvl_bf16*)z,
+  auto k = bits ? bn_apply_kernel<true, true, true> : bn_apply_kernel<true, true>;
+  hipLaunchKernelGGL(k, dim3((HW + rpb - 1) / rpb, B + 1), dim3(NT), 0, S_, (const cvl_bf16*)z,
                      (const float*)nullptr, gamma, beta, (const cvl_bf16*)nullptr, (cvl_bf16*)y, C, HW, relu, rpb,
                      BnFin{(const acc_u64*)stats, mean_rstd, run_mean, run_var, eps, momentum, g_acc_slots},
                      BnRes{(const cvl_bf16*)res_z, res_gamma, res_beta,
                            BnFin{(const acc_u64*)res_stats, res_mean_rstd, res_run_mean, res_run_var, res_eps,
-                                 res_momentum, g_acc_slots}});
-  return cvl_launch_status();
+                                 res_momentum, g_acc_slots}}, bits);
+  return cvl_launch_status();
+}
+
+extern "C" int cvl_bn_finalize_apply_bnres(uint64_t* stats, float* mean_rstd, float* run_mean, float* run_var,
+                                           const void* z, const float* gamma, const float* beta, uint64_t* res_stats,
+                                           float* res_mean_rstd, float* res_run_mean, float* res_run_var,
+                                           const void* res_z, const float* res_gamma, const float* res_beta,
+                                           float res_eps, float res_momentum, void* y, int B, int HW, int C, int relu,
+                                           float eps, float momentum, cvl_stream_t stream) {
+  return bn_finalize_apply_bnres_impl(stats, mean_rstd, run_mean, run_var, z, gamma, beta, res_stats, res_mean_rstd,
+                                      res_run_mean, res_run_var, res_z, res_gamma, res_beta, res_eps, res_momentum, y,
+                                      nullptr, B, HW, C, relu, eps, momentum, stream);
+}
+
+extern "C" int cvl_bn_finalize_apply_bnres_bits(uint64_t* stats, float* mean_rstd, float* run_mean, float* run_var,
+                                                const void* z, const float* gamma, const float* beta,
+                                                uint64_t* res_stats, float* res_mean_rstd, float* res_run_mean,
+                                                float* res_run_var, const void* res_z, const float* res_gamma,
+                                                const float* res_beta, float res_eps, float res_momentum, void* y,
+                                                uint8_t* relu_bits, int B, int HW, int C, int relu, float eps,
+                                                float momentum, cvl_stream_t stream) {
+  CVL_CHECK_ARG(relu_bits && relu == 1);
+  return bn_finalize_apply_bnres_impl(stats, mean_rstd, run_mean, run_var, z, gamma, beta, res_stats, res_mean_rstd,
+                                      res_run_mean, res_run_var, res_z, res_gamma, res_beta, res_eps, res_momentum, y,
+                                      relu_bits, B, HW, C, relu, eps, momentum, stream);
 }
 
 extern "C" size_t cvl_bn_backward_workspace_size(int B, int HW, int C) {
@@ -1494,7 +1552,8 @@
 static int bn_backward_impl(const void* dy, const void* y_relu, const float* bn_beta, const void* z,
                             const float* mean_rstd, const float* gamma, void* workspace, size_t workspace_bytes,
                             void* dz, void* g_out, float* dgamma, float* dbeta, float beta_acc, float* conv_dbias,
-                            int B, int HW, int C, cvl_stream_t stream, float act_hi = INFINITY) {
+                            int B, int HW, int C, cvl_stream_t stream, float act_hi = INFINITY,
+                            bool y_bits = false) {
   CVL_CHECK_ARG(dy && z && mean_rstd && gamma && workspace && dz && dgamma && dbeta && C % 8 == 0);
   CVL_CHECK_ARG(B > 0 && HW > 0);
   CVL_CHECK_ARG(workspace_bytes >= cvl_bn_backward_workspace_size(B, HW, C));
@@ -1505,8 +1564,8 @@
   float* part0 = reinterpret_cast<float*>(dbsum + 2 * (size_t)C);
   dim3 g1(nchunk, B);
   const bool ym = y_relu != nullptr, zm = !ym && bn_beta != nullptr;
-  auto k0 = ym ? bn_bwd_kernel<0, 1> : zm ? bn_bwd_kernel<0, 2> : bn_bwd_kernel<0, 3>;
-  auto k1 = ym ? bn_bwd_kernel<1, 1> : zm ? bn_bwd_kernel<1, 2> : bn_bwd_kernel<1, 3>;
+  auto k0 = ym ? (y_bits ? bn_bwd_kernel<0, 4> : bn_bwd_kernel<0, 1>) : zm ? bn_bwd_kernel<0, 2> : bn_bwd_kernel<0, 3>;
+  auto k1 = ym ? (y_bits ? bn_bwd_kernel<1, 4> : bn_bwd_kernel<1, 1>) : zm ? bn_bwd_kernel<1, 2> : bn_bwd_kernel<1, 3>;
   hipLaunchKernelGGL(k0, g1, dim3(NT), 0, S_, (const cvl_bf16*)dy, (const cvl_bf16*)y_relu,
                      (const cvl_bf16*)z, mean_rstd, gamma, (const acc_u64*)nullptr, (cvl_bf16*)nullptr,
                      (cvl_bf16*)nullptr, part0, C, HW, rpb, 1, 0.f, BnPG{}, bn_beta, act_hi);
@@ -1526,6 +1585,15 @@
                                int C, cvl_stream_t stream) {
   return bn_backward_impl(dy, y_relu, nullptr, z, mean_rstd, gamma, workspace, workspace_bytes, dz, g_out, dgamma,
                           dbeta, beta_acc, conv_dbias, B, HW, C, stream);
+}
+
+extern "C" int cvl_bn_backward_bits(const void* dy, const uint8_t* relu_bits, const void* z, const float* mean_rstd,
+                                    const float* gamma, void* workspace, size_t workspace_bytes, void* dz,
+                                    void* g_out, float* dgamma, float* dbeta, float beta_acc, float* conv_dbias,
+                                    int B, int HW, int C, cvl_stream_t stream) {
+  CVL_CHECK_ARG(relu_bits);
+  return bn_backward_impl(dy, relu_bits, nullptr, z, mean_rstd, gamma, workspace, workspace_bytes, dz, g_out, dgamma,
+                          dbeta, beta_acc, conv_dbias, B, HW, C, stream, INFINITY, true);
 }
 
 extern "C" int cvl_bn_backward_relu(const void* dy, const void* z, const float* mean_rstd, const float* gamma,
@@ -1562,20 +1630,37 @@
   return cvl_launch_status();
 }
 
-extern "C" int cvl_bn_backward_res_sums(const void* dy, const void* y, const void* z, const float* mean_rstd,
-                                        const float* gamma, uint64_t* sums, void* dz, void* g_out,
-                                        float* dgamma, float* dbeta, float beta_acc, float* conv_dbias, int B,
-                                        int HW, int C, cvl_stream_t stream) {
+static int bn_backward_res_sums_impl(const void* dy, const void* y, bool y_bits, const void* z,
+                                     const float* mean_rstd, const float* gamma, uint64_t* sums, void* dz,
+                                     void* g_out, float* dgamma, float* dbeta, float beta_acc, float* conv_dbias,
+                                     int B, int HW, int C, cvl_stream_t stream) {
   CVL_CHECK_ARG(dy && y && z && mean_rstd && gamma && sums && dz && dgamma && dbeta && C % 8 == 0);
   CVL_CHECK_ARG(B > 0 && HW > 0);
   const int dst = acc_decode_launch((acc_u64*)sums, 2L * B * C, S_);
   if (dst) return dst;
   const int rpb = bn1_rows_per_blk(B, HW, C);
   const int nchunk = (HW + rpb - 1) / rpb;
-  hipLaunchKernelGGL((bn_bwd_kernel<1, 1>), dim3(nchunk, B + 1), dim3(NT), 0, S_, (const cvl_bf16*)dy, (const cvl_bf16*)y,
+  auto k1 = y_bits ? bn_bwd_kernel<1, 4> : bn_bwd_kernel<1, 1>;
+  hipLaunchKernelGGL(k1, dim3(nchunk, B + 1), dim3(NT), 0, S_, (const cvl_bf16*)dy, (const cvl_bf16*)y,
                      (const cvl_bf16*)z, mean_rstd, gamma, (const acc_u64*)sums, (cvl_bf16*)dz, (cvl_bf16*)g_out, (float*)nullptr,
                      C, HW, rpb, 1, 0.f, BnPG{dgamma, dbeta, conv_dbias, beta_acc, nullptr, g_acc_slots}, (const float*)nullptr, INFINITY);
   return cvl_launch_status();
+}
+
+extern "C" int cvl_bn_backward_res_sums(const void* dy, const void* y, const void* z, const float* mean_rstd,
+                                        const float* gamma, uint64_t* sums, void* dz, void* g_out,
+                                        float* dgamma, float* dbeta, float beta_acc, float* conv_dbias, int B,
+                                        int HW, int C, cvl_stream_t stream) {
+  return bn_backward_res_sums_impl(dy, y, false, z, mean_rstd, gamma, sums, dz, g_out, dgamma, dbeta, beta_acc,
+                                   conv_dbias, B, HW, C, stream);
+}
+
+extern "C" int cvl_bn_backward_res_sums_bits(const void* dy, const uint8_t* relu_bits, const void* z,
+                                             const float* mean_rstd, const float* gamma, uint64_t* sums, void* dz,
+                                             void* g_out, float* dgamma, float* dbeta, float beta_acc,
+                                             float* conv_dbias, int B, int HW, int C, cvl_stream_t stream) {
+  return bn_backward_res_sums_impl(dy, relu_bits, true, z, mean_rstd, gamma, sums, dz, g_out, dgamma, dbeta, beta_acc,
+                                   conv_dbias, B, HW, C, stream);
 }
 
 extern "C" size_t cvl_bn_backward_res_sums_sc_workspace_size(int B, int HW, int C) {
@@ -1584,12 +1669,12 @@
   return sizeof(float) * 2 * (size_t)B * ((HW + rpb - 1) / rpb) * C;
 }
 
-extern "C" int cvl_bn_backward_res_sums_sc(const void* dy, const void* y, const void* z, const float* mean_rstd,
-                                           const float* gamma, uint64_t* sums, void* dz, void* g_out,
-                                           float* dgamma, float* dbeta, float beta_acc, float* conv_dbias,
-                                           const void* z_sc, const float* mean_rstd_sc, void* workspace,
-                                           size_t workspace_bytes, uint64_t* sc_sums, int B, int HW, int C,
-                                           cvl_stream_t stream) {
+static int bn_backward_res_sums_sc_impl(const void* dy, const void* y, bool y_bits, const void* z,
+                                        const float* mean_rstd, const float* gamma, uint64_t* sums, void* dz,
+                                        void* g_out, float* dgamma, float* dbeta, float beta_acc, float* conv_dbias,
+                                        const void* z_sc, const float* mean_rstd_sc, void* workspace,
+                                        size_t workspace_bytes, uint64_t* sc_sums, int B, int HW, int C,
+                                        cvl_stream_t stream) {
   CVL_CHECK_ARG(dy && y && z && mean_rstd && gamma && sums && dz && g_out && dgamma && dbeta && C % 8 == 0);
   CVL_CHECK_ARG(z_sc && mean_rstd_sc && workspace && sc_sums && B > 0 && HW > 0);
   CVL_CHECK_ARG(workspace_bytes >= cvl_bn_backward_res_sums_sc_workspace_size(B, HW, C));
@@ -1601,7 +1686,8 @@
   BnPG pg{dgamma, dbeta, conv_dbias, beta_acc, nullptr, g_acc_slots};
   pg.sc_z = (const cvl_bf16*)z_sc;
   pg.sc_mr = mean_rstd_sc;
-  hipLaunchKernelGGL((bn_bwd_kernel<1, 1, true>), dim3(nchunk, B + 1), dim3(NT), 0, S_, (const cvl_bf16*)dy,
+  auto k1 = y_bits ? bn_bwd_kernel<1, 4, true> : bn_bwd_kernel<1, 1, true>;
+  hipLaunchKernelGGL(k1, dim3(nchunk, B + 1), dim3(NT), 0, S_, (const cvl_bf16*)dy,
                      (const cvl_bf16*)y, (const cvl_bf16*)z, mean_rstd, gamma, (const acc_u64*)sums, (cvl_bf16*)dz,
                      (cvl_bf16*)g_out, part, C, HW, rpb, 1, 0.f, pg, (const float*)nullptr, INFINITY);
   hipLaunchKernelGGL(bn_colsum_kernel, dim3((C + 31) / 32, B), dim3(NT), 0, S_, (const float*)part, nchunk, C,
@@ -1609,16 +1695,38 @@
   return cvl_launch_status();
 }
 
+extern "C" int cvl_bn_backward_res_sums_sc(const void* dy, const void* y, const void* z, const float* mean_rstd,
+                                           const float* gamma, uint64_t* sums, void* dz, void* g_out,
+                                           float* dgamma, float* dbeta, float beta_acc, float* conv_dbias,
+                                           const void* z_sc, const float* mean_rstd_sc, void* workspace,
+                                           size_t workspace_bytes, uint64_t* sc_sums, int B, int HW, int C,
+                                           cvl_stream_t stream) {
+  return bn_backward_res_sums_sc_impl(dy, y, false, z, mean_rstd, gamma, sums, dz, g_out, dgamma, dbeta, beta_acc,
+                                      conv_dbias, z_sc, mean_rstd_sc, workspace, workspace_bytes, sc_sums, B, HW, C,
+                                      stream);
+}
+
+extern "C" int cvl_bn_backward_res_sums_sc_bits(const void* dy, const uint8_t* relu_bits, const void* z,
+                                                const float* mean_rstd, const float* gamma, uint64_t* sums, void* dz,
+                                                void* g_out, float* dgamma, float* dbeta, float beta_acc,
+                                                float* conv_dbias, const void* z_sc, const float* mean_rstd_sc,
+                                                void* workspace, size_t workspace_bytes, uint64_t* sc_sums, int B,
+                                                int HW, int C, cvl_stream_t stream) {
+  return bn_backward_res_sums_sc_impl(dy, relu_bits, true, z, mean_rstd, gamma, sums, dz, g_out, dgamma, dbeta,
+                                      beta_acc, conv_dbias, z_sc, mean_rstd_sc, workspace, workspace_bytes, sc_sums,
+                                      B, HW, C, stream);
+}
+
 extern "C" size_t cvl_bn_backward_sc_workspace_size(int B, int HW, int C) {
   if (B <= 0 || HW <= 0 || C <= 0) return 0;
   return cvl_bn_backward_workspace_size(B, HW, C) + cvl_bn_backward_res_sums_sc_workspace_size(B, HW, C);
 }
 
-extern "C" int cvl_bn_backward_sc(const void* dy, const void* y, const void* z, const float* mean_rstd,
-                                  const float* gamma, void* workspace, size_t workspace_bytes, void* dz, void* g_out,
-                                  float* dgamma, float* dbeta, float beta_acc, float* conv_dbias, const void* z_sc,
-                                  const float* mean_rstd_sc, uint64_t* sc_sums, int B, int HW, int C,
-                                  cvl_stream_t stream) {
+static int bn_backward_sc_impl(const void* dy, const void* y, bool y_bits, const void* z, const float* mean_rstd,
+                               const float* gamma, void* workspace, size_t workspace_bytes, void* dz, void* g_out,
+                               float* dgamma, float* dbeta, float beta_acc, float* conv_dbias, const void* z_sc,
+                               const float* mean_rstd_sc, uint64_t* sc_sums, int B, int HW, int C,
+                               cvl_stream_t stream) {
   CVL_CHECK_ARG(dy && y && z && mean_rstd && gamma && workspace && dz && g_out && dgamma && dbeta && C % 8 == 0);
   CVL_CHECK_ARG(z_sc && mean_rstd_sc && sc_sums && B > 0 && HW > 0);
   CVL_CHECK_ARG(workspace_bytes >= cvl_bn_backward_sc_workspace_size(B, HW, C));
@@ -1628,7 +1736,9 @@
   double* dbsum = reinterpret_cast<double*>(sums + 2 * (size_t)B * C);
   float* part0 = reinterpret_cast<float*>(dbsum + 2 * (size_t)C);
   float* part_sc = reinterpret_cast<float*>(reinterpret_cast<char*>(workspace) + cvl_bn_backward_workspace_size(B, HW, C));
-  hipLaunchKernelGGL((bn_bwd_kernel<0, 1>), dim3(nchunk, B), dim3(NT), 0, S_, (const cvl_bf16*)dy, (const cvl_bf16*)y,
+  auto k0 = y_bits ? bn_bwd_kernel<0, 4> : bn_bwd_kernel<0, 1>;
+  auto k1 = y_bits ? bn_bwd_kernel<1, 4, true> : bn_bwd_kernel<1, 1, true>;
+  hipLaunchKernelGGL(k0, dim3(nchunk, B), dim3(NT), 0, S_, (const cvl_bf16*)dy, (const cvl_bf16*)y,
                      (const cvl_bf16*)z, mean_rstd, gamma, (const acc_u64*)nullptr, (cvl_bf16*)nullptr,
                      (cvl_bf16*)nullptr, part0, C, HW, rpb, 1, 0.f, BnPG{}, (const float*)nullptr, INFINITY);
   hipLaunchKernelGGL(bn_colsum_kernel, dim3((C + 31) / 32, B), dim3(NT), 0, S_, (const float*)part0, nchunk, C,
@@ -1638,12 +1748,31 @@
   BnPG pg{dgamma, dbeta, conv_dbias, beta_acc, nullptr, 1};
   pg.sc_z = (const cvl_bf16*)z_sc;
   pg.sc_mr = mean_rstd_sc;
-  hipLaunchKernelGGL((bn_bwd_kernel<1, 1, true>), dim3(nchunk1, B + 1), dim3(NT), 0, S_, (const cvl_bf16*)dy,
+  hipLaunchKernelGGL(k1, dim3(nchunk1, B + 1), dim3(NT), 0, S_, (const cvl_bf16*)dy,
                      (const cvl_bf16*)y, (const cvl_bf16*)z, mean_rstd, gamma, (const acc_u64*)sums, (cvl_bf16*)dz,
                      (cvl_bf16*)g_out, part_sc, C, HW, rpb1, 1, 0.f, pg, (const float*)nullptr, INFINITY);
   hipLaunchKernelGGL(bn_colsum_kernel, dim3((C + 31) / 32, B), dim3(NT), 0, S_, (const float*)part_sc, nchunk1, C,
                      (acc_u64*)sc_sums, 1);
   return cvl_launch_status();
+}
+
+extern "C" int cvl_bn_backward_sc(const void* dy, const void* y, const void* z, const float* mean_rstd,
+                                  const float* gamma, void* workspace, size_t workspace_bytes, void* dz, void* g_out,
+                                  float* dgamma, float* dbeta, float beta_acc, float* conv_dbias, const void* z_sc,
+                                  const float* mean_rstd_sc, uint64_t* sc_sums, int B, int HW, int C,
+                                  cvl_stream_t stream) {
+  return bn_backward_sc_impl(dy, y, false, z, mean_rstd, gamma, workspace, workspace_bytes, dz, g_out, dgamma, dbeta,
+                             beta_acc, conv_dbias, z_sc, mean_rstd_sc, sc_sums, B, HW, C, stream);
+}
+
+extern "C" int cvl_bn_backward_sc_bits(const void* dy, const uint8_t* relu_bits, const void* z,
+                                       const float* mean_rstd, const float* gamma, void* workspace,
+                                       size_t workspace_bytes, void* dz, void* g_out, float* dgamma, float* dbeta,
+                                       float beta_acc, float* conv_dbias, const void* z_sc,
+                                       const float* mean_rstd_sc, uint64_t* sc_sums, int B, int HW, int C,
+                                       cvl_stream_t stream) {
+  return bn_backward_sc_impl(dy, relu_bits, true, z, mean_rstd, gamma, workspace, workspace_bytes, dz, g_out, dgamma,
+                             dbeta, beta_acc, conv_dbias, z_sc, mean_rstd_sc, sc_sums, B, HW, C, stream);
 }
 
 extern "C" int cvl_bn_backward_sums(const void* dy, const void* z, const float* mean_rstd, const float* gamma,
diff --git a/cv-lite-object-detection_amd/cvlite/_lib.py b/cv-lite-object-detection_amd/cvlite/_lib.py
--- a/cv-lite-object-detection_amd/cvlite/_lib.py
+++ b/cv-lite-object-detection_amd/cvlite/_lib.py
@@ -34,6 +34,18 @@
     "cvl_conv_igemm_last_ktile": (c_int, []),
     "cvl_conv_igemm_plan": (c_int, [P, c_int, c_size_t, P, P]),
     "cvl_conv_kernel_name": (ctypes.c_char_p, [c_int]),
+    "cvl_conv_igemm_plan_bnsum": (c_int, [P, c_int, c_size_t, P, P, P]),
+    "cvl_conv_igemm_dgrad_bnsum_res_bits": (c_int, [P, P, P, P, P, P, P, P, P, P, P, P, P, ctypes.c_size_t, P]),
+    "cvl_bn_finalize_apply_bits": (c_int, [P, P, P, P, P, P, P, P, P, P, c_int, c_int, c_int, c_int, c_float,
+                                           c_float, P]),
+    "cvl_bn_finalize_apply_bnres_bits": (c_int, [P, P, P, P, P, P, P, P, P, P, P, P, P, P, c_float, c_float, P, P,
+                                                 c_int, c_int, c_int, c_int, c_float, c_float, P]),
+    "cvl_bn_backward_bits": (c_int, [P, P, P, P, P, P, c_size_t, P, P, P, P, c_float, P, c_int, c_int, c_int, P]),
+    "cvl_bn_backward_res_sums_bits": (c_int, [P, P, P, P, P, P, P, P, P, P, c_float, P, c_int, c_int, c_int, P]),
+    "cvl_bn_backward_res_sums_sc_bits": (c_int, [P, P, P, P, P, P, P, P, P, P, c_float, P, P, P, P, c_size_t, P,
+                                                 c_int, c_int, c_int, P]),
+    "cvl_bn_backward_sc_bits": (c_int, [P, P, P, P, P, P, c_size_t, P, P, P, P, c_float, P, P, P, P, c_int, c_int,
+                                        c_int, P]),
     "cvl_centernet_peak_decode_workspace_size": (ctypes.c_size_t, [c_int, c_int, c_int, c_int]),
     "cvl_centernet_peak_decode": (c_int, [P, c_int, c_int, c_int, c_int, c_int, c_float, c_float, c_int, P, P, P,
                                           ctypes.c_size_t, P]),
@@ -192,7 +204,10 @@
 _lib = None
 
 
-NEWER = {"cvl_conv_igemm_last_ktile", "cvl_conv_igemm_plan"}
+NEWER = {"cvl_conv_igemm_last_ktile", "cvl_conv_igemm_plan", "cvl_conv_igemm_plan_bnsum",
+         "cvl_conv_igemm_dgrad_bnsum_res_bits", "cvl_bn_finalize_apply_bits", "cvl_bn_finalize_apply_bnres_bits",
+         "cvl_bn_backward_bits", "cvl_bn_backward_res_sums_bits", "cvl_bn_backward_res_sums_sc_bits",
+         "cvl_bn_backward_sc_bits"}
 
 
 def load():
diff --git a/cv-lite-object-detection_amd/cvlite/layers.py b/cv-lite-object-detection_amd/cvlite/layers.py
--- a/cv-lite-object-detection_amd/cvlite/layers.py
+++ b/cv-lite-object-detection_amd/cvlite/layers.py
@@ -221,6 +221,7 @@
 FUSE_BNSUM = not _lib.dispatch("no_bnsum_fuse")
 FUSE_BNSUM_RES = FUSE_BNSUM and not _lib.dispatch("no_bnsum_res")
 FUSE_SC_BNSUM = FUSE_BNSUM_RES and not _lib.dispatch("no_sc_bnsum")
+RELU_BITS = not _lib.dispatch("no_relu_bits")
 
 WGRAD_BATCH = not _lib.dispatch("no_wgrad_batch")
 _wgb = None
@@ -296,6 +297,8 @@
 
     def normalize(self, z, stats, B, HW, relu, residual=None, train=True, residual_bn=None):
         y = torch.empty_like(z)
+        if train and relu == 1 and RELU_BITS and (residual is not None or residual_bn is not None):
+            nn.attach_relu_bits(y)
         if train and residual_bn is not None:
             rz, rstats, rmr, rbn = residual_bn
             mr = torch.empty((B, self.c, 2), dtype=torch.float32, device=z.device)
diff --git a/cv-lite-object-detection_amd/cvlite/ops_nn.py b/cv-lite-object-detection_amd/cvlite/ops_nn.py
--- a/cv-lite-object-detection_amd/cvlite/ops_nn.py
+++ b/cv-lite-object-detection_amd/cvlite/ops_nn.py
@@ -297,8 +297,25 @@
               B, HW, C, int(relu), stream())
 
 
+def attach_relu_bits(y):
+    if y.dtype != torch.bfloat16 or y.shape[-1] % 8 or not hasattr(_lib.load(), "cvl_bn_finalize_apply_bits"):
+        return None
+    y._cvl_relu_bits = torch.empty(y.numel() // 8, dtype=torch.uint8, device=y.device)
+    return y._cvl_relu_bits
+
+
+def relu_bits(y):
+    return getattr(y, "_cvl_relu_bits", None) if y is not None else None
+
+
 def bn_finalize_apply(stats, mean_rstd, run_mean, run_var, z, gamma, beta, residual, y, B, HW, C, relu, eps,
                       momentum):
+    bits = relu_bits(y)
+    if bits is not None and int(relu) == 1 and not _is_f32(z):
+        _lib.call("cvl_bn_finalize_apply_bits", acc_ptr(stats), ptr(mean_rstd), ptr(run_mean), ptr(run_var), ptr(z),
+                  ptr(gamma), ptr(beta), ptr(residual), ptr(y), ptr(bits), B, HW, C, int(relu), float(eps),
+                  float(momentum), stream())
+        return
     _lib.call("cvl_bn_finalize_apply_f32" if _is_f32(z) else "cvl_bn_finalize_apply", acc_ptr(stats), ptr(mean_rstd), ptr(run_mean), ptr(run_var), ptr(z), ptr(gamma),
               ptr(beta), ptr(residual), ptr(y), B, HW, C, int(relu), float(eps), float(momentum), stream())
 
@@ -306,6 +323,13 @@
 def bn_finalize_apply_bnres(stats, mean_rstd, run_mean, run_var, z, gamma, beta, res_stats, res_mean_rstd,
                             res_run_mean, res_run_var, res_z, res_gamma, res_beta, res_eps, res_momentum, y, B,
                             HW, C, relu, eps, momentum):
+    bits = relu_bits(y)
+    if bits is not None and int(relu) == 1:
+        _lib.call("cvl_bn_finalize_apply_bnres_bits", acc_ptr(stats), ptr(mean_rstd), ptr(run_mean), ptr(run_var),
+                  ptr(z), ptr(gamma), ptr(beta), acc_ptr(res_stats), ptr(res_mean_rstd), ptr(res_run_mean),
+                  ptr(res_run_var), ptr(res_z), ptr(res_gamma), ptr(res_beta), float(res_eps), float(res_momentum),
+                  ptr(y), ptr(bits), B, HW, C, int(relu), float(eps), float(momentum), stream())
+        return
     _lib.call("cvl_bn_finalize_apply_bnres", acc_ptr(stats), ptr(mean_rstd), ptr(run_mean), ptr(run_var), ptr(z),
               ptr(gamma), ptr(beta), acc_ptr(res_stats), ptr(res_mean_rstd), ptr(res_run_mean), ptr(res_run_var),
               ptr(res_z), ptr(res_gamma), ptr(res_beta), float(res_eps), float(res_momentum), ptr(y), B, HW, C,
@@ -319,6 +343,12 @@
                                conv_dbias)
     n = int(_lib.load().cvl_bn_backward_workspace_size(B, HW, C))
     ws = torch.empty(n, dtype=torch.uint8, device=dy.device)
+    bits = relu_bits(y_relu)
+    if bits is not None:
+        _lib.call("cvl_bn_backward_bits", ptr(dy), ptr(bits), ptr(z), ptr(mean_rstd), ptr(gamma), ptr(ws), n,
+                  ptr(dz), ptr(g_out), ptr(dgamma), ptr(dbeta), float(beta_acc), ptr(conv_dbias), B, HW, C,
+                  stream())
+        return
     _lib.call("cvl_bn_backward", ptr(dy), ptr(y_relu), ptr(z), ptr(mean_rstd), ptr(gamma), ptr(ws), n,
               ptr(dz), ptr(g_out), ptr(dgamma), ptr(dbeta), float(beta_acc), ptr(conv_dbias), B, HW, C,
               stream())
@@ -388,6 +418,12 @@
     if zero:
         sums.zero_()
     flag = ctypes.c_int32(0)
+    bits = relu_bits(y)
+    if bits is not None and not _is_f32(src):
+        _lib.call("cvl_conv_igemm_dgrad_bnsum_res_bits", ctypes.byref(desc), ptr(src), ptr(dst), ptr(y), ptr(bits),
+                  ptr(z), ptr(mean_rstd), ptr(gamma), ptr(beta), acc_ptr(sums), ctypes.addressof(flag), None,
+                  ptr(ws), n if ws is not None else 0, stream())
+        return bool(flag.value)
     _lib.call("cvl_conv_igemm_dgrad_bnsum_res", ctypes.byref(desc), ptr(src), ptr(dst), ptr(y), ptr(z),
               ptr(mean_rstd), ptr(gamma), ptr(beta), acc_ptr(sums), ctypes.addressof(flag), ptr(ws),
               n if ws is not None else 0, stream())
@@ -396,6 +432,12 @@
 
 def bn_backward_res_sums(dy, y, z, mean_rstd, gamma, sums, dz, g_out, dgamma, dbeta, B, HW, C, beta_acc=0.0,
                          conv_dbias=None):
+    bits = relu_bits(y)
+    if bits is not None:
+        _lib.call("cvl_bn_backward_res_sums_bits", ptr(dy), ptr(bits), ptr(z), ptr(mean_rstd), ptr(gamma),
+                  acc_ptr(sums), ptr(dz), ptr(g_out), ptr(dgamma), ptr(dbeta), float(beta_acc), ptr(conv_dbias), B,
+                  HW, C, stream())
+        return
     _lib.call("cvl_bn_backward_res_sums", ptr(dy), ptr(y), ptr(z), ptr(mean_rstd), ptr(gamma), acc_ptr(sums), ptr(dz),
               ptr(g_out), ptr(dgamma), ptr(dbeta), float(beta_acc), ptr(conv_dbias), B, HW, C, stream())
 
@@ -404,7 +446,9 @@
                             B, HW, C, beta_acc=0.0, conv_dbias=None):
     n = int(_lib.load().cvl_bn_backward_res_sums_sc_workspace_size(B, HW, C))
     ws = torch.empty(n, dtype=torch.uint8, device=dy.device)
-    _lib.call("cvl_bn_backward_res_sums_sc", ptr(dy), ptr(y), ptr(z), ptr(mean_rstd), ptr(gamma), acc_ptr(sums),
+    bits = relu_bits(y)
+    _lib.call("cvl_bn_backward_res_sums_sc_bits" if bits is not None else "cvl_bn_backward_res_sums_sc", ptr(dy),
+              ptr(bits if bits is not None else y), ptr(z), ptr(mean_rstd), ptr(gamma), acc_ptr(sums),
               ptr(dz), ptr(g_out), ptr(dgamma), ptr(dbeta), float(beta_acc), ptr(conv_dbias), ptr(z_sc),
               ptr(mean_rstd_sc), ptr(ws), n, ptr(sc_sums), B, HW, C, stream())
 
@@ -413,7 +457,9 @@
                    beta_acc=0.0, conv_dbias=None):
     n = int(_lib.load().cvl_bn_backward_sc_workspace_size(B, HW, C))
     ws = torch.empty(n, dtype=torch.uint8, device=dy.device)
-    _lib.call("cvl_bn_backward_sc", ptr(dy), ptr(y), ptr(z), ptr(mean_rstd), ptr(gamma), ptr(ws), n, ptr(dz),
+    bits = relu_bits(y)
+    _lib.call("cvl_bn_backward_sc_bits" if bits is not None else "cvl_bn_backward_sc", ptr(dy),
+              ptr(bits if bits is not None else y), ptr(z), ptr(mean_rstd), ptr(gamma), ptr(ws), n, ptr(dz),
               ptr(g_out), ptr(dgamma), ptr(dbeta), float(beta_acc), ptr(conv_dbias), ptr(z_sc), ptr(mean_rstd_sc),
               ptr(sc_sums), B, HW, C, stream())
 
diff --git a/include/cvlite.h b/include/cvlite.h
--- a/include/cvlite.h
+++ b/include/cvlite.h
@@ -184,6 +184,40 @@
                          const uint64_t* sums, void* dz, float* dgamma, float* dbeta, float beta_acc,
                          float* conv_dbias, int B, int HW, int C, cvl_stream_t stream);
 
+int cvl_bn_finalize_apply_bits(uint64_t* stats, float* mean_rstd, float* run_mean, float* run_var, const void* z,
+                               const float* gamma, const float* beta, const void* residual, void* y,
+                               uint8_t* relu_bits, int B, int HW, int C, int relu, float eps, float momentum,
+                               cvl_stream_t stream);
+int cvl_bn_finalize_apply_bnres_bits(uint64_t* stats, float* mean_rstd, float* run_mean, float* run_var,
+                                     const void* z, const float* gamma, const float* beta, uint64_t* res_stats,
+                                     float* res_mean_rstd, float* res_run_mean, float* res_run_var,
+                                     const void* res_z, const float* res_gamma, const float* res_beta,
+                                     float res_eps, float res_momentum, void* y, uint8_t* relu_bits, int B, int HW,
+                                     int C, int relu, float eps, float momentum, cvl_stream_t stream);
+int cvl_bn_backward_bits(const void* dy, const uint8_t* relu_bits, const void* z, const float* mean_rstd,
+                         const float* gamma, void* workspace, size_t workspace_bytes, void* dz, void* g_out,
+                         float* dgamma, float* dbeta, float beta_acc, float* conv_dbias, int B, int HW, int C,
+                         cvl_stream_t stream);
+int cvl_bn_backward_res_sums_bits(const void* dy, const uint8_t* relu_bits, const void* z, const float* mean_rstd,
+                                  const float* gamma, uint64_t* sums, void* dz, void* g_out, float* dgamma,
+                                  float* dbeta, float beta_acc, float* conv_dbias, int B, int HW, int C,
+                                  cvl_stream_t stream);
+int cvl_bn_backward_res_sums_sc_bits(const void* dy, const uint8_t* relu_bits, const void* z, const float* mean_rstd,
+                                     const float* gamma, uint64_t* sums, void* dz, void* g_out, float* dgamma,
+                                     float* dbeta, float beta_acc, float* conv_dbias, const void* z_sc,
+                                     const float* mean_rstd_sc, void* workspace, size_t workspace_bytes,
+                                     uint64_t* sc_sums, int B, int HW, int C, cvl_stream_t stream);
+int cvl_bn_backward_sc_bits(const void* dy, const uint8_t* relu_bits, const void* z, const float* mean_rstd,
+                            const float* gamma, void* workspace, size_t workspace_bytes, void* dz, void* g_out,
+                            float* dgamma, float* dbeta, float beta_acc, float* conv_dbias, const void* z_sc,
+                            const float* mean_rstd_sc, uint64_t* sc_sums, int B, int HW, int C, cvl_stream_t stream);
+int cvl_conv_igemm_dgrad_bnsum_res_bits(const cvl_conv_desc* d, const void* src, void* dst, const void* y,
+                                        const uint8_t* relu_bits, const void* z, const float* mean_rstd,
+                                        const float* gamma, const float* beta, uint64_t* sums, int32_t* fused,
+                                        int32_t* form, void* workspace, size_t workspace_bytes, cvl_stream_t stream);
+int cvl_conv_igemm_plan_bnsum(const cvl_conv_desc* d, int offer, size_t workspace_bytes, int32_t* form,
+                              int32_t* kernel, int32_t* ktile);
+
 int cvl_bn_backward_relu6(const void* dy, const void* z, const float* mean_rstd, const float* gamma,
                           const float* beta, void* workspace, size_t workspace_bytes, void* dz, float* dgamma,
                           float* dbeta, float beta_acc, float* conv_dbias, int B, int HW, int C, cvl_stream_t stream);
```

Result: faster. 1454 images/s, median of 6 (+1.9%).
